# fnzhan/EMLight

Hardware: AMD Instinct MI355X
Metric: training images/sec (regression step: DenseNet-BC fwd + Sinkhorn loss + bwd + Adam) (higher is better)
Workload: dtype f32; 1 GPU; RegressionNetwork train step, BASELINE configs[1]; per_gpu_batch=64, global_batch=64, anchors=128, parallelism=single

## Files before the change

emlight_amd/RegressionNetwork/dense_engine_bwd.py:

```python
import ctypes
import os

import torch

from .. import _lib
from .._knobs import knob_choice, knob_flag


def _r16(v):
    return (v + 15) // 16 * 16


def _side_stream(dev, prio):
    if prio <= 0:
        return torch.cuda.Stream(device=dev, priority=prio)
    hip = ctypes.CDLL("libamdhip64.so")
    h = ctypes.c_void_p()
    with torch.cuda.device(dev):
        rc = hip.hipStreamCreateWithPriority(ctypes.byref(h), ctypes.c_uint(1), ctypes.c_int(prio))
    if rc != 0:
        raise RuntimeError("hipStreamCreateWithPriority failed (%d)" % rc)
    return torch.cuda.ExternalStream(h.value, device=dev)


def _masked_stream(dev, n_cu, keep):
    hip = ctypes.CDLL("libamdhip64.so")
    words = (n_cu + 31) // 32
    mask = (ctypes.c_uint32 * words)()
    for i in range(n_cu):
        if keep(i):
            mask[i // 32] |= 1 << (i % 32)
    h = ctypes.c_void_p()
    with torch.cuda.device(dev):
        rc = hip.hipExtStreamCreateWithCUMask(ctypes.byref(h), ctypes.c_uint32(words), mask)
    if rc != 0:
        raise RuntimeError("hipExtStreamCreateWithCUMask failed (%d)" % rc)
    return torch.cuda.ExternalStream(h.value, device=dev)


class _BwdBuffers:
    def gf12(self, r):
        if self.GF12[r] is None:
            self.GF12[r] = self._gf12_new()
        return self.GF12[r]

    def __init__(self, enc, ws, dev):
        f32 = dict(dtype=torch.float32, device=dev)
        self.G = [torch.zeros(blk["P"], blk["ld"], **f32) for blk in ws.blocks]
        self.GF = torch.zeros(ws.F.shape[0], ws.F.shape[1], **f32)
        maxP = ws.blocks[0]["P"]
        self.DZ = torch.empty(2, maxP, 48, **f32)
        self.ring = max(1, int(os.environ.get("EML_WGRAD_RING", 4))) if enc.overlap_wgrad(dev) else 1
        self.GF12 = [None] * self.ring
        self._gf12_new = lambda: torch.empty(maxP, 12, **f32)
        self.N12 = torch.empty(maxP, 12, **f32)
        self.TOP = torch.empty(2 * maxP * 12, **f32) if knob_flag("EML_DGRAD_TOP", True) else None
        kp, ko, g = enc.kp_max, max(enc.ko_max, 48), enc.grid_max
        self.Wd = [[torch.empty(lay["Kp"] * 48, **f32) for lay in blk["layers"]] for blk in ws.blocks]
        self.WdT = [torch.empty(blk["trans"]["Kp"] * blk["trans"]["Ko"], **f32) for blk in ws.blocks]
        self.permutes = None
        self.coef = torch.zeros(8, max(kp, ko), **f32)
        self.part2 = torch.zeros(2, g * kp * 2, dtype=torch.float64, device=dev)
        self.partW = torch.empty(g * max(kp * 48, 2 * 27 * 256, 4 * 1024), **f32)
        i32 = dict(dtype=torch.int32, device=dev)
        self.cond = [[torch.zeros(lay["Kp"], **i32) for lay in blk["layers"]] for blk in ws.blocks]
        self.condT = [torch.zeros(blk["trans"]["Kp"], **i32) for blk in ws.blocks]
        self.any_ill = torch.zeros(1, **i32)
        self.dg_grid = 128
        self.dg_scratch = torch.empty(self.dg_grid * kp, dtype=torch.float64, device=dev)
        self.side = None
        if enc.overlap_wgrad(dev):
            m = int(os.environ.get("EML_CU_SPLIT", 0))
            self.main_masked = None
            if m > 1:
                n_cu = torch.cuda.get_device_properties(dev).multi_processor_count
                self.side = _masked_stream(dev, n_cu, lambda i: i % m == m - 1)
                self.main_masked = _masked_stream(dev, n_cu, lambda i: i % m != m - 1)
            else:
                self.side = _side_stream(dev, int(os.environ.get("EML_SIDE_PRIO", 0)))
            self.partW3 = [torch.empty(g * 2 * 27 * 256, **f32) for _ in range(self.ring)]
            self.ev_ready = [torch.cuda.Event() for _ in range(self.ring)]
            self.ev_done = [None] * self.ring


def run_backward(enc, ws, x, gpooled, need_x=False, need_params=None):
    if getattr(ws, "bwd", None) is None:
        ws.bwd = _BwdBuffers(enc, ws, x.device)
    masked = getattr(ws.bwd, "main_masked", None)
    if masked is None:
        return _run_backward(enc, ws, x, gpooled, need_x, need_params)
    cur = torch.cuda.current_stream(x.device)
    masked.wait_stream(cur)
    with torch.cuda.stream(masked):
        out = _run_backward(enc, ws, x, gpooled, need_x, need_params)
    cur.wait_stream(masked)
    return out


def _run_backward(enc, ws, x, gpooled, need_x, need_params):
    L, p, st = _lib.lib(), _lib.ptr, _lib.current_stream()
    m = enc.model
    f = m.features
    if not m.training:
        raise NotImplementedError("HIP DenseNet backward is implemented for train-mode BatchNorm "
                                  "(EMLight trains and tests in train mode, train.py:42 / test.py:36-37)")
    dev = x.device
    B, _, H, W = x.shape
    G = enc._grid(dev)
    G3 = enc._grid3(dev)
    G3d = enc._tuned("EML_GRID3_DGRAD", 2 * G3 if knob_flag("EML_D3_SHORT", False) else G3)
    Gw = enc._tuned("EML_GRID_WGRAD1", G)
    Gd = enc._tuned("EML_GRID_DGRAD", G)
    Gb = min(enc.grid_max, 4 * enc._cu)
    bw = ws.bwd
    part = ws.partials
    ring = [0]
    if bw.side is not None:
        main = torch.cuda.current_stream(dev)
        st_side = ctypes.c_void_p(bw.side.cuda_stream)
        G3s = enc._tuned("EML_GRID3_SIDE", G3)
        bw.side.wait_stream(main)
    if bw.permutes is None:
        from .dense_engine import _PermuteTable
        bw.permutes = _PermuteTable()
    items = []
    for bi_, blk_ in enumerate(ws.blocks):
        mod_ = getattr(f, "denseblock%d" % (bi_ + 1))
        for l_, lay_ in enumerate(blk_["layers"]):
            items.append((getattr(mod_, "denselayer%d" % (l_ + 1)).conv1.weight, bw.Wd[bi_][l_], 2, 48, lay_["Cin"],
                          lay_["Kp"], 48))
        tr_ = blk_["trans"]
        items.append((getattr(f, "transition%d" % (bi_ + 1)).conv.weight, bw.WdT[bi_], 2, tr_["Cout"], blk_["Ctot"],
                      tr_["Kp"], tr_["Ko"]))
    bw.permutes.launch(L, st, items)
    params = enc.param_list()
    if need_params is None:
        need_params = [True] * len(params)
    from .._dist import grad_slot
    grads = {}
    for q, need in zip(params, need_params):
        slot = grad_slot(q) if need else None
        grads[id(q)] = slot if slot is not None else torch.empty_like(q)
    gr = lambda q: p(grads[id(q)])
    coefs = [tuple(bw.coef[3 * k + i] for i in range(3)) for k in range(2)]
    cA, cB, cC = coefs[0]
    sB, sC = bw.coef[6], bw.coef[7]

    direct = knob_choice("EML_DGAMMA_DIRECT", "always", ("always", "never")) != "never"
    c3_fold = knob_flag("EML_C3_FOLD", True)
    c3_gf = knob_flag("EML_C3_GF", False)
    bw.any_ill.zero_()

    def dgamma_direct(blk, X_ld, Pin, Hin, Win, pool, DY, ld_dy, Zr, ld_z, co, Cout, conv, Cin, scale1, shift1, cond, bn):
        if not direct:
            return
        a, b, c = co if co is not None else (None, None, None)
        _lib.check(L.eml_dense_bn_dgamma_direct_f32(
            p(blk["X"]), X_ld, Pin, Hin, Win, pool, p(DY), ld_dy, p(Zr), ld_z, p(a), p(b), p(c), Cout, p(conv.weight), Cin,
            p(scale1), p(shift1), p(blk["mean"]), p(blk["istd"]), p(cond), p(bw.dg_scratch), gr(bn.weight), bw.dg_grid, st),
            "eml_dense_bn_dgamma_direct_f32")

    def finalize(R, pstride, count, bn, mean, istd, C, Cpad, coef=0, s_acc=None, src=None, c_lo=0, c_hi=None, conv=None,
                 cond=None):
        a, b, c = coefs[coef] if coef is not None else (None, None, None)
        wargs = (p(bn.bias), p(conv.weight), gr(conv.weight), conv.weight.shape[0]) if conv is not None else (None, None, None, 0)
        _lib.check(L.eml_dense_bn_bwd_finalize_f32(
            p(part if src is None else src), R, pstride, float(count), p(bn.weight), p(mean), p(istd), C, Cpad, 1,
            gr(bn.weight), gr(bn.bias), p(a), p(b), p(c),
            p(sB) if s_acc is not None else None, p(sC) if s_acc is not None else None, int(bool(s_acc)),
            c_lo, Cpad if c_hi is None else c_hi, *wargs, p(cond), p(bw.any_ill) if cond is not None else None, st),
            "eml_dense_bn_bwd_finalize_f32")

    def parr(tensors):
        return (ctypes.c_void_p * len(tensors))(*[t.data_ptr() for t in tensors])

    def materialize(Gbuf, blk, c0, n):
        _lib.check(L.eml_dense_grad_materialize_f32(p(Gbuf), blk["ld"], p(blk["X"]), blk["ld"], p(sB), p(sC), c0, n,
                                                    blk["P"], st), "eml_dense_grad_materialize_f32")

    cf, k = enc.trans_cout[-1], enc.avgpool
    ldF = ws.F.shape[1]
    _lib.check(L.eml_dense_head_pool_bwd_f32(p(gpooled), p(ws.F), ldF, cf, B, ws.hf, ws.wf, k, p(bw.GF), ldF, st),
               "eml_dense_head_pool_bwd_f32")
    dY, ld_dy = bw.GF, ldF
    nb = len(ws.blocks)
    for bi in reversed(range(nb)):
        blk, tr = ws.blocks[bi], ws.blocks[bi]["trans"]
        mod = getattr(f, "denseblock%d" % (bi + 1))
        T, LN = getattr(f, "transition%d" % (bi + 1)), getattr(f, "last_norm%d" % (bi + 1))
        P, Hb, Wb, ld, ctot = blk["P"], blk["H"], blk["W"], blk["ld"], blk["Ctot"]
        cout, Ko, kpt = tr["Cout"], tr["Ko"], tr["Kp"]
        Pn = B * (Hb // 2) * (Wb // 2)
        Gbuf = bw.G[bi]
        gl0 = sum(enc.block_layers[:bi])
        top2 = bw.TOP[:2 * P * 12].view(2, P, 12) if bw.TOP is not None else None
        _lib.check(L.eml_dense_bn_bwd_stats_f32(p(dY), ld_dy, p(tr["T"]), Ko, None, 0, 0, cout, Pn, p(tr["tmean"]),
                                                p(tr["tistd"]), p(part), Gb, st), "eml_dense_bn_bwd_stats_f32")
        finalize(Gb, 2 * cout, Pn, LN, tr["tmean"], tr["tistd"], cout, Ko, coef=0)
        _lib.check(L.eml_dense_conv1x1_bwd_weight_f32(
            p(tr["A"]), kpt, Pn, Hb // 2, Wb // 2, 0, kpt, ctot, p(tr["one"]), p(tr["zero"]), p(dY), ld_dy, p(tr["T"]),
            Ko, p(cA), p(cB), p(cC), cout, p(bw.partW), gr(T.conv.weight), G, None, None, 0, None, 0, None, None, st),
            "eml_dense_conv1x1_bwd_weight_f32")
        _lib.check(L.eml_dense_conv1x1_bwd_data_f32(
            p(dY), ld_dy, p(tr["T"]), Ko, p(cA), p(cB), p(cC), Ko, p(bw.WdT[bi]), None, ld, p(tr["scale"]),
            p(tr["shift"]), None, None, Pn, Hb, Wb, 1, kpt, p(Gbuf), ld, 0, p(part), G, p(tr["mask16"]), st),
            "eml_dense_conv1x1_bwd_data_f32")
        finalize(G, 2 * kpt, P, T.norm, blk["mean"], blk["istd"], ctot, kpt, coef=None, s_acc=False, conv=T.conv,
                 cond=bw.condT[bi])
        dgamma_direct(blk, ld, P, Hb, Wb, 1, dY, ld_dy, tr["T"], Ko, coefs[0], cout, T.conv, ctot, tr["scale"], tr["shift"],
                      bw.condT[bi], T.norm)
        def conv2_backward(l, slot, n12=False, narrow_lo=None, top=False):
            lay = blk["layers"][l]
            Lm = getattr(mod, "denselayer%d" % (l + 1))
            cin, kp, z, dz = lay["Cin"], lay["Kp"], blk["Z"][l], bw.DZ[slot]
            gsrc = (p(bw.N12), 12, 0) if n12 else (p(top2[1]), 12, 0) if top else (p(Gbuf), ld, cin)
            r = ring[0] = (ring[0] + 1) % bw.ring
            if bw.side is not None and bw.ev_done[r] is not None:
                main.wait_event(bw.ev_done[r])
            fold = (bw.side is None and c3_fold
                    and L.eml_dense_conv3x3_bwd_fused_supported(gsrc[1], gsrc[2], ld, cin) == 1)
            q = ws.drop_plan[bi][l] if ws.drop_plan is not None else 0.0
            drop = (ws.drop_key, gl0 + l, q) if q > 0 else ()
            if fold:
                fn = "eml_dense_conv3x3_bwd_fused_drop_f32" if drop else "eml_dense_conv3x3_bwd_fused_f32"
                _lib.check(getattr(L, fn)(*gsrc, p(Lm.conv2.weight), p(z), p(lay["zmean"]), p(lay["zistd"]), p(dz), B, Hb, Wb,
                                          p(part), G3d, p(blk["X"]), ld, cin, p(sB), p(sC), p(bw.gf12(r)) if c3_gf else None,
                                          p(lay["scale2"]), p(lay["shift2"]), p(bw.partW), gr(Lm.conv2.weight), *drop, st), fn)
            else:
                fn = "eml_dense_conv3x3_bwd_data_drop_f32" if drop else "eml_dense_conv3x3_bwd_data_f32"
                _lib.check(getattr(L, fn)(*gsrc, p(Lm.conv2.weight), p(z), p(lay["zmean"]), p(lay["zistd"]), p(dz), B, Hb, Wb,
                                          p(part), G3d, p(blk["X"]), ld, cin, p(sB), p(sC), p(bw.gf12(r)), *drop, st), fn)
            if fold:
                pass
            elif bw.side is None:
                _lib.check(L.eml_dense_conv3x3_bwd_weight_f32(p(bw.gf12(r)), 12, 0, p(z), p(lay["scale2"]),
                                                              p(lay["shift2"]), B, Hb, Wb, p(bw.partW),
                                                              gr(Lm.conv2.weight), G3, st),
                           "eml_dense_conv3x3_bwd_weight_f32")
            else:
                bw.ev_ready[r].record(main)
                bw.side.wait_event(bw.ev_ready[r])
                _lib.check(L.eml_dense_conv3x3_bwd_weight_f32(p(bw.gf12(r)), 12, 0, p(z), p(lay["scale2"]),
                                                              p(lay["shift2"]), B, Hb, Wb, p(bw.partW3[r]),
                                                              gr(Lm.conv2.weight), G3s, st_side),
                           "eml_dense_conv3x3_bwd_weight_f32")
                if bw.ev_done[r] is None:
                    bw.ev_done[r] = torch.cuda.Event()
                bw.ev_done[r].record(bw.side)
            finalize(G3d, 96, P, Lm.norm2, lay["zmean"], lay["zistd"], 48, 48, coef=slot)
            a, b, c = coefs[slot]
            _lib.check(L.eml_dense_conv1x1_bwd_weight_f32(
                p(blk["X"]), ld, P, Hb, Wb, 0, kp, cin, p(lay["scale1"]), p(lay["shift1"]), p(dz), 48, p(z), 48,
                p(a), p(b), p(c), 48, p(bw.partW), gr(Lm.conv1.weight), Gw, p(dz),
                *((p(Lm.conv1.weight), narrow_lo, *((p(top2[0]), 12) if top else (p(Gbuf), ld)), p(bw.N12),
                   p(bw.part2[slot])) if narrow_lo is not None
                  else (None, 0, None, 0, None, None)), st), "eml_dense_conv1x1_bwd_weight_f32")
            return Lm

        def dgrad(layers, slots, k_lo, k_hi, top=False):
            lays = [blk["layers"][l] for l in layers]
            if top:
                _lib.check(L.eml_dense_conv1x1_bwd_data_multi_top_f32(
                    parr([bw.DZ[s_] for s_ in slots]), parr([bw.Wd[bi][l_] for l_ in layers]),
                    parr([y["scale1"] for y in lays]), parr([y["shift1"] for y in lays]),
                    parr([bw.part2[s_] for s_ in slots]), (ctypes.c_int * len(layers))(*[y["Kp"] for y in lays]),
                    P, k_hi, p(Gbuf), ld, Gd, parr([y["mask"] for y in lays]), p(top2), st),
                    "eml_dense_conv1x1_bwd_data_multi_top_f32")
                return
            _lib.check(L.eml_dense_conv1x1_bwd_data_multi_f32(
                len(layers), parr([bw.DZ[s_] for s_ in slots]), None, None, None, None,
                parr([bw.Wd[bi][l_] for l_ in layers]),
                parr([y["scale1"] for y in lays]), parr([y["shift1"] for y in lays]),
                parr([bw.part2[s_] for s_ in slots]), (ctypes.c_int * len(layers))(*[y["Kp"] for y in lays]),
                None, ld, None, None, P, k_lo, k_hi, p(Gbuf), ld, Gd,
                parr([y["mask"] for y in lays]), st),
                "eml_dense_conv1x1_bwd_data_multi_f32")

        def bn1_finalize(l, Lm, slot, c_lo, c_hi, rows=None):
            lay = blk["layers"][l]
            finalize(Gd if rows is None else rows, 2 * lay["Kp"], P, Lm.norm1, blk["mean"], blk["istd"], lay["Cin"], lay["Kp"], coef=None,
                     s_acc=True, src=bw.part2[slot], c_lo=c_lo, c_hi=c_hi, conv=Lm.conv1, cond=bw.cond[bi][l])

        def bn1_direct(l, Lm, slot):
            lay = blk["layers"][l]
            dgamma_direct(blk, ld, P, Hb, Wb, 0, bw.DZ[slot], 48, None, 0, None, 48, Lm.conv1, lay["Cin"], lay["scale1"],
                          lay["shift1"], bw.cond[bi][l], Lm.norm1)

        l = len(blk["layers"]) - 1
        have_top = False
        while l >= 0:
            if l >= 1:
                la, lb = l, l - 1
                cin_a, cin_b = blk["layers"][la]["Cin"], blk["layers"][lb]["Cin"]
                Lma = conv2_backward(la, 0, narrow_lo=cin_b, top=have_top)
                bn1_finalize(la, Lma, 0, cin_b, cin_a, rows=Gw)
                Lmb = conv2_backward(lb, 1, n12=True)
                to_top = (top2 is not None and lb >= 2 and blk["layers"][la]["mask"] is not None and bw.side is None
                          and cin_b >= 24 and cin_b % 4 == 0)
                dgrad([la, lb], [0, 1], 0, cin_b, top=to_top)
                have_top = to_top
                bn1_finalize(la, Lma, 0, 0, cin_b)
                bn1_finalize(lb, Lmb, 1, 0, blk["layers"][lb]["Kp"])
                bn1_direct(la, Lma, 0)
                bn1_direct(lb, Lmb, 1)
                l -= 2
            else:
                Lm0 = conv2_backward(l, 0)
                dgrad([l], [0], 0, blk["layers"][l]["Cin"])
                bn1_finalize(l, Lm0, 0, 0, blk["layers"][l]["Kp"])
                bn1_direct(l, Lm0, 0)
                l -= 1
        c0b = blk["C0"]
        norm0_fused = bi == 0 and knob_flag("EML_NORM0_FUSED", True) and c0b % 4 == 0 and c0b <= 32
        if not norm0_fused:
            materialize(Gbuf, blk, 0, c0b)
        dY, ld_dy = Gbuf, ld
    b0 = ws.blocks[0]
    c0 = enc.c_init
    if norm0_fused:
        _lib.check(L.eml_dense_norm0_bwd_stats_f32(p(dY), ld_dy, p(ws.Y0), c0, p(ws.scale0), p(ws.shift0), p(sB), p(sC), c0,
                                                   b0["P"], p(ws.mean0), p(ws.istd0), p(part), Gb, st),
                   "eml_dense_norm0_bwd_stats_f32")
    else:
        _lib.check(L.eml_dense_bn_bwd_stats_f32(p(dY), ld_dy, p(ws.Y0), c0, p(b0["X"]), b0["ld"], 1, c0, b0["P"],
                                                p(ws.mean0), p(ws.istd0), p(part), Gb, st), "eml_dense_bn_bwd_stats_f32")
    finalize(Gb, 2 * c0, b0["P"], f.norm0, ws.mean0, ws.istd0, c0, _r16(c0), coef=0)
    if norm0_fused:
        _lib.check(L.eml_dense_conv0_bwd_weight_fused_f32(p(x), p(dY), ld_dy, p(ws.Y0), c0, p(ws.scale0), p(ws.shift0), p(sB),
                                                          p(sC), p(cA), p(cB), p(cC), B, H, W, p(bw.partW),
                                                          gr(f.conv0.weight), G, st), "eml_dense_conv0_bwd_weight_fused_f32")
    else:
        _lib.check(L.eml_dense_conv0_bwd_weight_f32(p(x), p(dY), ld_dy, p(b0["X"]), b0["ld"], p(ws.Y0), c0, p(cA), p(cB),
                                                    p(cC), B, H, W, p(bw.partW), gr(f.conv0.weight), G, st),
                   "eml_dense_conv0_bwd_weight_f32")
    dx = None
    if need_x:
        dx = torch.empty(B, 3, H, W, dtype=torch.float32, device=dev)
        X1 = (None, 0) if norm0_fused else (p(b0["X"]), b0["ld"])
        _lib.check(L.eml_dense_conv0_bwd_data_f32(p(dY), ld_dy, *X1, p(ws.Y0), c0, p(ws.scale0), p(ws.shift0), p(sB), p(sC),
                                                  p(cA), p(cB), p(cC), p(f.conv0.weight), B, H, W, p(dx), st),
                   "eml_dense_conv0_bwd_data_f32")
    if bw.side is not None:
        main.wait_stream(bw.side)
    return dx, [grads[id(q)] for q in params]
```

emlight_amd/_lib.py:

```python
import ctypes
import os
import threading

_HERE = os.path.dirname(os.path.abspath(__file__))
LIB_PATH = os.environ.get("EML_LIB_PATH") or os.path.join(_HERE, "libemlight_hip.so")

_f32p = ctypes.c_void_p
_i32p = ctypes.c_void_p
_f64p = ctypes.c_void_p
_stream = ctypes.c_void_p
_int = ctypes.c_int
_u64 = ctypes.c_ulonglong

ABI_VERSION = 31

SIGNATURES = {
    "eml_abi_version": (_int, []),
    "eml_last_error": (ctypes.c_char_p, []),
    "eml_sg_rasterise_f32": (_int, [_f32p, _f32p, _f32p, _f32p, _int, _int, _int, _int, _stream]),
    "eml_sg_rasterise_ex_f32": (_int, [_f32p, _f32p, _f32p, _f32p, _int, _int, _int, _int, _int, ctypes.c_void_p, _stream]),
    "eml_sg_rasterise_bwd_colors_f32": (_int, [_f32p, _f32p, _f32p, _f32p, _int, _int, _int, _int, _stream]),
    "eml_emd_anchor_cost_f32": (_int, [_f32p, _f32p, _int, _stream]),
    "eml_sinkhorn_schedule_f32": (_int, [_f32p, _f32p, ctypes.c_long, ctypes.c_double, ctypes.c_double, _int,
                                         ctypes.c_double, _f32p, _f32p, _i32p, _f32p, _stream]),
    "eml_sinkhorn_work_floats": (ctypes.c_size_t, [_int, _int]),
    "eml_sinkhorn_fwd_f32": (_int, [_f32p, _f32p, _f32p, _f32p, _f32p, _f32p, ctypes.c_double, ctypes.c_double, _int,
                                    ctypes.c_double, _f32p, _f32p, _i32p, _f32p, _f32p, _f32p, _f32p, _f32p, _int, _int,
                                    _stream]),
    "eml_sinkhorn_fwd_ex_f32": (_int, [_f32p, _f32p, _f32p, _f32p, _f32p, _f32p, ctypes.c_double, ctypes.c_double, _int,
                                       ctypes.c_double, _f32p, _f32p, _i32p, _f32p, _f32p, _f32p, _f32p, _f32p, _int, _int,
                                       _int, _stream]),
    "eml_sinkhorn_fwd_rho_f32": (_int, [_f32p, _f32p, _f32p, _f32p, _f32p, _f32p, ctypes.c_double, ctypes.c_double, _int,
                                        ctypes.c_double, _f32p, _f32p, _i32p, _f32p, _f32p, _f32p, _f32p, _f32p, _int, _int,
                                        _int, ctypes.c_double, _f32p, _stream]),
    "eml_sinkhorn_bwd_f32": (_int, [_f32p, _f32p, _f32p, _int, _int, _stream]),
    "eml_sinkhorn_dim_work_floats": (ctypes.c_size_t, [_int, _int, _int]),
    "eml_sinkhorn_fwd_dim_f32": (_int, [_f32p, _f32p, _f32p, _f32p, _f32p, _f32p, ctypes.c_double, ctypes.c_double, _int,
                                        ctypes.c_double, _f32p, _f32p, _i32p, _f32p, _f32p, _f32p, _f32p, _f32p, _int, _int,
                                        _int, _int, ctypes.c_double, _f32p, _stream]),
    "eml_sinkhorn_schedule_dim_f32": (_int, [_f32p, _f32p, ctypes.c_long, _int, ctypes.c_double, ctypes.c_double, _int,
                                             ctypes.c_double, _f32p, _f32p, _i32p, _f32p, _stream]),
    "eml_sinkhorn_bwd_weights_f32": (_int, [_f32p, _f32p, _f32p, _f32p, _int, _int, _stream]),
    "eml_l1_pairs_partial_doubles": (ctypes.c_size_t, [_int]),
    "eml_l1_pairs_fwd_f32": (_int, [_int, ctypes.c_void_p, ctypes.c_void_p, ctypes.c_void_p, ctypes.c_void_p, ctypes.c_void_p,
                                    ctypes.c_void_p, _f64p, _f32p, _stream]),
    "eml_l1_pairs_bwd_f32": (_int, [_int, ctypes.c_void_p, ctypes.c_void_p, ctypes.c_void_p, ctypes.c_void_p, ctypes.c_void_p,
                                    ctypes.c_void_p, _f32p, ctypes.c_void_p, ctypes.c_void_p, ctypes.c_void_p, _stream]),
    "eml_colsum_partial_doubles": (ctypes.c_size_t, [_int]),
    "eml_colsum_f32": (_int, [_f32p, ctypes.c_long, _int, _f64p, _f32p, _stream]),
    "eml_gt_anchor_index_i32": (_int, [_f32p, _int, _int, _int, _i32p, _stream]),
    "eml_gt_parametrise_f64": (_int, [_f32p, _i32p, _i32p, _int, _int, _int, _int, _f32p, _f32p, _f32p, _stream]),
    "eml_pano_crop_f32": (_int, [ctypes.c_void_p, _int, _int, _int, _int, _int, _int, ctypes.c_double, ctypes.c_double, _f64p,
                                 ctypes.c_double, _f64p, _f32p, _stream]),
    "eml_pano_resize_area_f32": (_int, [_f32p, _int, _int, _int, _int, _int, ctypes.c_double, _f64p, _f32p, _stream]),
    "eml_tonemap_work_floats": (ctypes.c_size_t, [_int]),
    "eml_tonemap_f32": (_int, [_f32p, _int, ctypes.c_long, _int, ctypes.c_double, ctypes.c_double, ctypes.c_double, _f32p,
                               _int, _f32p, _f32p, _i32p, _f32p, ctypes.c_void_p, _stream]),
    "eml_projector_targets_work_floats": (ctypes.c_size_t, [_int, _int, _int]),
    "eml_projector_targets_f32": (_int, [_f32p, _f32p, _int, _int, _int, _f32p, _f32p, _f32p, _stream]),
    "eml_resize_bilinear_f32": (_int, [_f32p, _f32p, _int, _int, _int, _int, _int, _int, _int, _f32p, _stream]),
    "eml_sphere_tap_table_f32": (_int, [_f32p, _int, _int, _int, _int, _i32p, _f32p, _stream]),
    "eml_sphere_im2col_f32": (_int, [_f32p, _i32p, _f32p, _f32p, _int, _int, _int, _int, _stream]),
    "eml_sphere_col2im_f32": (_int, [_f32p, _i32p, _i32p, _f32p, _f32p, _int, _int, _int, _int, _stream]),
    "eml_sphere_conv_fwd_fused_f32": (_int, [_f32p, _i32p, _f32p, _f32p, _f32p, _f32p, _int, _int, _int, _int, _int, _int,
                                             _stream]),
    "eml_sphere_conv_fwd_fused_ex_f32": (_int, [_f32p, _i32p, _f32p, _f32p, _f32p, _f32p, _int, _int, _int, _int, _int, _int,
                                                _f32p, ctypes.c_float, _int, _stream]),
    "eml_sphere_conv_small_supported": (_int, [_int, _int]),
    "eml_sphere_conv_small_fwd_f32": (_int, [_f32p, _i32p, _f32p, _f32p, _f32p, _f32p, _int, _int, _int, _int, _int,
                                             ctypes.c_float, _stream]),
    "eml_sphere_conv_small_wgrad_partial_floats": (ctypes.c_size_t, [_int, _int, _int, _int]),
    "eml_sphere_conv_small_wgrad_f32": (_int, [_f32p, _i32p, _f32p, _f32p, _f32p, ctypes.c_float, _f32p, _f32p, _f32p, _int,
                                               _int, _int, _int, _int, _stream]),
    "eml_sphere_conv_small_da9_f32": (_int, [_f32p, _f32p, ctypes.c_float, _f32p, _f32p, ctypes.c_long, _int, _int, _stream]),
    "eml_spade_norm_modulate_up2_fwd_f32": (_int, [_f32p, _f32p, _f32p, _int, _int, _int, _int, ctypes.c_float, _f32p, _f32p,
                                                   _stream]),
    "eml_spade_norm_modulate_bwd_cols_f32": (_int, [_f32p, _f32p, _f32p, _f32p, _f32p, _int, _int, _int, _int, _int,
                                                    ctypes.c_float, _f32p, _f32p, _f32p, _int, _stream]),
    "eml_sg_rasterise_bwd_work_floats": (ctypes.c_size_t, [_int, _int, _int, _int]),
    "eml_sg_rasterise_bwd_colors_ex_f32": (_int, [_f32p, _f32p, _f32p, _f32p, _f32p, _int, _int, _int, _int, _int, _stream]),
    "eml_sg_rasterise_bwd_full_work_floats": (ctypes.c_size_t, [_int, _int, _int, _int]),
    "eml_sg_rasterise_bwd_f32": (_int, [_f32p, _f32p, _f32p, _f32p, _f32p, _f32p, _f32p, _f32p, _int, _int, _int, _int, _int,
                                        _stream]),
    "eml_sphere_conv_narrow_supported": (_int, [_int, _int]),
    "eml_sphere_conv_narrow_fwd_f32": (_int, [_f32p, _i32p, _f32p, _f32p, _f32p, _f32p, _int, _int, _int, _int, _int, _stream]),
    "eml_sphere_conv_narrow_dgrad_f32": (_int, [_f32p, _i32p, _f32p, _int, _f32p, _f32p, _int, _int, _int, _int, _int, _stream]),
    "eml_sphere_conv_narrow_wgrad_partial_floats": (ctypes.c_size_t, [_int, _int, _int, _int]),
    "eml_sphere_conv_narrow_wgrad_f32": (_int, [_f32p, _i32p, _f32p, _f32p, _f32p, _f32p, _int, _int, _int, _int, _int, _stream]),
    "eml_sphere_conv_narrow_scratch_floats": (ctypes.c_size_t, [_int, _int]),
    "eml_sphere_conv_narrow_fwd2_f32": (_int, [_f32p, _i32p, _f32p, _f32p, _f32p, _f32p, _f32p, _int, _int, _int, _int, _int, _stream]),
    "eml_sphere_conv_narrow_wgrad2_partial_floats": (ctypes.c_size_t, [_int, _int, _int]),
    "eml_sphere_conv_narrow_dgrad2_f32": (_int, [_f32p, _i32p, _f32p, _int, ctypes.c_void_p, _f32p, _f32p, _f32p, _int, _int, _int,
                                                 _int, _int, _int, _stream]),
    "eml_sphere_conv_narrow_wgrad2_f32": (_int, [_f32p, _i32p, _f32p, _int, ctypes.c_void_p, _f32p, _f32p, _f32p, _f32p, _int, _int,
                                                 _int, _int, _int, _stream]),
    "eml_sphere_conv_spade_supported": (_int, [_int, _int, ctypes.c_long]),
    "eml_sphere_conv_spade_fwd_f32": (_int, [_f32p, _i32p, _f32p, _f32p, _f32p, _f32p, _f32p, _f32p, _f32p, _f32p, _int, _int,
                                             _int, _int, _int, _int, ctypes.c_float, _int, _stream]),
    "eml_spade_norm_modulate_bwd_y_f32": (_int, [_f32p, _f32p, _f32p, _f32p, _f32p, _f32p, _int, _int, _int, _int, _int,
                                                 ctypes.c_float, _f32p, _f32p, _f32p, _int, _stream]),
    "eml_bn_bwd_apply_up2_f32": (_int, [_f32p, _f32p, _int, _int, _int, _int, _f32p, _f32p, _f32p, _f32p, _stream]),
    "eml_spectral_norm_scratch_floats": (ctypes.c_size_t, [_int, _int]),
    "eml_spectral_norm_w2_f32": (_int, [_f32p, _f32p, _f32p, _int, ctypes.c_float, _f32p, _f32p, _f32p, _f32p, _int, _int,
                                        _stream]),
    "eml_spectral_norm_w2_bwd_f32": (_int, [_f32p, _f32p, _f32p, _f32p, _f32p, _f32p, _f32p, _int, _int, _stream]),
    "eml_spectral_norm_w2_batch_f32": (_int, [_int, ctypes.c_void_p, ctypes.c_void_p, ctypes.c_void_p, _int, ctypes.c_float,
                                              ctypes.c_void_p, ctypes.c_void_p, ctypes.c_void_p, ctypes.c_void_p, ctypes.c_void_p,
                                              ctypes.c_void_p, _stream]),
    "eml_spade_heads_w2_f32": (_int, [_f32p, _f32p, _f32p, _f32p, _f32p, _f32p, _int, _int, _int, _stream]),
    "eml_instance_norm_act_fwd_f32": (_int, [_f32p, _f32p, _f32p, _int, _int, _int, _int, ctypes.c_float, ctypes.c_float,
                                             _stream]),
    "eml_instance_norm_act_bwd_f32": (_int, [_f32p, _f32p, _f32p, _f32p, _int, _int, _int, _int, ctypes.c_float, _stream]),
    "eml_sphere_conv_dgrad_fused_f32": (_int, [_f32p, _i32p, _f32p, _i32p, _int, _f32p, _f32p, _int, _int, _int, _int, _int,
                                               _int, _stream]),
    "eml_sphere_conv_lowres_variant": (_int, [_int, _int, _int, _int]),
    "eml_sphere_conv_lowres_table_i32": (_int, [_i32p, _i32p, _i32p, _int, _int, _stream]),
    "eml_sphere_conv_lowres_partial_floats": (ctypes.c_size_t, [ctypes.c_long, _int, _int]),
    "eml_sphere_conv_lowres_f32": (_int, [_f32p, _i32p, _f32p, _i32p, _int, _i32p, _int, _f32p, _f32p, _f32p, _f32p, _int, _int,
                                          _int, _int, _int, _int, _f32p, ctypes.c_float, _stream]),
    "eml_sphere_conv_wgrad_partial_floats": (ctypes.c_size_t, [_int, _int, _int]),
    "eml_sphere_conv_wgrad_fused_f32": (_int, [_f32p, _i32p, _f32p, _f32p, _f32p, _f32p, _int, _int, _int, _int, _int, _int,
                                               _stream]),
    "eml_spade_modulate_fwd_f32": (_int, [_f32p, _int, _f32p, _int, _f32p, _int, ctypes.c_long, _int, ctypes.c_float,
                                          _stream]),
    "eml_spade_modulate_bwd_f32": (_int, [_f32p, _int, _f32p, _int, _f32p, _int, _f32p, _int, _f32p, _int, ctypes.c_long,
                                          _int, ctypes.c_float, _stream]),
    "eml_bn_stats_f32": (_int, [_f32p, _int, ctypes.c_long, _int, _f32p, _int, _stream]),
    "eml_bn_fold_f64": (_int, [_f32p, _int, _int, _f32p, _stream]),
    "eml_bn_finalize_f32": (_int, [_f32p, _int, ctypes.c_float, ctypes.c_float, _f32p, _f32p, _f32p, _f32p, _stream]),
    "eml_spade_norm_modulate_fwd_f32": (_int, [_f32p, _int, _f32p, _int, _f32p, _int, ctypes.c_long, _int, ctypes.c_float,
                                               _f32p, _f32p, _stream]),
    "eml_bn_bwd_apply_f32": (_int, [_f32p, _int, _f32p, _int, ctypes.c_long, _int, _f32p, _f32p, _f32p, _f32p, _int,
                                    _stream]),
    "eml_dense_conv0_fwd_f32": (_int, [_f32p, _f32p, _f32p, _int, _int, _int, _int, _int, _f32p, _int, _stream]),
    "eml_dense_conv0_fwd_mfma_f32": (_int, [_f32p, _f32p, _f32p, _int, _int, _int, _int, _int, _f32p, _int, _stream]),
    "eml_dense_bn_apply_f32": (_int, [_f32p, _int, _f32p, _int, _int, ctypes.c_long, _f32p, _f32p, _int, _f32p,
                                      _int, _stream]),
    "eml_dense_bn_prepare_f32": (_int, [_f32p, _int, _int, _int, _int, ctypes.c_double, _f32p, _f32p, _f32p, _f32p,
                                        _f32p, _f32p, _f32p, _int, _int, ctypes.c_float, ctypes.c_float, _int,
                                        _f32p, _f32p, _stream]),
    "eml_dense_permute_w1_f32": (_int, [_f32p, _int, _int, _int, _f32p, _stream]),
    "eml_dense_permute_w2_f32": (_int, [_f32p, _int, _f32p, _stream]),
    "eml_dense_permute_batch_f32": (_int, [ctypes.c_void_p, _int, _stream]),
    "eml_dense_conv1x1_fwd_f32": (_int, [_f32p, _int, ctypes.c_long, _int, _int, _int, _int, _f32p, _f32p, _f32p,
                                         _int, _f32p, _int, _f32p, _int, ctypes.c_void_p, _stream]),
    "eml_dense_conv3x3_fwd_f32": (_int, [_f32p, _f32p, _f32p, _f32p, _f32p, _int, _int, _int, _int, _int, _f32p,
                                         _int, _stream]),
    "eml_dense_permute_w2_tp_f32": (_int, [_f32p, _f32p, _stream]),
    "eml_dense_conv3x3_fwd_tp_supported": (_int, [_int, _int, _int]),
    "eml_dense_conv3x3_fwd_tp_f32": (_int, [_f32p, _f32p, _f32p, _f32p, _f32p, _int, _int, _int, _int, _int, _int, _f32p,
                                            _int, _stream]),
    "eml_dense_conv3x3_fwd_drop_f32": (_int, [_f32p, _f32p, _f32p, _f32p, _f32p, _int, _int, _int, _int, _int, _f32p,
                                              _int, _u64, _int, ctypes.c_double, _stream]),
    "eml_dense_conv3x3_fwd_tp_drop_f32": (_int, [_f32p, _f32p, _f32p, _f32p, _f32p, _int, _int, _int, _int, _int, _int, _f32p,
                                                 _int, _u64, _int, ctypes.c_double, _stream]),
    "eml_dense_dropout_mask_u16": (_int, [_u64, _int, ctypes.c_double, ctypes.c_long, ctypes.c_void_p, _stream]),
    "eml_dense_pool_act_f32": (_int, [_f32p, _int, _int, _int, _int, _int, _f32p, _f32p, _f32p, _int, ctypes.c_void_p,
                                      _stream]),
    "eml_dense_head_pool_fwd_f32": (_int, [_f32p, _int, _int, _int, _int, _int, _int, _f32p, _stream]),
    "eml_dense_conv3x3_bwd_data_f32": (_int, [_f32p, _int, _int, _f32p, _f32p, _f32p, _f32p, _f32p, _int, _int, _int,
                                              _f32p, _int, _f32p, _int, _int, _f32p, _f32p, _f32p, _stream]),
    "eml_dense_conv3x3_bwd_fused_supported": (_int, [_int, _int, _int, _int]),
    "eml_dense_conv3x3_bwd_fused_f32": (_int, [_f32p, _int, _int, _f32p, _f32p, _f32p, _f32p, _f32p, _int, _int, _int, _f64p, _int,
                                               _f32p, _int, _int, _f32p, _f32p, _f32p, _f32p, _f32p, _f32p, _f32p, _stream]),
    "eml_dense_conv3x3_bwd_data_drop_f32": (_int, [_f32p, _int, _int, _f32p, _f32p, _f32p, _f32p, _f32p, _int, _int, _int,
                                                   _f32p, _int, _f32p, _int, _int, _f32p, _f32p, _f32p, _u64, _int,
                                                   ctypes.c_double, _stream]),
    "eml_dense_conv3x3_bwd_fused_drop_f32": (_int, [_f32p, _int, _int, _f32p, _f32p, _f32p, _f32p, _f32p, _int, _int, _int,
                                                    _f64p, _int, _f32p, _int, _int, _f32p, _f32p, _f32p, _f32p, _f32p, _f32p,
                                                    _f32p, _u64, _int, ctypes.c_double, _stream]),
    "eml_dense_conv3x3_bwd_weight_f32": (_int, [_f32p, _int, _int, _f32p, _f32p, _f32p, _int, _int, _int, _f32p,
                                                _f32p, _int, _stream]),
    "eml_dense_bn_bwd_finalize_f32": (_int, [_f32p, _int, _int, ctypes.c_double, _f32p, _f32p, _f32p, _int, _int,
                                             _int, _f32p, _f32p, _f32p, _f32p, _f32p, _f32p, _f32p, _int, _int, _int,
                                             _f32p, _f32p, _f32p, _int, _i32p, _i32p, _stream]),
    "eml_dense_bn_dgamma_direct_f32": (_int, [_f32p, _int, ctypes.c_long, _int, _int, _int, _f32p, _int, _f32p, _int,
                                              _f32p, _f32p, _f32p, _int, _f32p, _int, _f32p, _f32p, _f32p, _f32p, _i32p,
                                              _f32p, _f32p, _int, _stream]),
    "eml_dense_conv1x1_bwd_weight_f32": (_int, [_f32p, _int, ctypes.c_long, _int, _int, _int, _int, _int, _f32p,
                                                _f32p, _f32p, _int, _f32p, _int, _f32p, _f32p, _f32p, _int, _f32p,
                                                _f32p, _int, _f32p, _f32p, _int, _f32p, _int, _f32p, _f32p, _stream]),
    "eml_dense_conv1x1_bwd_narrow_f32": (_int, [_f32p, _f32p, _int, _int, _f32p, _int, _f32p, _f32p, _f32p, _f32p,
                                                ctypes.c_long, _f32p, _int, _f32p, _f32p, _int, _int, _stream]),
    "eml_dense_permute_w1_bwd_f32": (_int, [_f32p, _int, _int, _int, _int, _f32p, _stream]),
    "eml_dense_conv1x1_bwd_data_f32": (_int, [_f32p, _int, _f32p, _int, _f32p, _f32p, _f32p, _int, _f32p, _f32p,
                                              _int, _f32p, _f32p, _f32p, _f32p, ctypes.c_long, _int, _int, _int,
                                              _int, _f32p, _int, _int, _f32p, _int, ctypes.c_void_p, _stream]),
    "eml_dense_conv1x1_bwd_data_multi_f32": (_int, [_int] + [ctypes.c_void_p] * 10 + [_f32p, _int, _f32p, _f32p,
                                                    ctypes.c_long, _int, _int, _f32p, _int, _int, ctypes.c_void_p,
                                                    _stream]),
    "eml_dense_conv1x1_bwd_data_multi_top_f32": (_int, [ctypes.c_void_p] * 6 + [ctypes.c_long, _int, _f32p, _int, _int,
                                                        ctypes.c_void_p, _f32p, _stream]),
    "eml_dense_grad_materialize_f32": (_int, [_f32p, _int, _f32p, _int, _f32p, _f32p, _int, _int, ctypes.c_long,
                                              _stream]),
    "eml_dense_bn_bwd_stats_f32": (_int, [_f32p, _int, _f32p, _int, _f32p, _int, _int, _int, ctypes.c_long, _f32p,
                                          _f32p, _f32p, _int, _stream]),
    "eml_dense_norm0_bwd_stats_f32": (_int, [_f32p, _int, _f32p, _int, _f32p, _f32p, _f32p, _f32p, _int, ctypes.c_long, _f32p, _f32p,
                                             ctypes.c_void_p, _int, _stream]),
    "eml_dense_conv0_bwd_weight_fused_f32": (_int, [_f32p, _f32p, _int, _f32p, _int, _f32p, _f32p, _f32p, _f32p, _f32p, _f32p, _f32p,
                                                    _int, _int, _int, _f32p, _f32p, _int, _stream]),
    "eml_dense_conv0_bwd_weight_f32": (_int, [_f32p, _f32p, _int, _f32p, _int, _f32p, _int, _f32p, _f32p, _f32p,
                                              _int, _int, _int, _f32p, _f32p, _int, _stream]),
    "eml_dense_conv0_bwd_data_f32": (_int, [_f32p, _int, _f32p, _int, _f32p, _int, _f32p, _f32p, _f32p, _f32p, _f32p, _f32p,
                                            _f32p, _f32p, _int, _int, _int, _f32p, _stream]),
    "eml_dense_head_pool_bwd_f32": (_int, [_f32p, _f32p, _int, _int, _int, _int, _int, _int, _f32p, _int, _stream]),
}

_lock = threading.Lock()
_lib = None


class EmlightHipError(RuntimeError):
    pass


def lib():
    global _lib
    if _lib is not None:
        return _lib
    with _lock:
        if _lib is not None:
            return _lib
        if not os.path.exists(LIB_PATH):
            raise EmlightHipError(
                "libemlight_hip.so not found at %s -- build it with "
                "`python -c 'import __graft_entry__ as g; g.build()'` or `make -C emlight_amd/csrc`. "
                "There is no CPU fallback." % LIB_PATH)
        handle = ctypes.CDLL(LIB_PATH)
        for name, (res, args) in SIGNATURES.items():
            try:
                fn = getattr(handle, name)
            except AttributeError as e:
                raise EmlightHipError("libemlight_hip.so lacks symbol %s" % name) from e
            fn.restype, fn.argtypes = res, args
        got = handle.eml_abi_version()
        if got != ABI_VERSION:
            raise EmlightHipError("libemlight_hip.so has ABI version %d, this binding expects %d -- rebuild it "
                                  "(make -C emlight_amd/csrc)" % (got, ABI_VERSION))
        _lib = handle
    from . import _gemm_selection
    _gemm_selection.ensure_if_requested()
    return _lib


_DEBUG_SYNC = bool(os.environ.get("EML_DEBUG_SYNC"))


def check(rc, what):
    if rc != 0:
        msg = lib().eml_last_error()
        raise EmlightHipError("%s failed (rc=%d): %s" % (what, rc, msg.decode() if msg else "?"))
    if _DEBUG_SYNC:
        import sys
        import torch
        sys.stderr.write("[eml] %s ... " % what)
        sys.stderr.flush()
        torch.cuda.synchronize()
        sys.stderr.write("ok\n")


def ptr(t):
    if t is None:
        return None
    return ctypes.c_void_p(t.data_ptr())


def current_stream():
    import torch
    return ctypes.c_void_p(torch.cuda.current_stream().cuda_stream)


def require_gpu_tensor(t, name, dtype=None):
    import torch
    if not isinstance(t, torch.Tensor) or not t.is_cuda:
        raise EmlightHipError("%s must be a tensor on the MI355X (got %s); there is no CPU path"
                              % (name, getattr(t, "device", type(t))))
    if t.dtype != (dtype or torch.float32):
        raise EmlightHipError("%s must be %s (got %s)" % (name, dtype or torch.float32, t.dtype))
    return t.contiguous()
```

emlight_amd/csrc/dense_bwd.hip:

```cpp
#include "eml_common.h"
#include "eml_dropout.h"

#include <cstdint>
#include <cstdlib>
#include <type_traits>

namespace {

using f32x4 = __attribute__((ext_vector_type(4))) float;

__device__ __forceinline__ f32x4 mfma16(float a, float b, f32x4 c) {
  return __builtin_amdgcn_mfma_f32_16x16x4f32(a, b, c, 0, 0, 0);
}
__device__ __forceinline__ float f4c(const float4& v, int t) { return t == 0 ? v.x : t == 1 ? v.y : t == 2 ? v.z : v.w; }
__device__ __forceinline__ double shfl_xor_d(double v, int m) { return __shfl_xor(v, m, 64); }

constexpr int kTH = 8, kTW = 32, kHH = kTH + 2, kHW = kTW + 2;

constexpr int kPSG = 14;
constexpr int kBD = 512;
constexpr int kGRows = 2;
constexpr int kGPass = kHH / kGRows;

template <bool FUSE, bool WIDE, int TH, bool DROP = false>
// ... 837 lines not shown
    asm volatile("s_mov_b32 %0, m0\n\ts_mov_b32 m0, %2\n\ts_nop 0\n\tglobal_load_lds_dwordx4 %1, off\n\ts_mov_b32 m0, %0"
                 : "=&s"(keep) : "v"(src), "s"(dst) : "memory");
  };

  int tile = blockIdx.x, cur = 0;
  __syncthreads();
  if (tile < ntiles) {
    stage_begin(tile);
    g_load(0);
    g_load(1);
    {
      const int b = tile / (ty_n * tx_n), rem = tile - b * (ty_n * tx_n);
#pragma unroll
      for (int it = 0; it < kZI; ++it) z_dma(it, b, (rem / tx_n) * kTH, (rem % tx_n) * kTW, 0);
    }
    g_wait();
    g_commit(0, g_l);
    g_commit(1, g_l);
    g_store(0);
    g_store(1);
  }
  __syncthreads();
#ifdef EML_STAMPS
  unsigned long long st_acc[5] = {0, 0, 0, 0, 0}, st_last = __builtin_readcyclecounter();
#endif
  for (; tile < ntiles; tile += gridDim.x) {
    const int nxt = tile + gridDim.x;
    const float* gc = g_l + cur * kGT;
    float* gn = g_l + (cur ^ 1) * kGT;
    const int b = tile / (ty_n * tx_n), rem = tile - b * (ty_n * tx_n);
    const int ty = rem / tx_n, tx = rem - ty * tx_n;
    const int gy = ty * kTH + wave;
    size_t prow[2];
    bool pv[2];
#pragma unroll
    for (int m = 0; m < 2; ++m) {
      const int gx = tx * kTW + 16 * m + r;
      pv[m] = gy < H && gx < W;
      prow[m] = ((size_t)(b * H + min(gy, H - 1)) * W + min(gx, W - 1)) * 48;
    }
    stage_begin(nxt < ntiles ? nxt : tile);
    f32x4 acc[2][3];
#pragma unroll
    for (int m = 0; m < 2; ++m)
#pragma unroll
      for (int n = 0; n < 3; ++n) acc[m][n] = f32x4{0.f, 0.f, 0.f, 0.f};
    float aq[2][2], wq[2][3];
#pragma unroll
    for (int n = 0; n < 3; ++n) wq[0][n] = w_l[n * 64 + lane];
#pragma unroll
    for (int m = 0; m < 2; ++m) aq[0][m] = gc[((wave + 2) * kHW + 16 * m + r + 2) * kPSG + kk];
#pragma unroll
    for (int tap = 0; tap < 9; ++tap) {
#pragma unroll
      for (int s3 = 0; s3 < 3; ++s3) {
        const int gi = tap * 3 + s3;
        if (gi < 2) {
          g_load(gi);
          asm volatile("" ::: "memory");
          __builtin_amdgcn_sched_barrier(0);
        }
        if (gi + 1 < 27) {
          const int tn = (gi + 1) / 3, sn = (gi + 1) - 3 * tn, dyn = tn / 3, dxn = tn - 3 * dyn;
#pragma unroll
          for (int n = 0; n < 3; ++n) wq[(gi + 1) & 1][n] = w_l[((gi + 1) * 3 + n) * 64 + lane];
#pragma unroll
          for (int m = 0; m < 2; ++m)
            aq[(gi + 1) & 1][m] = gc[((wave + 2 - dyn) * kHW + 16 * m + r + 2 - dxn) * kPSG + 4 * sn + kk];
        }
        __builtin_amdgcn_sched_barrier(0);
#pragma unroll
        for (int m = 0; m < 2; ++m)
#pragma unroll
          for (int n = 0; n < 3; ++n) acc[m][n] = mfma16(wq[gi & 1][n], aq[gi & 1][m], acc[m][n]);
        if (gi >= 25) {
          __builtin_amdgcn_sched_barrier(0);
          if (gi == 25) g_wait();
          g_commit(gi - 25, gn);
        }
      }
    }
    g_store(0);
    g_store(1);
    EML_C3_STAMP(0);
#ifndef EML_C3_NOZWAIT
    asm volatile("s_waitcnt vmcnt(0)" ::: "memory");
#endif
    eml::lds_barrier();
    EML_C3_STAMP(1);
    const float* ga = gc + ((2 * pairj + 1) * kHW + kk + 1) * kPSG;
    const float* zc = z_l + cur * (kTH * kTW * kZS);
    const float* zb = zc + (kTW * 2 * pairj + kk) * kZS + r;
    const int xl0 = ty * kTH + 2 * pairj < H ? W - tx * kTW - kk : 0, xl1 = ty * kTH + 2 * pairj + 1 < H ? W - tx * kTW - kk : 0;
    auto phase_b = [&](auto nt_tag) {
      constexpr int NT = decltype(nt_tag)::value;
      float av[2][NT], bz[2][3];
#pragma unroll
      for (int i = 0; i < NT; ++i) av[0][i] = ga[goff[i]];
#pragma unroll
      for (int n = 0; n < 3; ++n) bz[0][n] = zb[16 * n];
#pragma unroll
      for (int ks = 0; ks < 16; ++ks) {
        if (ks + 1 < 16) {
          const int k1 = ks + 1, go = ((k1 >> 3) * kHW + 4 * (k1 & 7)) * kPSG, zo = ((k1 >> 3) * kTW + 4 * (k1 & 7)) * kZS;
#pragma unroll
          for (int i = 0; i < NT; ++i) av[k1 & 1][i] = ga[go + goff[i]];
#pragma unroll
          for (int n = 0; n < 3; ++n) bz[k1 & 1][n] = zb[zo + 16 * n];
        }
        __builtin_amdgcn_sched_barrier(0);
        if (ks == 1) {
          const int t2 = nxt < ntiles ? nxt : tile;
          const int b2 = t2 / (ty_n * tx_n), rem2 = t2 - b2 * (ty_n * tx_n);
#ifndef EML_C3_NOZDMA
#pragma unroll
          for (int it = 0; it < kZI; ++it) z_dma(it, b2, (rem2 / tx_n) * kTH, (rem2 % tx_n) * kTW, cur ^ 1);
#endif
          __builtin_amdgcn_sched_barrier(0);
        }
        const bool pin = 4 * (ks & 7) < (ks < 8 ? xl0 : xl1);
        float bv[3];
#pragma unroll
        for (int n = 0; n < 3; ++n) bv[n] = pin ? fmaf(bz[ks & 1][n], scb[n], shb[n]) : 0.f;
#pragma unroll
        for (int i = 0; i < NT; ++i) {
          const float a = (i < 3 || r < 12) ? av[ks & 1][i] : 0.f;
#pragma unroll
          for (int n = 0; n < 3; ++n) accw[i][n] = mfma16(a, bv[n], accw[i][n]);
        }
        if (ks == 2 || ks == 4 || ks == 6) {
          const int n = (ks - 2) >> 1;
          float l1[4] = {0.f, 0.f, 0.f, 0.f}, l2[4] = {0.f, 0.f, 0.f, 0.f};
#pragma unroll
          for (int m = 0; m < 2; ++m) {
            const float4 z = *reinterpret_cast<const float4*>(zc + (kTW * wave + 16 * m + r) * kZS + 16 * n + 4 * kk);
#pragma unroll
            for (int g = 0; g < 4; ++g) {
              const float v = pv[m] ? acc[m][n][g] : 0.f;
              l1[g] += v;
              l2[g] = fmaf(v, f4c(z, g), l2[g]);
            }
          }
#pragma unroll
          for (int g = 0; g < 4; ++g) {
            const float t1 = eml::row16_sum(l1[g]), t2 = eml::row16_sum(l2[g]);
            if (r == 0) {
              double* d = red + (wave * 48 + 16 * n + 4 * kk + g) * 2;
              d[0] += (double)t1;
              d[1] += (double)t2;
            }
          }
        } else if (ks >= 8 && ks < 14) {
          const int si = ks - 8, m = si / 3, n = si - 3 * m;
          if (pv[m])
            *reinterpret_cast<float4*>(DZ + prow[m] + 16 * n + 4 * kk) =
                make_float4(acc[m][n][0], acc[m][n][1], acc[m][n][2], acc[m][n][3]);
        }
        __builtin_amdgcn_sched_barrier(0);
      }
    };
    if (role == 0) phase_b(std::integral_constant<int, 3>{});
    else phase_b(std::integral_constant<int, 4>{});
    EML_C3_STAMP(2);
    eml::lds_barrier();
    EML_C3_STAMP(3);
#ifdef EML_STAMPS
    st_acc[4] += 1;
#endif
    cur ^= 1;
  }
#ifdef EML_STAMPS
  if (tid == 0)
    for (int i = 0; i < 5; ++i) atomicAdd(&eml_c3_stamps[i], st_acc[i]);
#endif
  asm volatile("s_waitcnt vmcnt(0)" ::: "memory");
  __syncthreads();
  float* wsum = smem;
  for (int w8 = 0; w8 < 8; ++w8) {
    if (wave == w8) {
#pragma unroll
      for (int i = 0; i < 4; ++i)
        if (i < 3 + role) {
#pragma unroll
          for (int n = 0; n < 3; ++n)
#pragma unroll
            for (int g = 0; g < 4; ++g) {
              float* q = wsum + ((((3 * role + i) * 3 + n) * 16 + 4 * kk + g) * 16 + r);
              *q = ((w8 & 3) == 0 ? 0.f : *q) + accw[i][n][g];
            }
        }
    }
    __syncthreads();
  }
  for (int e = tid; e < 21 * 256; e += 512) partialW[(size_t)blockIdx.x * (21 * 256) + e] = wsum[e];
  if (tid < 48) {
    double t1 = 0.0, t2 = 0.0;
#pragma unroll
    for (int w8 = 0; w8 < 8; ++w8) {
      t1 += red[(w8 * 48 + tid) * 2 + 0];
      t2 += red[(w8 * 48 + tid) * 2 + 1];
    }
    partials[(size_t)blockIdx.x * 96 + 2 * tid + 0] = t1;
    partials[(size_t)blockIdx.x * 96 + 2 * tid + 1] = (double)zistd[tid] * (t2 - (double)zmean[tid] * t1);
  }
}


__global__ __launch_bounds__(256) void bn_bwd_finalize_kernel(
    const double* __restrict__ partials, int R, int pstride, double count, const float* __restrict__ gamma,
    const float* __restrict__ mean, const float* __restrict__ istd, int C, int Cpad, int training,
    float* __restrict__ dgamma, float* __restrict__ dbeta, float* __restrict__ cA, float* __restrict__ cB,
    float* __restrict__ cC, float* __restrict__ sB, float* __restrict__ sC, int s_accumulate, int c_lo, int c_hi,
    const float* __restrict__ beta, const float* __restrict__ Wc, const float* __restrict__ dWc, int w_rows,
    int* __restrict__ cond , int* __restrict__ any_cond ) {
  const int lane = threadIdx.x & 63, wave = threadIdx.x >> 6;
  const int c = c_lo + blockIdx.x * 4 + wave;
  if (c >= Cpad || c >= c_hi) return;
  float a = 0.f, b = 0.f, d = 0.f;
  if (c < C) {
    double S1 = 0.0, S2 = 0.0;
    for (int g = lane; g < R; g += 64) {
      S1 += partials[(size_t)g * pstride + 2 * c];
      S2 += partials[(size_t)g * pstride + 2 * c + 1];
    }
    double Q = 0.0;
    if (Wc)
      for (int o = lane; o < w_rows; o += 64) Q += (double)Wc[(size_t)o * C + c] * (double)dWc[(size_t)o * C + c];
#pragma unroll
    for (int o = 32; o > 0; o >>= 1) {
      S1 += __shfl_xor(S1, o, 64);
      S2 += __shfl_xor(S2, o, 64);
      Q += __shfl_xor(Q, o, 64);
    }
    if (Wc) {
      const double ga0 = gamma[c], bs = (double)beta[c] * S1, num = Q - bs;
      S2 = fabs(ga0) >= 1e-12 ? num / ga0 : 0.0;
      if (cond && lane == 0) {
        const int ill = fabs(ga0) < 1e-3 * fabs((double)beta[c]) || ga0 == 0.0;
        cond[c] = ill;
        if (ill && any_cond) *any_cond = 1;
      }
    }
    if (lane == 0) {
      dgamma[c] = (float)S2;
      dbeta[c] = (float)S1;
    }
    const double ga = gamma[c], is = istd[c], mu = mean[c];
    a = (float)(ga * is);
    if (training) {
      b = (float)(-ga * is * is * S2 / count);
      d = (float)(-ga * is * S1 / count + ga * is * is * S2 / count * mu);
    }
  }
  if (lane != 0) return;
  if (cA) {
    cA[c] = a;
    cB[c] = b;
    cC[c] = d;
  }
  if (sB) {
    sB[c] = (s_accumulate ? sB[c] : 0.f) + b;
    sC[c] = (s_accumulate ? sC[c] : 0.f) + d;
  }
}

__global__ __launch_bounds__(256) void reduce_rows_kernel(const float* __restrict__ partial, int R, size_t row_stride,
                                                          int mode, int dim0, int dim1, int n0,
                                                          float* __restrict__ out) {
  __shared__ double red[4][64];
  const int tid = threadIdx.x, e = blockIdx.x * 64 + (tid & 63), slice = tid >> 6;
  size_t src = 0, dst = 0;
  bool valid = false;
  if (mode == 0) {
    const int k = e / 48, o = e - 48 * k;
    valid = k < dim0 && o < dim1;
    src = (size_t)e;
    dst = (size_t)(n0 + o) * dim0 + k;
  } else if (mode == 1) {
    const int o = e & 15, ci = (e >> 4) & 15, pair = e >> 8, tap = pair / 3, mc = pair - 3 * tap;
    valid = pair < 27 && o < 12;
    src = (size_t)e;
    dst = (size_t)(o * 48 + 16 * mc + ci) * 9 + tap;
  } else if (mode == 3) {
    const int j = e & 15, i = (e >> 4) & 15, tn = e >> 8, t = tn / 3, n = tn - 3 * t, row = 16 * t + i;
    valid = tn < 21 && row < 108;
    src = (size_t)e;
    dst = (size_t)((row % 12) * 48 + 16 * n + j) * 9 + row / 12;
  } else {
    const int t = e >> 5, o = e & 31;
    valid = t < 27 && o < dim1;
    src = (size_t)e;
    dst = (size_t)o * 27 + t;
  }
  double s = 0.0;
  if (valid) {
#pragma unroll 8
    for (int r = slice; r < R; r += 4) s += (double)partial[(size_t)r * row_stride + src];
  }
  red[slice][tid & 63] = s;
  __syncthreads();
  if (slice == 0 && valid) out[dst] = (float)((red[0][tid] + red[1][tid]) + (red[2][tid] + red[3][tid]));
}

struct NarrowArgs {
  const float* W1;
  const float* G;
  float* N12;
  double* partials;
  int Cin, k_lo, ldg;
};
template <bool POOL, bool NARROW = false, int VEC = 2>
__global__ __launch_bounds__(256, (NARROW || VEC == 4) ? 2 : 1) void conv1x1_bwd_weight_kernel(
    const float* __restrict__ X, int ldx, int P, int Hin, int Win, int Kp, const float* __restrict__ scale1,
    const float* __restrict__ shift1, const float* __restrict__ DY, int ld_dy, const float* __restrict__ Zr,
    int ld_z, const float* __restrict__ cA, const float* __restrict__ cB, const float* __restrict__ cC, int n_valid,
    int n_load ,
    float* __restrict__ partial ,
    float* __restrict__ dz_out ,
    NarrowArgs na) {
  __shared__ __attribute__((aligned(16))) float dz_l[2][64 * 48];
  const int tid = threadIdx.x, lane = tid & 63, wave = tid >> 6;
  const int r = lane & 15, kk = lane >> 4;
  static_assert(VEC == 2 || (VEC == 4 && !POOL), "float4 operand: dense layers only");
  constexpr int GW = 16 * VEC;
  constexpr int MAXG = VEC == 2 ? 3 : 2;
  const int ngroups = (Kp + GW - 1) / GW;
  float nsk[4] = {0.f, 0.f, 0.f, 0.f}, ntk[4] = {0.f, 0.f, 0.f, 0.f};
  double ns1[4] = {0.0, 0.0, 0.0, 0.0};
  const int kq = min(kk, 2);
  if constexpr (NARROW) {
#pragma unroll
    for (int g = 0; g < 4; ++g) {
      nsk[g] = kk < 3 ? scale1[na.k_lo + 4 * kq + g] : 0.f;
      ntk[g] = kk < 3 ? shift1[na.k_lo + 4 * kq + g] : 0.f;
    }
  }

  float sv[MAXG][VEC], tv[MAXG][VEC];
  int coff[MAXG];
  bool gv[MAXG];
#pragma unroll
  for (int i = 0; i < MAXG; ++i) {
    const int cg = wave + 4 * i;
    const int ch = GW * cg + VEC * r;
    gv[i] = cg < ngroups && ch < Kp;
    coff[i] = gv[i] ? ch : 0;
#pragma unroll
    for (int t = 0; t < VEC; ++t) {
      sv[i][t] = gv[i] ? scale1[ch + t] : 0.f;
      tv[i][t] = gv[i] ? shift1[ch + t] : 0.f;
    }
  }
  const int spix = tid >> 2, sq = tid & 3;
  __shared__ __attribute__((aligned(16))) float co_l[3 * 48];
  __shared__ float wn_l[NARROW ? 12 * 64 : 1];
  constexpr bool CO_LDS = NARROW || VEC == 4;
  float4 sa_r[CO_LDS ? 1 : 3], sb_r[CO_LDS ? 1 : 3], sc_r[CO_LDS ? 1 : 3];
  if constexpr (CO_LDS) {
    if (tid < 48) {
      const bool v = tid < n_valid;
      co_l[tid] = v ? cA[tid] : 0.f;
      co_l[48 + tid] = v ? cB[tid] : 0.f;
      co_l[96 + tid] = v ? cC[tid] : 0.f;
    }
  } else {
#pragma unroll
    for (int j = 0; j < 3; ++j) {
      const int col = 4 * (sq + 4 * j);
      float a[4], b[4], c[4];
#pragma unroll
      for (int e = 0; e < 4; ++e) {
        const bool v = col + e < n_valid;
        a[e] = v ? cA[col + e] : 0.f;
        b[e] = v ? cB[col + e] : 0.f;
        c[e] = v ? cC[col + e] : 0.f;
      }
      sa_r[j] = make_float4(a[0], a[1], a[2], a[3]);
      sb_r[j] = make_float4(b[0], b[1], b[2], b[3]);
      sc_r[j] = make_float4(c[0], c[1], c[2], c[3]);
    }
  }
  if constexpr (NARROW) {
    for (int e = tid; e < 12 * 64; e += 256) {
      const int st = e >> 6, l = e & 63, rr = l & 15, k4 = l >> 4;
      wn_l[e] = rr < 12 ? na.W1[(size_t)(4 * st + k4) * na.Cin + na.k_lo + rr] : 0.f;
    }
  }
  __syncthreads();
  f32x4 acc[MAXG][VEC][3];
#pragma unroll
  for (int i = 0; i < MAXG; ++i)
#pragma unroll
    for (int t = 0; t < VEC; ++t)
#pragma unroll
      for (int n = 0; n < 3; ++n) acc[i][t][n] = f32x4{0.f, 0.f, 0.f, 0.f};

  const int Wo = Win >> 1, Ho = Hin >> 1;
  const int nchunks = (P + 63) >> 6;
  const int ngw = (ngroups > wave) ? (ngroups - wave + 3) >> 2 : 0;

  float4 rdy[3], rzr[3];
  bool rpv = false;
  int rp = 0;
  auto stage_load = [&](int chunk) {
    const int p = chunk * 64 + spix;
    rpv = chunk < nchunks && p < P;
    const size_t pc = rpv ? p : 0;
    rp = (int)pc;
#pragma unroll
    for (int j = 0; j < 3; ++j) {
      const int col = 4 * (sq + 4 * j);
      const bool cv = col < n_load;
      rdy[j] = cv ? *reinterpret_cast<const float4*>(DY + pc * ld_dy + col) : make_float4(0.f, 0.f, 0.f, 0.f);
      rzr[j] = cv ? *reinterpret_cast<const float4*>(Zr + pc * ld_z + col) : make_float4(0.f, 0.f, 0.f, 0.f);
    }
  };
  auto stage_write = [&](float* dzb) {
#pragma unroll
    for (int j = 0; j < 3; ++j) {
      const int col = 4 * (sq + 4 * j);
      float4 sa, sb, sc;
      if constexpr (CO_LDS) {
        sa = *reinterpret_cast<const float4*>(co_l + col);
        sb = *reinterpret_cast<const float4*>(co_l + 48 + col);
        sc = *reinterpret_cast<const float4*>(co_l + 96 + col);
      } else {
        sa = sa_r[j];
        sb = sb_r[j];
        sc = sc_r[j];
      }
      float4 v;
      v.x = rpv ? fmaf(sa.x, rdy[j].x, fmaf(sb.x, rzr[j].x, sc.x)) : 0.f;
      v.y = rpv ? fmaf(sa.y, rdy[j].y, fmaf(sb.y, rzr[j].y, sc.y)) : 0.f;
      v.z = rpv ? fmaf(sa.z, rdy[j].z, fmaf(sb.z, rzr[j].z, sc.z)) : 0.f;
      v.w = rpv ? fmaf(sa.w, rdy[j].w, fmaf(sb.w, rzr[j].w, sc.w)) : 0.f;
      *reinterpret_cast<float4*>(dzb + spix * 48 + col) = v;
      if (dz_out && rpv) *reinterpret_cast<float4*>(dz_out + (size_t)rp * 48 + col) = v;
    }
  };
  auto chunk_loop = [&](auto ngw_c) {
    constexpr int NGW = decltype(ngw_c)::value;
#ifdef EML_WGRAD_DEEP
    constexpr int UQ = POOL ? 1 : 2;
    constexpr int NBUF = POOL ? 2 : 4;
#else
    constexpr int UQ = POOL ? 1 : (VEC == 4 ? 2 : 4);
    constexpr int NBUF = 2;
#endif
    constexpr int NS = POOL ? 4 : 1;
    constexpr int NB = 16 / UQ;
    constexpr int AHEAD = NBUF - 1;
    using xv_t = std::conditional_t<VEC == 2, float2, float4>;
    xv_t xr[NBUF][UQ][NGW > 0 ? NGW : 1][NS];
    auto load_batch = [&](int chunk, int q0, xv_t (&dst)[UQ][NGW > 0 ? NGW : 1][NS]) {
#pragma unroll
      for (int u = 0; u < UQ; ++u) {
        const int pc = min(chunk * 64 + 4 * (q0 + u) + kk, P - 1);
        const float* xp;
        if constexpr (POOL) {
          const int b = pc / (Ho * Wo), rem = pc - b * (Ho * Wo);
          const int oy = rem / Wo, ox = rem - oy * Wo;
          xp = X + ((size_t)(b * Hin + 2 * oy) * Win + 2 * ox) * ldx;
        } else {
          xp = X + (size_t)pc * ldx;
        }
#pragma unroll
        for (int i = 0; i < NGW; ++i)
#pragma unroll
          for (int sub = 0; sub < NS; ++sub)
            dst[u][i][sub] = *reinterpret_cast<const xv_t*>(xp + ((sub >> 1) * (size_t)Win + (sub & 1)) * ldx + coff[i]);
      }
    };
    stage_load(blockIdx.x);
    stage_write(dz_l[0]);
    if constexpr (NGW > 0) {
#pragma unroll
      for (int a = 0; a < AHEAD; ++a) load_batch(min((int)blockIdx.x, nchunks - 1), a * UQ, xr[a]);
    }
    __syncthreads();
    int it = 0;
    for (int chunk = blockIdx.x; chunk < nchunks; chunk += gridDim.x, ++it) {
      const float* dzb = dz_l[it & 1];
      stage_load(chunk + gridDim.x);
      float2 nx[2], ng[2];
      const int pn = chunk * 64 + 16 * wave + r;
      if constexpr (NARROW) {
        const size_t pc = (size_t)min(pn, P - 1);
        const float* xs = X + pc * ldx + na.k_lo + 4 * kq;
        const float* gs = na.G + pc * na.ldg + (na.ldg == 12 ? 0 : na.k_lo) + 4 * kq;
        nx[0] = *reinterpret_cast<const float2*>(xs);
        nx[1] = *reinterpret_cast<const float2*>(xs + 2);
        ng[0] = *reinterpret_cast<const float2*>(gs);
        ng[1] = *reinterpret_cast<const float2*>(gs + 2);
      }
      if constexpr (NGW > 0) {
        float bzq[2][3];
#pragma unroll
        for (int n = 0; n < 3; ++n) bzq[0][n] = dzb[kk * 48 + 16 * n + r];
#pragma unroll
        for (int bi = 0; bi < NB; ++bi) {
          const int q0 = bi * UQ;
          if (bi + AHEAD < NB)
            load_batch(chunk, q0 + AHEAD * UQ, xr[(bi + AHEAD) % NBUF]);
          else
            load_batch(min(chunk + (int)gridDim.x, nchunks - 1), (bi + AHEAD - NB) * UQ, xr[(bi + AHEAD) % NBUF]);
          __builtin_amdgcn_sched_barrier(0);
#pragma unroll
          for (int u = 0; u < UQ; ++u) {
            const int pl = 4 * (q0 + u) + kk;
            const bool pvu = chunk * 64 + pl < P;
            float bz[3];
#pragma unroll
            for (int n = 0; n < 3; ++n) bz[n] = bzq[(q0 + u) & 1][n];
            if (q0 + u + 1 < 16) {
#pragma unroll
              for (int n = 0; n < 3; ++n) bzq[(q0 + u + 1) & 1][n] = dzb[(pl + 4) * 48 + 16 * n + r];
            }
#pragma unroll
            for (int i = 0; i < NGW; ++i) {
              float av[VEC];
#pragma unroll
              for (int t = 0; t < VEC; ++t) av[t] = 0.f;
#pragma unroll
              for (int sub = 0; sub < NS; ++sub) {
                const xv_t xv = xr[bi % NBUF][u][i][sub];
                av[0] += fmaxf(fmaf(xv.x, sv[i][0], tv[i][0]), 0.f);
                av[1] += fmaxf(fmaf(xv.y, sv[i][1], tv[i][1]), 0.f);
                if constexpr (VEC == 4) {
                  av[2] += fmaxf(fmaf(xv.z, sv[i][2], tv[i][2]), 0.f);
                  av[3] += fmaxf(fmaf(xv.w, sv[i][3], tv[i][3]), 0.f);
                }
              }
#pragma unroll
              for (int t = 0; t < VEC; ++t) {
                if constexpr (POOL) av[t] *= 0.25f;
                if (!pvu) av[t] = 0.f;
              }
#pragma unroll
              for (int n = 0; n < 3; ++n)
#pragma unroll
                for (int t = 0; t < VEC; ++t) acc[i][t][n] = mfma16(av[t], bz[n], acc[i][t][n]);
            }
          }
          __builtin_amdgcn_sched_barrier(0);
        }
      }
      if constexpr (NARROW) {
        asm volatile("" ::"v"(ng[0].x), "v"(ng[0].y), "v"(ng[1].x), "v"(ng[1].y), "v"(nx[0].x), "v"(nx[0].y), "v"(nx[1].x), "v"(nx[1].y));
        f32x4 an = f32x4{0.f, 0.f, 0.f, 0.f};
#pragma unroll
        for (int st = 0; st < 12; ++st) an = mfma16(wn_l[st * 64 + lane], dzb[(16 * wave + r) * 48 + 4 * st + kk], an);
        const bool nv = pn < P && kk < 3;
        const float xg[4] = {nx[0].x, nx[0].y, nx[1].x, nx[1].y}, gg[4] = {ng[0].x, ng[0].y, ng[1].x, ng[1].y};
        float o4[4];
#pragma unroll
        for (int g = 0; g < 4; ++g) {
          const float dam = (nv && fmaf(xg[g], nsk[g], ntk[g]) > 0.f) ? an[g] : 0.f;
          o4[g] = fmaf(nsk[g], dam, gg[g]);
          ns1[g] += (double)dam;
        }
        if (nv) *reinterpret_cast<float4*>(na.N12 + ((unsigned)pn * 12u + 4u * (unsigned)kk)) = make_float4(o4[0], o4[1], o4[2], o4[3]);
      }
      stage_write(dz_l[(it + 1) & 1]);
      eml::lds_barrier();
    }
  };
  switch (ngw) {
    case 0: chunk_loop(std::integral_constant<int, 0>{}); break;
    case 1: chunk_loop(std::integral_constant<int, 1>{}); break;
    case 2: chunk_loop(std::integral_constant<int, 2>{}); break;
    default: chunk_loop(std::integral_constant<int, MAXG>{}); break;
  }
  float* out = partial + (size_t)blockIdx.x * Kp * 48;
#pragma unroll
  for (int i = 0; i < MAXG; ++i) {
    const int cg = wave + 4 * i;
#pragma unroll
    for (int t = 0; t < VEC; ++t)
#pragma unroll
      for (int g = 0; g < 4; ++g) {
        const int ch = GW * cg + VEC * (4 * kk + g) + t;
        if (cg < ngroups && ch < Kp) {
#pragma unroll
          for (int n = 0; n < 3; ++n) out[(size_t)ch * 48 + 16 * n + r] = acc[i][t][n][g];
        }
      }
  }
  if constexpr (NARROW) {
    __syncthreads();
    double* red = reinterpret_cast<double*>(&dz_l[0][0]);
#pragma unroll
    for (int g = 0; g < 4; ++g) {
#pragma unroll
      for (int o = 1; o < 16; o <<= 1) ns1[g] += shfl_xor_d(ns1[g], o);
      if (r == 0 && kk < 3) red[wave * 12 + 4 * kk + g] = ns1[g];
    }
    __syncthreads();
    if (tid < 12) {
      double* dst = na.partials + ((size_t)blockIdx.x * Kp + na.k_lo + tid) * 2;
      dst[0] = (red[tid] + red[12 + tid]) + (red[24 + tid] + red[36 + tid]);
      dst[1] = 0.0;
    }
  }
}

template <bool POOL, bool RES , int NCH = 4>
__global__ __launch_bounds__(256) void conv1x1_bwd_data_kernel(
    const float* __restrict__ DY, int ld_dy, const float* __restrict__ Zr, int ld_z, const float* __restrict__ cA,
    const float* __restrict__ cB, const float* __restrict__ cC, int Ko, const float* __restrict__ Wd,
    const float* __restrict__ X, int ldx, const float* __restrict__ scale1, const float* __restrict__ shift1,
    const float* __restrict__ mean, const float* __restrict__ istd, int P, int Hin, int Win, int Kp,
    float* __restrict__ Gd, int ldg, int accumulate, double* __restrict__ partials ) {
  extern __shared__ __attribute__((aligned(16))) float smem[];
  double* sacc = reinterpret_cast<double*>(smem);
  const int tid = threadIdx.x, lane = tid & 63, wave = tid >> 6;
  const int r = lane & 15, kk = lane >> 4;
  for (int e = tid; e < 4 * Kp * 2; e += 256) sacc[e] = 0.0;
  __syncthreads();
  double* my = sacc + (size_t)wave * Kp * 2;
  const int nnt = Kp >> 4, njo = Ko >> 4;
  const int ntiles = (P + 255) >> 8;
  const int Wo = Win >> 1, Ho = Hin >> 1;

  for (int tile = blockIdx.x; tile < ntiles; tile += gridDim.x) {
    const int p0 = tile * 256 + wave * 64;
    long prow[4];
    size_t pin[4];
#pragma unroll
    for (int m = 0; m < 4; ++m) {
      prow[m] = min(p0 + 16 * m + r, P - 1);
      if constexpr (POOL) {
        const int b = (int)(prow[m] / (Ho * Wo)), rem = (int)(prow[m] - (long)b * (Ho * Wo));
        const int oy = rem / Wo, ox = rem - oy * Wo;
        pin[m] = (size_t)(b * Hin + 2 * oy) * Win + 2 * ox;
      } else {
        pin[m] = (size_t)prow[m];
      }
    }
    auto load_dz = [&](int jo, float4 (&dz)[4]) {
      const int ch = 16 * jo + 4 * kk;
      const float4 a4 = *reinterpret_cast<const float4*>(cA + ch);
      const float4 b4 = *reinterpret_cast<const float4*>(cB + ch);
      const float4 c4 = *reinterpret_cast<const float4*>(cC + ch);
#pragma unroll
      for (int m = 0; m < 4; ++m) {
        const float4 dy = *reinterpret_cast<const float4*>(DY + prow[m] * ld_dy + ch);
        const float4 zr = *reinterpret_cast<const float4*>(Zr + prow[m] * ld_z + ch);
        dz[m].x = fmaf(a4.x, dy.x, fmaf(b4.x, zr.x, c4.x));
        dz[m].y = fmaf(a4.y, dy.y, fmaf(b4.y, zr.y, c4.y));
        dz[m].z = fmaf(a4.z, dy.z, fmaf(b4.z, zr.z, c4.z));
        dz[m].w = fmaf(a4.w, dy.w, fmaf(b4.w, zr.w, c4.w));
      }
    };
    float4 dzr[3][4];
    if constexpr (RES) {
#pragma unroll
      for (int jo = 0; jo < 3; ++jo) load_dz(jo, dzr[jo]);
    }
    for (int nt0 = 0; nt0 < nnt; nt0 += NCH) {
      f32x4 acc[4][NCH];
#pragma unroll
      for (int m = 0; m < 4; ++m)
#pragma unroll
        for (int n = 0; n < NCH; ++n) acc[m][n] = f32x4{0.f, 0.f, 0.f, 0.f};
      auto mma = [&](int jo, const float4 (&dz)[4]) {
#pragma unroll
        for (int n = 0; n < NCH; ++n) {
          const int nt = min(nt0 + n, nnt - 1);
          const float4 w = *reinterpret_cast<const float4*>(Wd + ((((size_t)nt * njo + jo) * 4 + kk) * 16 + r) * 4);
#pragma unroll
          for (int t = 0; t < 4; ++t)
#pragma unroll
            for (int m = 0; m < 4; ++m) acc[m][n] = mfma16(f4c(w, t), f4c(dz[m], t), acc[m][n]);
        }
      };
      if constexpr (RES) {
#pragma unroll
        for (int jo = 0; jo < 3; ++jo) mma(jo, dzr[jo]);
      } else {
        for (int jo = 0; jo < njo; ++jo) {
          float4 dz[4];
          load_dz(jo, dz);
          mma(jo, dz);
        }
      }
#pragma unroll
      for (int n = 0; n < NCH; ++n) {
        const int nt = nt0 + n;
        if (nt < nnt) {
          const int k4 = 16 * nt + 4 * kk;
          const float4 sk = *reinterpret_cast<const float4*>(scale1 + k4);
          const float4 tk = *reinterpret_cast<const float4*>(shift1 + k4);
          const float4 mu = *reinterpret_cast<const float4*>(mean + k4);
          const float4 is = *reinterpret_cast<const float4*>(istd + k4);
          float l1[4] = {0.f, 0.f, 0.f, 0.f}, l2[4] = {0.f, 0.f, 0.f, 0.f};
#pragma unroll
          for (int m = 0; m < 4; ++m) {
            if (p0 + 16 * m + r < P) {
              const float da[4] = {acc[m][n][0], acc[m][n][1], acc[m][n][2], acc[m][n][3]};
              constexpr int NSUB = POOL ? 4 : 1;
#pragma unroll
              for (int sub = 0; sub < NSUB; ++sub) {
                const size_t pi = pin[m] + (sub >> 1) * (size_t)Win + (sub & 1);
                const float4 xv = *reinterpret_cast<const float4*>(X + pi * ldx + k4);
                float4* gp = reinterpret_cast<float4*>(Gd + pi * ldg + k4);
                float4 g = accumulate ? *gp : make_float4(0.f, 0.f, 0.f, 0.f);
                const float f = POOL ? 0.25f : 1.0f;
                const float d0 = (fmaf(xv.x, sk.x, tk.x) > 0.f) ? f * da[0] : 0.f;
                const float d1 = (fmaf(xv.y, sk.y, tk.y) > 0.f) ? f * da[1] : 0.f;
                const float d2 = (fmaf(xv.z, sk.z, tk.z) > 0.f) ? f * da[2] : 0.f;
                const float d3 = (fmaf(xv.w, sk.w, tk.w) > 0.f) ? f * da[3] : 0.f;
                g.x = fmaf(sk.x, d0, g.x);
                g.y = fmaf(sk.y, d1, g.y);
                g.z = fmaf(sk.z, d2, g.z);
                g.w = fmaf(sk.w, d3, g.w);
                *gp = g;
                l1[0] += d0;
                l1[1] += d1;
                l1[2] += d2;
                l1[3] += d3;
                l2[0] = fmaf(d0, (xv.x - mu.x) * is.x, l2[0]);
                l2[1] = fmaf(d1, (xv.y - mu.y) * is.y, l2[1]);
                l2[2] = fmaf(d2, (xv.z - mu.z) * is.z, l2[2]);
                l2[3] = fmaf(d3, (xv.w - mu.w) * is.w, l2[3]);
              }
            }
          }
#pragma unroll
          for (int g = 0; g < 4; ++g) {
            l1[g] = eml::row16_sum(l1[g]);
            l2[g] = eml::row16_sum(l2[g]);
            if (r == 0) {
              my[2 * (k4 + g)] += (double)l1[g];
              my[2 * (k4 + g) + 1] += (double)l2[g];
            }
          }
        }
      }
    }
  }
  __syncthreads();
  for (int e = tid; e < Kp * 2; e += 256)
    partials[(size_t)blockIdx.x * Kp * 2 + e] =
        (sacc[e] + sacc[(size_t)Kp * 2 + e]) + (sacc[(size_t)2 * Kp * 2 + e] + sacc[(size_t)3 * Kp * 2 + e]);
}

template <int MT, int NCH, bool ACC , bool MASKED = false, int NJO = 0>
__global__ __launch_bounds__(256, 2) void transition_bwd_data_kernel(
    const float* __restrict__ DY, int ld_dy, const float* __restrict__ Zr, int ld_z, const float* __restrict__ cA,
    const float* __restrict__ cB, const float* __restrict__ cC, int Ko, const float* __restrict__ Wd,
    const float* __restrict__ X, int ldx, const float* __restrict__ scale1, const float* __restrict__ shift1,
    const float* __restrict__ mean, const float* __restrict__ istd, int P, int Hin, int Win, int Kp,
    float* __restrict__ Gd, int ldg, double* __restrict__ partials ,
    const unsigned short* __restrict__ mask16) {
  extern __shared__ __attribute__((aligned(16))) float smem[];
  double* sacc = reinterpret_cast<double*>(smem);
  float* vec_l = reinterpret_cast<float*>(sacc + (size_t)4 * Kp * 2);
  float* co_l = vec_l + 4 * Kp;
  float* stg = co_l + 3 * Ko + (size_t)(threadIdx.x >> 6) * 16 * 36;
  const int tid = threadIdx.x, lane = tid & 63, wave = tid >> 6;
  const int r = lane & 15, kk = lane >> 4;
  for (int e = tid; e < 4 * Kp * 2; e += 256) sacc[e] = 0.0;
  for (int e = tid; e < Kp; e += 256) {
    vec_l[e] = scale1[e];
    vec_l[Kp + e] = shift1[e];
    vec_l[2 * Kp + e] = MASKED ? 0.f : mean[e];
    vec_l[3 * Kp + e] = MASKED ? 0.f : istd[e];
  }
  for (int e = tid; e < Ko; e += 256) {
    co_l[e] = cA[e];
    co_l[Ko + e] = cB[e];
    co_l[2 * Ko + e] = cC[e];
  }
  __syncthreads();
  double* my = sacc + (size_t)wave * Kp * 2;
  const int nnt = Kp >> 4, njo = Ko >> 4;
  constexpr int TP = 64 * MT;
  const int ntiles = (P + TP - 1) / TP;
  const int Wo = Win >> 1, Ho = Hin >> 1;

  for (int tile = blockIdx.x; tile < ntiles; tile += gridDim.x) {
    const int p0 = tile * TP + wave * 16 * MT;
    long prow[MT];
    size_t pin[MT];
    bool pv[MT];
#pragma unroll
    for (int m = 0; m < MT; ++m) {
      pv[m] = p0 + 16 * m + r < P;
      prow[m] = min(p0 + 16 * m + r, P - 1);
      const int b = (int)(prow[m] / (Ho * Wo)), rem = (int)(prow[m] - (long)b * (Ho * Wo));
      const int oy = rem / Wo, ox = rem - oy * Wo;
      pin[m] = (size_t)(b * Hin + 2 * oy) * Win + 2 * ox;
    }
    size_t pinx[MT][2];
    bool pvx[MT][2];
    if constexpr (MASKED && !ACC) {
#pragma unroll
      for (int m = 0; m < MT; ++m)
#pragma unroll
        for (int h = 0; h < 2; ++h) {
          const int src = (lane >> 3) + 8 * h;
          pinx[m][h] = (size_t)__shfl((unsigned long long)pin[m], src, 64);
          pvx[m][h] = __shfl((int)pv[m], src, 64) != 0;
        }
    }
    float4 dzr[NJO > 0 ? NJO : 1][MT];
    if constexpr (NJO > 0) {
#pragma unroll
      for (int jo = 0; jo < NJO; ++jo) {
        const int ch = 16 * jo + 4 * kk;
        const float4 a4 = *reinterpret_cast<const float4*>(co_l + ch);
        const float4 b4 = *reinterpret_cast<const float4*>(co_l + Ko + ch);
        const float4 c4 = *reinterpret_cast<const float4*>(co_l + 2 * Ko + ch);
#pragma unroll
        for (int m = 0; m < MT; ++m) {
          const float4 y4 = *reinterpret_cast<const float4*>(DY + prow[m] * ld_dy + ch);
          const float4 z4 = *reinterpret_cast<const float4*>(Zr + prow[m] * ld_z + ch);
          dzr[jo][m].x = fmaf(a4.x, y4.x, fmaf(b4.x, z4.x, c4.x));
          dzr[jo][m].y = fmaf(a4.y, y4.y, fmaf(b4.y, z4.y, c4.y));
          dzr[jo][m].z = fmaf(a4.z, y4.z, fmaf(b4.z, z4.z, c4.z));
          dzr[jo][m].w = fmaf(a4.w, y4.w, fmaf(b4.w, z4.w, c4.w));
        }
      }
    }
    for (int nt0 = 0; nt0 < nnt; nt0 += NCH) {
      float4 xv[MASKED ? 1 : MT][MASKED ? 1 : NCH][4], gs[ACC ? MT : 1][ACC ? NCH : 1][4];
      unsigned mk[MT][NCH];
#pragma unroll
      for (int n = 0; n < NCH; ++n) {
        const int k4 = 16 * min(nt0 + n, nnt - 1) + 4 * kk;
#pragma unroll
        for (int m = 0; m < MT; ++m) {
          if constexpr (MASKED) mk[m][n] = mask16[(size_t)prow[m] * (Kp >> 2) + (k4 >> 2)];
#pragma unroll
          for (int sub = 0; sub < 4; ++sub) {
            const size_t pi = pin[m] + (sub >> 1) * (size_t)Win + (sub & 1);
            if constexpr (!MASKED) xv[m][n][sub] = *reinterpret_cast<const float4*>(X + pi * ldx + k4);
            if constexpr (ACC) gs[m][n][sub] = *reinterpret_cast<const float4*>(Gd + pi * ldg + k4);
          }
        }
      }
      f32x4 acc[MT][NCH];
#pragma unroll
      for (int m = 0; m < MT; ++m)
#pragma unroll
        for (int n = 0; n < NCH; ++n) acc[m][n] = f32x4{0.f, 0.f, 0.f, 0.f};
      float4 ry[MT], rz[MT], wq[NCH];
      auto load_group = [&](int jo) {
        const int ch = 16 * jo + 4 * kk;
        if constexpr (NJO == 0) {
#pragma unroll
          for (int m = 0; m < MT; ++m) {
            ry[m] = *reinterpret_cast<const float4*>(DY + prow[m] * ld_dy + ch);
            rz[m] = *reinterpret_cast<const float4*>(Zr + prow[m] * ld_z + ch);
          }
        }
#pragma unroll
        for (int n = 0; n < NCH; ++n) {
          const int nt = min(nt0 + n, nnt - 1);
          wq[n] = *reinterpret_cast<const float4*>(Wd + ((((size_t)nt * njo + jo) * 4 + kk) * 16 + r) * 4);
        }
      };
      load_group(0);
      auto group_step = [&](int jo, const float4 (&dz)[MT]) {
        float4 wc[NCH];
#pragma unroll
        for (int n = 0; n < NCH; ++n) wc[n] = wq[n];
        load_group(min(jo + 1, njo - 1));
        __builtin_amdgcn_sched_barrier(0);
#pragma unroll
        for (int t = 0; t < 4; ++t)
#pragma unroll
          for (int n = 0; n < NCH; ++n)
#pragma unroll
            for (int m = 0; m < MT; ++m) acc[m][n] = mfma16(f4c(wc[n], t), f4c(dz[m], t), acc[m][n]);
      };
      if constexpr (NJO > 0) {
#pragma unroll
        for (int jo = 0; jo < NJO; ++jo) group_step(jo, dzr[jo]);
      } else {
        for (int jo = 0; jo < njo; ++jo) {
          const int ch = 16 * jo + 4 * kk;
          const float4 a4 = *reinterpret_cast<const float4*>(co_l + ch);
          const float4 b4 = *reinterpret_cast<const float4*>(co_l + Ko + ch);
          const float4 c4 = *reinterpret_cast<const float4*>(co_l + 2 * Ko + ch);
          float4 dz[MT];
#pragma unroll
// ... 643 lines not shown
  }
#pragma unroll
  for (int g = 0; g < 4; ++g) {
    red[wave][lane][2 * g] = live ? a1[g] : 0.0;
    red[wave][lane][2 * g + 1] = live ? a2[g] : 0.0;
  }
  __syncthreads();
  for (int e = tid; e < C * 2; e += 256) {
    const int c = e >> 1, k = e & 1, q = c >> 2, g = c & 3;
    double t = 0.0;
    for (int w = 0; w < 4; ++w)
      for (int sl = 0; sl < PW; ++sl) t += red[w][sl * CQ + q][2 * g + k];
    partials[(size_t)blockIdx.x * C * 2 + e] = t;
  }
}

template <bool FUSED>
__global__ __launch_bounds__(256) void conv0_bwd_weight_kernel(
    const float* __restrict__ x, const float* __restrict__ Gd, int ldg, const float* __restrict__ X1, int ldx,
    const float* __restrict__ Y0, int C0, const float* __restrict__ cA, const float* __restrict__ cB,
    const float* __restrict__ cC, int B, int H, int W, float* __restrict__ partial ,
    const float* __restrict__ scale0, const float* __restrict__ shift0, const float* __restrict__ sB,
    const float* __restrict__ sC) {
  const int tid = threadIdx.x, lane = tid & 63, wave = tid >> 6;
  const int r = lane & 15, kk = lane >> 4;
  f32x4 acc[2][2];
#pragma unroll
  for (int i = 0; i < 2; ++i)
#pragma unroll
    for (int n = 0; n < 2; ++n) acc[i][n] = f32x4{0.f, 0.f, 0.f, 0.f};
  float ca[2], cb[2], cc[2], fs0[2] = {0.f, 0.f}, ft0[2] = {0.f, 0.f}, fb[2] = {0.f, 0.f}, fc[2] = {0.f, 0.f};
  bool ov[2];
#pragma unroll
  for (int n = 0; n < 2; ++n) {
    ov[n] = 16 * n + r < C0;
    ca[n] = ov[n] ? cA[16 * n + r] : 0.f;
    cb[n] = ov[n] ? cB[16 * n + r] : 0.f;
    cc[n] = ov[n] ? cC[16 * n + r] : 0.f;
    if constexpr (FUSED) {
      fs0[n] = ov[n] ? scale0[16 * n + r] : 0.f;
      ft0[n] = ov[n] ? shift0[16 * n + r] : 0.f;
      fb[n] = ov[n] ? sB[16 * n + r] : 0.f;
      fc[n] = ov[n] ? sC[16 * n + r] : 0.f;
    }
  }
  int ci[2], dyi[2], dxi[2];
  bool iv[2];
#pragma unroll
  for (int i = 0; i < 2; ++i) {
    const int t = 16 * i + r;
    iv[i] = t < 27;
    ci[i] = iv[i] ? t / 9 : 0;
    dyi[i] = iv[i] ? (t % 9) / 3 - 1 : 0;
    dxi[i] = iv[i] ? (t % 3) - 1 : 0;
  }
  const size_t P = (size_t)B * H * W, plane = (size_t)H * W;
  const size_t nq = (P + 3) >> 2;
  constexpr int kU = 4;
  for (size_t q0 = ((size_t)blockIdx.x * 4 + wave) * kU; q0 < nq; q0 += (size_t)gridDim.x * 4 * kU) {
    float av[kU][2], gv[kU][2], xv[kU][2], yv[kU][2];
    bool pvu[kU], inb[kU][2];
#pragma unroll
    for (int u = 0; u < kU; ++u) {
      const size_t p = 4 * (q0 + u) + kk;
      pvu[u] = p < P;
      const size_t pc = pvu[u] ? p : P - 1;
      const int b = (int)(pc / plane), rem = (int)(pc - (size_t)b * plane);
      const int yy = rem / W, xx = rem - yy * W;
#pragma unroll
      for (int i = 0; i < 2; ++i) {
        const int gy = yy + dyi[i], gx = xx + dxi[i];
        inb[u][i] = pvu[u] && iv[i] && gy >= 0 && gy < H && gx >= 0 && gx < W;
        const int gyc = min(max(gy, 0), H - 1), gxc = min(max(gx, 0), W - 1);
        av[u][i] = x[((size_t)(b * 3 + ci[i]) * H + gyc) * W + gxc];
      }
#pragma unroll
      for (int n = 0; n < 2; ++n) {
        const int o = ov[n] ? 16 * n + r : 0;
        gv[u][n] = Gd[pc * ldg + o];
        if constexpr (!FUSED) xv[u][n] = X1[pc * ldx + o];
        yv[u][n] = Y0[pc * C0 + o];
      }
    }
#pragma unroll
    for (int u = 0; u < kU; ++u) {
      float a[2], d[2];
#pragma unroll
      for (int i = 0; i < 2; ++i) a[i] = inb[u][i] ? av[u][i] : 0.f;
#pragma unroll
      for (int n = 0; n < 2; ++n) {
        float g;
        if constexpr (FUSED) {
          const float xx = fmaxf(fmaf(yv[u][n], fs0[n], ft0[n]), 0.f);
          g = xx > 0.f ? gv[u][n] + fmaf(fb[n], xx, fc[n]) : 0.f;
        } else {
          g = xv[u][n] > 0.f ? gv[u][n] : 0.f;
        }
        const float v = fmaf(ca[n], g, fmaf(cb[n], yv[u][n], cc[n]));
        d[n] = (pvu[u] && ov[n]) ? v : 0.f;
      }
#pragma unroll
      for (int i = 0; i < 2; ++i)
#pragma unroll
        for (int n = 0; n < 2; ++n) acc[i][n] = mfma16(a[i], d[n], acc[i][n]);
    }
  }
  float* out = partial + ((size_t)blockIdx.x * 4 + wave) * 1024;
#pragma unroll
  for (int i = 0; i < 2; ++i)
#pragma unroll
    for (int n = 0; n < 2; ++n)
#pragma unroll
      for (int g = 0; g < 4; ++g) out[(16 * i + 4 * kk + g) * 32 + 16 * n + r] = acc[i][n][g];
}

constexpr int kC0dTH = 8, kC0dTW = 32, kC0dC = 24;
constexpr int kC0dHW = kC0dTW + 2, kC0dNP = (kC0dTH + 2) * kC0dHW;
constexpr int kC0dLd = 28;
constexpr int kC0dPP = 256 / (kC0dC / 4);
constexpr int kC0dPasses = (kC0dNP + kC0dPP - 1) / kC0dPP;

template <bool FUSED>
__global__ __launch_bounds__(256) void conv0_bwd_data_kernel(
    const float* __restrict__ Gd, int ldg, const float* __restrict__ X1, int ldx, const float* __restrict__ Y0,
    const float* __restrict__ scale0, const float* __restrict__ shift0, const float* __restrict__ sB,
    const float* __restrict__ sC, const float* __restrict__ cA, const float* __restrict__ cB, const float* __restrict__ cC,
    const float* __restrict__ W0, int B, int H, int W, float* __restrict__ dX) {
  __shared__ __attribute__((aligned(16))) float dz[kC0dNP * kC0dLd];
  __shared__ __attribute__((aligned(16))) float wl[9 * 3 * kC0dC];
  const int tid = threadIdx.x;
  for (int e = tid; e < kC0dC * 27; e += 256) wl[((e % 9) * 3 + (e % 27) / 9) * kC0dC + e / 27] = W0[e];
  const int q = tid % (kC0dC / 4), s0 = tid / (kC0dC / 4);
  const bool stager = s0 < kC0dPP;
  const int o4 = 4 * q;
  const float4 ca = *reinterpret_cast<const float4*>(cA + o4), cb = *reinterpret_cast<const float4*>(cB + o4),
               cc = *reinterpret_cast<const float4*>(cC + o4);
  float4 fs0 = {0.f, 0.f, 0.f, 0.f}, ft0 = fs0, fb = fs0, fc = fs0;
  if constexpr (FUSED) {
    fs0 = *reinterpret_cast<const float4*>(scale0 + o4);
    ft0 = *reinterpret_cast<const float4*>(shift0 + o4);
    fb = *reinterpret_cast<const float4*>(sB + o4);
    fc = *reinterpret_cast<const float4*>(sC + o4);
  }
  const float cav[4] = {ca.x, ca.y, ca.z, ca.w}, cbv[4] = {cb.x, cb.y, cb.z, cb.w}, ccv[4] = {cc.x, cc.y, cc.z, cc.w};
  const float fsv[4] = {fs0.x, fs0.y, fs0.z, fs0.w}, ftv[4] = {ft0.x, ft0.y, ft0.z, ft0.w};
  const float fbv[4] = {fb.x, fb.y, fb.z, fb.w}, fcv[4] = {fc.x, fc.y, fc.z, fc.w};
  const int ty = tid / kC0dTW, tx = tid % kC0dTW;
  const int tiles_x = (W + kC0dTW - 1) / kC0dTW, tiles_y = (H + kC0dTH - 1) / kC0dTH;
  const size_t plane = (size_t)H * W;
  {
    const int b = (int)(blockIdx.x / (tiles_y * tiles_x));
    const int r = (int)(blockIdx.x - b * tiles_y * tiles_x);
    const int h0 = (r / tiles_x) * kC0dTH, w0 = (r % tiles_x) * kC0dTW;
    float4 gv[kC0dPasses], yv[kC0dPasses], xv[kC0dPasses];
    bool in[kC0dPasses];
#pragma unroll
    for (int k = 0; k < kC0dPasses; ++k) {
      const int s = s0 + k * kC0dPP;
      const int hy = h0 - 1 + s / kC0dHW, hx = w0 - 1 + s % kC0dHW;
      in[k] = stager && s < kC0dNP && hy >= 0 && hy < H && hx >= 0 && hx < W;
      const size_t p = (size_t)b * plane + (size_t)(in[k] ? hy : 0) * W + (in[k] ? hx : 0);
      gv[k] = in[k] ? *reinterpret_cast<const float4*>(Gd + p * ldg + o4) : float4{0.f, 0.f, 0.f, 0.f};
      yv[k] = in[k] ? *reinterpret_cast<const float4*>(Y0 + p * kC0dC + o4) : float4{0.f, 0.f, 0.f, 0.f};
      if constexpr (!FUSED) xv[k] = in[k] ? *reinterpret_cast<const float4*>(X1 + p * ldx + o4) : float4{0.f, 0.f, 0.f, 0.f};
    }
#pragma unroll
    for (int k = 0; k < kC0dPasses; ++k) {
      const int s = s0 + k * kC0dPP;
      if (!stager || s >= kC0dNP) continue;
      const float g4[4] = {gv[k].x, gv[k].y, gv[k].z, gv[k].w}, y4[4] = {yv[k].x, yv[k].y, yv[k].z, yv[k].w};
      float d[4];
#pragma unroll
      for (int e = 0; e < 4; ++e) {
        float g;
        if constexpr (FUSED) {
          const float xx = fmaxf(fmaf(y4[e], fsv[e], ftv[e]), 0.f);
          g = xx > 0.f ? g4[e] + fmaf(fbv[e], xx, fcv[e]) : 0.f;
        } else {
          const float x4[4] = {xv[k].x, xv[k].y, xv[k].z, xv[k].w};
          g = x4[e] > 0.f ? g4[e] : 0.f;
        }
        d[e] = in[k] ? fmaf(cav[e], g, fmaf(cbv[e], y4[e], ccv[e])) : 0.f;
      }
      *reinterpret_cast<float4*>(&dz[s * kC0dLd + o4]) = float4{d[0], d[1], d[2], d[3]};
    }
    __syncthreads();
    float acc[3] = {0.f, 0.f, 0.f};
#pragma unroll
    for (int ky = 0; ky < 3; ++ky)
#pragma unroll
      for (int kx = 0; kx < 3; ++kx) {
        const float* src = &dz[((ty + 2 - ky) * kC0dHW + (tx + 2 - kx)) * kC0dLd];
        const float* wt = &wl[(ky * 3 + kx) * 3 * kC0dC];
#pragma unroll
        for (int o4i = 0; o4i < kC0dC / 4; ++o4i) {
          const float4 v = *reinterpret_cast<const float4*>(src + 4 * o4i);
          const float vv[4] = {v.x, v.y, v.z, v.w};
#pragma unroll
          for (int c = 0; c < 3; ++c) {
            const float4 wq = *reinterpret_cast<const float4*>(wt + c * kC0dC + 4 * o4i);
            const float ww[4] = {wq.x, wq.y, wq.z, wq.w};
#pragma unroll
            for (int e = 0; e < 4; ++e) acc[c] = fmaf(ww[e], vv[e], acc[c]);
          }
        }
      }
    const int h = h0 + ty, w = w0 + tx;
    if (h < H && w < W) {
#pragma unroll
      for (int c = 0; c < 3; ++c) dX[((size_t)b * 3 + c) * plane + (size_t)h * W + w] = acc[c];
    }
  }
}

__global__ __launch_bounds__(256) void head_pool_bwd_kernel(const float* __restrict__ gp, const float* __restrict__ F,
                                                            int ldf, int C, int B, int H, int W, int k,
                                                            float* __restrict__ dF, int ldd) {
  const int Ho = H / k, Wo = W / k;
  const size_t total = (size_t)B * H * W * C;
  const float inv = 1.0f / (float)(k * k);
  for (size_t e = (size_t)blockIdx.x * 256 + threadIdx.x; e < total; e += (size_t)gridDim.x * 256) {
    const int c = (int)(e % C);
    const size_t p = e / C;
    const int xx = (int)(p % W);
    const size_t rest = p / W;
    const int yy = (int)(rest % H), b = (int)(rest / H);
    const int oy = yy / k, ox = xx / k;
    float v = 0.f;
    if (oy < Ho && ox < Wo && F[p * ldf + c] > 0.f) v = gp[(((size_t)b * C + c) * Ho + oy) * Wo + ox] * inv;
    dF[p * ldd + c] = v;
  }
}

}

__global__ __launch_bounds__(256) void bn_dgamma_direct_partial_kernel(
    const float* __restrict__ X, int ldx, long P, int Hin, int Win, int pool, const float* __restrict__ DY, int ld_dy,
    const float* __restrict__ Zr, int ld_z, const float* __restrict__ cA, const float* __restrict__ cB,
    const float* __restrict__ cC, int Cout, const float* __restrict__ W, int Cin, const float* __restrict__ scale1,
    const float* __restrict__ shift1, const float* __restrict__ mean, const float* __restrict__ istd,
    const int* __restrict__ cond, double* __restrict__ partial) {
  __shared__ int list[384];
  __shared__ int cnt;
  __shared__ float wcol[192], co[3][192];
  __shared__ double red[4];
  const int tid = threadIdx.x;
  if (tid == 0) cnt = 0;
  __syncthreads();
  for (int c = tid; c < Cin; c += 256)
    if (cond[c]) list[atomicAdd(&cnt, 1)] = c;
  __syncthreads();
  const int n = cnt;
  if (n == 0) return;
  for (int o = tid; o < Cout; o += 256) {
    co[0][o] = Zr ? cA[o] : 1.f;
    co[1][o] = Zr ? cB[o] : 0.f;
    co[2][o] = Zr ? cC[o] : 0.f;
  }
  const long per = (P + gridDim.x - 1) / gridDim.x, p_lo = (long)blockIdx.x * per, p_hi = min(P, p_lo + per);
  const int Ho = Hin >> 1, Wo = Win >> 1;
  for (int li = 0; li < n; ++li) {
    const int c = list[li];
    __syncthreads();
    for (int o = tid; o < Cout; o += 256) wcol[o] = W[(size_t)o * Cin + c];
    __syncthreads();
    const float s1 = scale1[c], t1 = shift1[c];
    const double mu = mean[c], is = istd[c];
    double acc = 0.0;
    for (long p = p_lo + tid; p < p_hi; p += 256) {
      const float x = X[(size_t)p * ldx + c];
      if (fmaf(x, s1, t1) > 0.f) {
        long pp = p;
        if (pool) {
          const long b = p / ((long)Hin * Win), rem = p - b * (long)Hin * Win;
          const int y = (int)(rem / Win), xx = (int)(rem - (long)y * Win);
          pp = (b * Ho + (y >> 1)) * Wo + (xx >> 1);
        }
        const float* dy = DY + (size_t)pp * ld_dy;
        const float* zr = Zr ? Zr + (size_t)pp * ld_z : dy;
        double d = 0.0;
        for (int o = 0; o < Cout; ++o) d += (double)wcol[o] * (double)fmaf(co[0][o], dy[o], fmaf(co[1][o], zr[o], co[2][o]));
        if (pool) d *= 0.25;
        acc += d * (((double)x - mu) * is);
      }
    }
#pragma unroll
    for (int o = 32; o > 0; o >>= 1) acc += shfl_xor_d(acc, o);
    if ((tid & 63) == 0) red[tid >> 6] = acc;
    __syncthreads();
    if (tid == 0) partial[(size_t)blockIdx.x * Cin + c] = (red[0] + red[1]) + (red[2] + red[3]);
  }
}

__global__ __launch_bounds__(256) void bn_dgamma_direct_reduce_kernel(const double* __restrict__ partial, int R, int Cin,
                                                                      const int* __restrict__ cond,
                                                                      float* __restrict__ dgamma) {
  const int c = blockIdx.x * 256 + threadIdx.x;
  if (c >= Cin || !cond[c]) return;
  double s = 0.0;
  for (int g = 0; g < R; ++g) s += partial[(size_t)g * Cin + c];
  dgamma[c] = (float)s;
}

extern "C" int eml_dense_conv3x3_bwd_data_f32(const float* G, int ldg, int c0, const float* W2, const float* Z,
                                              const float* zmean, const float* zistd, float* DZ, int B, int H, int W,
                                              double* partials, int grid, const float* X, int ldx, int cx,
                                              const float* sB, const float* sC, float* GF, eml_stream_t stream) {
  if (!G || !W2 || !Z || !zmean || !zistd || !DZ || !partials || B < 1 || H < 1 || W < 1 || grid < 1 || (c0 & 1) ||
      (ldg & 1))
    return eml::fail(EML_EINVAL, "eml_dense_conv3x3_bwd_data_f32: bad arguments");
  if (X) {
    if (!sB || !sC || !GF || (ldx & 1))
      return eml::fail(EML_EINVAL, "eml_dense_conv3x3_bwd_data_f32: fused affine needs X, sB, sC, GF");
    if (cx < 0 || (cx & 1)) return eml::fail(EML_EINVAL, "eml_dense_conv3x3_bwd_data_f32: cx must be even");
  }
  static const bool narrow = [] { const char* v = getenv("EML_D3_NARROW"); return v && v[0] == '1'; }();
  static const bool tall = [] { const char* v = getenv("EML_D3_SHORT"); return !(v && v[0] == '1'); }();
  const auto al16 = [](const void* q) { return (reinterpret_cast<uintptr_t>(q) & 15) == 0; };
  const bool wide = !narrow && (ldg & 3) == 0 && (c0 & 3) == 0 && al16(G) &&
                    (!X || ((ldx & 3) == 0 && (cx & 3) == 0 && al16(X) && al16(sB) && al16(sC) && al16(GF)));
#define EML_LAUNCH_D3(FUSEV, WIDEV, THV)                                                                                \
  hipLaunchKernelGGL((conv3x3_bwd_data_kernel<FUSEV, WIDEV, THV>), dim3(grid), dim3(THV * 64), 0, (hipStream_t)stream, G, ldg, \
                     c0, W2, Z, zmean, zistd, DZ, B, H, W, partials, X, ldx, cx, sB, sC, GF, eml::DropKey{})
  if (X) {
    if (tall) { if (wide) EML_LAUNCH_D3(true, true, 8); else EML_LAUNCH_D3(true, false, 8); }
    else      { EML_LAUNCH_D3(true, false, 4); }
  } else {
    if (tall) { if (wide) EML_LAUNCH_D3(false, true, 8); else EML_LAUNCH_D3(false, false, 8); }
    else      { if (wide) EML_LAUNCH_D3(false, true, 4); else EML_LAUNCH_D3(false, false, 4); }
  }
#undef EML_LAUNCH_D3
  return eml::check_launch("eml_dense_conv3x3_bwd_data_f32");
}

extern "C" int eml_dense_conv3x3_bwd_data_drop_f32(const float* G, int ldg, int c0, const float* W2, const float* Z,
                                                   const float* zmean, const float* zistd, float* DZ, int B, int H, int W,
                                                   double* partials, int grid, const float* X, int ldx, int cx,
                                                   const float* sB, const float* sC, float* GF, unsigned long long seed,
                                                   int layer, double p, eml_stream_t stream) {
  if (!G || !W2 || !Z || !zmean || !zistd || !DZ || !partials || B < 1 || H < 1 || W < 1 || grid < 1 || (c0 & 1) ||
      (ldg & 1))
    return eml::fail(EML_EINVAL, "eml_dense_conv3x3_bwd_data_drop_f32: bad arguments");
  if (!X || !sB || !sC || !GF || (ldx & 1))
    return eml::fail(EML_EINVAL, "eml_dense_conv3x3_bwd_data_drop_f32: fused affine needs X, sB, sC, GF");
  if (cx < 0 || (cx & 1)) return eml::fail(EML_EINVAL, "eml_dense_conv3x3_bwd_data_drop_f32: cx must be even");
  if (!(p >= 0.0 && p <= 1.0) || layer < 0)
    return eml::fail(EML_EINVAL, "eml_dense_conv3x3_bwd_data_drop_f32: p must be in [0, 1] and layer >= 0 (p = %g, layer = %d)", p,
                     layer);
  if ((long long)B * H * W > 0x7FFFFFFFll)
    return eml::fail(EML_EINVAL, "eml_dense_conv3x3_bwd_data_drop_f32: B*H*W must fit the 32-bit pixel counter");
  static const bool narrow = [] { const char* v = getenv("EML_D3_NARROW"); return v && v[0] == '1'; }();
  static const bool tall = [] { const char* v = getenv("EML_D3_SHORT"); return !(v && v[0] == '1'); }();
  const auto al16 = [](const void* q) { return (reinterpret_cast<uintptr_t>(q) & 15) == 0; };
  const bool wide = !narrow && (ldg & 3) == 0 && (c0 & 3) == 0 && al16(G) && (ldx & 3) == 0 && (cx & 3) == 0 && al16(X) &&
                    al16(sB) && al16(sC) && al16(GF);
  const eml::DropKey dk = eml_drop_key(seed, layer, p);
#define EML_LAUNCH_D3(WIDEV, THV)                                                                                       \
  hipLaunchKernelGGL((conv3x3_bwd_data_kernel<true, WIDEV, THV, true>), dim3(grid), dim3(THV * 64), 0, (hipStream_t)stream, G, \
                     ldg, c0, W2, Z, zmean, zistd, DZ, B, H, W, partials, X, ldx, cx, sB, sC, GF, dk)
  if (tall) { if (wide) EML_LAUNCH_D3(true, 8); else EML_LAUNCH_D3(false, 8); }
  else      { EML_LAUNCH_D3(false, 4); }
#undef EML_LAUNCH_D3
  return eml::check_launch("eml_dense_conv3x3_bwd_data_drop_f32");
}

extern "C" int eml_dense_conv3x3_bwd_weight_f32(const float* G, int ldg, int c0, const float* Z, const float* scale2,
                                                const float* shift2, int B, int H, int W, float* partial, float* dW2,
                                                int grid, eml_stream_t stream) {
  if (!G || !Z || !scale2 || !shift2 || !partial || !dW2 || B < 1 || H < 1 || W < 1 || grid < 1)
    return eml::fail(EML_EINVAL, "eml_dense_conv3x3_bwd_weight_f32: bad arguments");
  static const bool greg = [] { const char* v = getenv("EML_W3_GREG"); return v && v[0] == '1'; }();
  if (!greg && (ldg & 3) == 0 && (c0 & 3) == 0 && (reinterpret_cast<uintptr_t>(G) & 15) == 0) {
    const size_t lds = (size_t)(2 * kHH * kHW * kPSW + 2 * kGL) * sizeof(float);
    EML_ENSURE_LDS((&conv3x3_bwd_weight_kernel<true>), lds);
    hipLaunchKernelGGL(conv3x3_bwd_weight_kernel<true>, dim3(grid), dim3(kBW), lds, (hipStream_t)stream, G, ldg, c0, Z,
                       scale2, shift2, B, H, W, partial);
  } else {
    const size_t lds = (size_t)(2 * kHH * kHW * kPSW) * sizeof(float);
    EML_ENSURE_LDS((&conv3x3_bwd_weight_kernel<false>), lds);
    hipLaunchKernelGGL(conv3x3_bwd_weight_kernel<false>, dim3(grid), dim3(kBW), lds, (hipStream_t)stream, G, ldg, c0, Z,
                       scale2, shift2, B, H, W, partial);
  }
  int rc = eml::check_launch("eml_dense_conv3x3_bwd_weight_f32");
  if (rc) return rc;
  hipLaunchKernelGGL(reduce_rows_kernel, dim3(27 * 256 / 64), dim3(256), 0, (hipStream_t)stream, partial, 2 * grid,
                     (size_t)27 * 256, 1, 0, 0, 0, dW2);
  return eml::check_launch("eml_dense_conv3x3_bwd_weight_f32(reduce)");
}

#ifdef EML_STAMPS
extern "C" int eml_c3_read_stamps(unsigned long long* out, int reset) {
  if (hipMemcpyFromSymbol(out, HIP_SYMBOL(eml_c3_stamps), 8 * sizeof(unsigned long long)) != hipSuccess) return -1;
  if (reset) {
    const unsigned long long z[8] = {0};
    if (hipMemcpyToSymbol(HIP_SYMBOL(eml_c3_stamps), z, sizeof(z)) != hipSuccess) return -1;
  }
  return 0;
}
#endif
extern "C" int eml_dense_conv3x3_bwd_fused_supported(int ldg, int c0, int ldx, int cx) {
  return ((ldg & 1) == 0 && (c0 & 1) == 0 && (ldx & 1) == 0 && (cx & 1) == 0) ? 1 : 0;
}
template <bool DROP>
static int conv3x3_bwd_fused_launch(const char* name, const float* G, int ldg, int c0, const float* W2, const float* Z,
                                    const float* zmean, const float* zistd, float* DZ, int B, int H, int W, double* partials,
                                    int grid, const float* X, int ldx, int cx, const float* sB, const float* sC, float* GF,
                                    const float* scale2, const float* shift2, float* partialW, float* dW2, eml::DropKey dk,
                                    eml_stream_t stream) {
  if (!G || !W2 || !Z || !zmean || !zistd || !DZ || !partials || !X || !sB || !sC || !scale2 || !shift2 || !partialW ||
      !dW2 || B < 1 || H < 1 || W < 1 || grid < 1 || cx < 0)
    return eml::fail(EML_EINVAL, "%s: bad arguments", name);
  const auto al16 = [](const void* q) { return (reinterpret_cast<uintptr_t>(q) & 15) == 0; };
  if (!eml_dense_conv3x3_bwd_fused_supported(ldg, c0, ldx, cx) || !al16(G) || !al16(X) || !al16(GF) || !al16(Z) || !al16(scale2) ||
      !al16(shift2))
    return eml::fail(EML_EINVAL, "%s: needs even ldg, c0, ldx, cx and 16-byte aligned buffers", name);
  const bool a16 = (ldg & 3) == 0 && (c0 & 3) == 0 && (ldx & 3) == 0 && (cx & 3) == 0;
#ifndef EML_C3_WTP
#define EML_C3_WTP 1
#endif
#if EML_C3_WTP
  const size_t lds = (size_t)(2 * kHH * kHW * kPSG + 2 * kTH * kTW * 48 + 27 * 3 * 64 + 32) * sizeof(float) + 8 * 48 * 2 * sizeof(double);
  if (a16) {
    if (GF) {
      EML_ENSURE_LDS((&conv3x3_bwd_fused_tp_kernel<true, DROP, true>), lds);
      hipLaunchKernelGGL((conv3x3_bwd_fused_tp_kernel<true, DROP, true>), dim3(grid), dim3(512), lds, (hipStream_t)stream, G, ldg, c0, W2, Z,
                         zmean, zistd, DZ, B, H, W, partials, X, ldx, cx, sB, sC, GF, scale2, shift2, partialW, dk);
    } else {
      EML_ENSURE_LDS((&conv3x3_bwd_fused_tp_kernel<true, DROP, false>), lds);
      hipLaunchKernelGGL((conv3x3_bwd_fused_tp_kernel<true, DROP, false>), dim3(grid), dim3(512), lds, (hipStream_t)stream, G, ldg, c0, W2, Z,
                         zmean, zistd, DZ, B, H, W, partials, X, ldx, cx, sB, sC, GF, scale2, shift2, partialW, dk);
    }
  } else {
    if (GF) {
      EML_ENSURE_LDS((&conv3x3_bwd_fused_tp_kernel<false, DROP, true>), lds);
      hipLaunchKernelGGL((conv3x3_bwd_fused_tp_kernel<false, DROP, true>), dim3(grid), dim3(512), lds, (hipStream_t)stream, G, ldg, c0, W2, Z,
                         zmean, zistd, DZ, B, H, W, partials, X, ldx, cx, sB, sC, GF, scale2, shift2, partialW, dk);
    } else {
      EML_ENSURE_LDS((&conv3x3_bwd_fused_tp_kernel<false, DROP, false>), lds);
      hipLaunchKernelGGL((conv3x3_bwd_fused_tp_kernel<false, DROP, false>), dim3(grid), dim3(512), lds, (hipStream_t)stream, G, ldg, c0, W2, Z,
                         zmean, zistd, DZ, B, H, W, partials, X, ldx, cx, sB, sC, GF, scale2, shift2, partialW, dk);
    }
  }
  int rc = eml::check_launch(name);
  if (rc) return rc;
  hipLaunchKernelGGL(reduce_rows_kernel, dim3(21 * 256 / 64), dim3(256), 0, (hipStream_t)stream, partialW, grid,
                     (size_t)21 * 256, 3, 0, 0, 0, dW2);
  return eml::check_launch(DROP ? "eml_dense_conv3x3_bwd_fused_drop_f32(reduce)" : "eml_dense_conv3x3_bwd_fused_f32(reduce)");
#else
  const size_t lds = (size_t)(2 * kHH * kHW * kPSG + kHH * kHW * kPSW + 27 * 3 * 64 + 32) * sizeof(float) + 8 * 48 * 2 * sizeof(double);
  if (a16) {
    if (GF) {
      EML_ENSURE_LDS((&conv3x3_bwd_fused_kernel<true, DROP, true>), lds);
      hipLaunchKernelGGL((conv3x3_bwd_fused_kernel<true, DROP, true>), dim3(grid), dim3(512), lds, (hipStream_t)stream, G, ldg, c0, W2, Z, zmean,
                         zistd, DZ, B, H, W, partials, X, ldx, cx, sB, sC, GF, scale2, shift2, partialW, dk);
    } else {
      EML_ENSURE_LDS((&conv3x3_bwd_fused_kernel<true, DROP, false>), lds);
      hipLaunchKernelGGL((conv3x3_bwd_fused_kernel<true, DROP, false>), dim3(grid), dim3(512), lds, (hipStream_t)stream, G, ldg, c0, W2, Z, zmean,
                         zistd, DZ, B, H, W, partials, X, ldx, cx, sB, sC, GF, scale2, shift2, partialW, dk);
    }
  } else {
    if (GF) {
      EML_ENSURE_LDS((&conv3x3_bwd_fused_kernel<false, DROP, true>), lds);
      hipLaunchKernelGGL((conv3x3_bwd_fused_kernel<false, DROP, true>), dim3(grid), dim3(512), lds, (hipStream_t)stream, G, ldg, c0, W2, Z, zmean,
                         zistd, DZ, B, H, W, partials, X, ldx, cx, sB, sC, GF, scale2, shift2, partialW, dk);
    } else {
      EML_ENSURE_LDS((&conv3x3_bwd_fused_kernel<false, DROP, false>), lds);
      hipLaunchKernelGGL((conv3x3_bwd_fused_kernel<false, DROP, false>), dim3(grid), dim3(512), lds, (hipStream_t)stream, G, ldg, c0, W2, Z, zmean,
                         zistd, DZ, B, H, W, partials, X, ldx, cx, sB, sC, GF, scale2, shift2, partialW, dk);
    }
  }
  int rc = eml::check_launch(name);
  if (rc) return rc;
  hipLaunchKernelGGL(reduce_rows_kernel, dim3(27 * 256 / 64), dim3(256), 0, (hipStream_t)stream, partialW, 2 * grid,
                     (size_t)27 * 256, 1, 0, 0, 0, dW2);
  return eml::check_launch(DROP ? "eml_dense_conv3x3_bwd_fused_drop_f32(reduce)" : "eml_dense_conv3x3_bwd_fused_f32(reduce)");
#endif
}

extern "C" int eml_dense_conv3x3_bwd_fused_f32(const float* G, int ldg, int c0, const float* W2, const float* Z,
                                               const float* zmean, const float* zistd, float* DZ, int B, int H, int W,
                                               double* partials, int grid, const float* X, int ldx, int cx,
                                               const float* sB, const float* sC, float* GF, const float* scale2,
                                               const float* shift2, float* partialW, float* dW2, eml_stream_t stream) {
  return conv3x3_bwd_fused_launch<false>("eml_dense_conv3x3_bwd_fused_f32", G, ldg, c0, W2, Z, zmean, zistd, DZ, B, H, W, partials,
                                         grid, X, ldx, cx, sB, sC, GF, scale2, shift2, partialW, dW2, eml::DropKey{}, stream);
}

extern "C" int eml_dense_conv3x3_bwd_fused_drop_f32(const float* G, int ldg, int c0, const float* W2, const float* Z,
                                                    const float* zmean, const float* zistd, float* DZ, int B, int H, int W,
                                                    double* partials, int grid, const float* X, int ldx, int cx,
                                                    const float* sB, const float* sC, float* GF, const float* scale2,
                                                    const float* shift2, float* partialW, float* dW2, unsigned long long seed,
                                                    int layer, double p, eml_stream_t stream) {
  if (!(p >= 0.0 && p <= 1.0) || layer < 0)
    return eml::fail(EML_EINVAL, "eml_dense_conv3x3_bwd_fused_drop_f32: p must be in [0, 1] and layer >= 0 (p = %g, layer = %d)", p,
                     layer);
  if ((long long)B * H * W > 0x7FFFFFFFll)
    return eml::fail(EML_EINVAL, "eml_dense_conv3x3_bwd_fused_drop_f32: B*H*W must fit the 32-bit pixel counter");
  return conv3x3_bwd_fused_launch<true>("eml_dense_conv3x3_bwd_fused_drop_f32", G, ldg, c0, W2, Z, zmean, zistd, DZ, B, H, W,
                                        partials, grid, X, ldx, cx, sB, sC, GF, scale2, shift2, partialW, dW2,
                                        eml_drop_key(seed, layer, p), stream);
}

namespace {
__global__ __launch_bounds__(256) void dropout_mask_kernel(eml::DropKey dk, unsigned P, unsigned short* __restrict__ out) {
  for (unsigned q = blockIdx.x * 256u + threadIdx.x; q < P; q += gridDim.x * 256u) {
    unsigned m = 0;
#pragma unroll
    for (unsigned grp = 0; grp < 3; ++grp) {
      const uint4 d = eml::drop_draws(dk, q, grp);
#pragma unroll
      for (int w = 0; w < 4; ++w)
        if ((unsigned long long)eml::draw_word(d, w) >= dk.thr) m |= 1u << (4 * grp + w);
    }
    out[q] = (unsigned short)m;
  }
}
}

extern "C" int eml_dense_dropout_mask_u16(unsigned long long seed, int layer, double p, long P, unsigned short* mask,
                                          eml_stream_t stream) {
  if (!mask || P < 1 || P > 0x7FFFFFFFl || layer < 0 || !(p >= 0.0 && p <= 1.0))
    return eml::fail(EML_EINVAL, "eml_dense_dropout_mask_u16: bad arguments (mask null, P outside [1, 2^31), layer < 0 or p "
                                 "outside [0, 1])");
  const unsigned grid = (unsigned)std::min<long>((P + 255) / 256, 4096);
  hipLaunchKernelGGL(dropout_mask_kernel, dim3(grid), dim3(256), 0, (hipStream_t)stream, eml_drop_key(seed, layer, p), (unsigned)P,
                     mask);
  return eml::check_launch("eml_dense_dropout_mask_u16");
}

extern "C" int eml_dense_bn_bwd_finalize_f32(const double* partials, int R, int pstride, double count,
                                             const float* gamma, const float* mean, const float* istd, int C, int Cpad,
                                             int training, float* dgamma, float* dbeta, float* cA, float* cB,
                                             float* cC, float* sB, float* sC, int s_accumulate, int c_lo,
                                             int c_hi, const float* beta, const float* W, const float* dW, int w_rows,
                                             int* cond, int* any_cond, eml_stream_t stream) {
  if (!partials || !gamma || !mean || !istd || !dgamma || !dbeta || C < 1 || Cpad < C || R < 1 ||
      (cA && (!cB || !cC)) || (sB && !sC) || c_lo < 0 || c_hi <= c_lo)
    return eml::fail(EML_EINVAL, "eml_dense_bn_bwd_finalize_f32: bad arguments");
  if (W && (!dW || !beta || w_rows < 1))
    return eml::fail(EML_EINVAL, "eml_dense_bn_bwd_finalize_f32: W given without dW / beta / w_rows");
  if (c_hi > Cpad) c_hi = Cpad;
  hipLaunchKernelGGL(bn_bwd_finalize_kernel, dim3((c_hi - c_lo + 3) / 4), dim3(256), 0, (hipStream_t)stream, partials,
                     R, pstride, count, gamma, mean, istd, C, Cpad, training, dgamma, dbeta, cA, cB, cC, sB, sC,
                     s_accumulate, c_lo, c_hi, beta, W, dW, w_rows, W ? cond : nullptr, W ? any_cond : nullptr);
  return eml::check_launch("eml_dense_bn_bwd_finalize_f32");
}

extern "C" int eml_dense_bn_dgamma_direct_f32(const float* X, int ldx, long P, int Hin, int Win, int pool, const float* DY,
                                              int ld_dy, const float* Zr, int ld_z, const float* cA, const float* cB,
                                              const float* cC, int Cout, const float* W, int Cin, const float* scale1,
                                              const float* shift1, const float* mean, const float* istd, const int* cond,
                                              double* scratch, float* dgamma, int grid, eml_stream_t stream) {
  if (!X || !DY || !W || !scale1 || !shift1 || !mean || !istd || !cond || !scratch || !dgamma || P < 1 || grid < 1 ||
      Cin < 1 || Cin > 384 || Cout < 1 || Cout > 192 || Cin > ldx || Cout > ld_dy || (Zr && (!cA || !cB || !cC || Cout > ld_z)) ||
      (pool && ((Hin | Win) & 1)))
    return eml::fail(EML_EINVAL, "eml_dense_bn_dgamma_direct_f32: bad arguments (Cin <= 384, Cout <= 192, even maps when pooled)");
  hipLaunchKernelGGL(bn_dgamma_direct_partial_kernel, dim3(grid), dim3(256), 0, (hipStream_t)stream, X, ldx, P, Hin, Win,
                     pool, DY, ld_dy, Zr, ld_z, cA, cB, cC, Cout, W, Cin, scale1, shift1, mean, istd, cond, scratch);
  int rc = eml::check_launch("eml_dense_bn_dgamma_direct_f32(partial)");
  if (rc) return rc;
  hipLaunchKernelGGL(bn_dgamma_direct_reduce_kernel, dim3((Cin + 255) / 256), dim3(256), 0, (hipStream_t)stream, scratch,
                     grid, Cin, cond, dgamma);
  return eml::check_launch("eml_dense_bn_dgamma_direct_f32(reduce)");
}

extern "C" int eml_dense_conv1x1_bwd_weight_f32(const float* X, int ldx, long P, int Hin, int Win, int pool, int Kp,
                                                int Cin, const float* scale1, const float* shift1, const float* DY,
                                                int ld_dy, const float* Zr, int ld_z, const float* cA, const float* cB,
                                                const float* cC, int Cout, float* partial, float* dW, int grid,
                                                float* dz_out, const float* W1, int k_lo, const float* G, int ldg,
                                                float* N12, double* partials_n, eml_stream_t stream) {
  if (dz_out && (Cout != 48 || pool))
    return eml::fail(EML_EINVAL, "eml_dense_conv1x1_bwd_weight_f32: dz_out is for dense layers (Cout == 48, no pool)");
  if (N12 && (Cout != 48 || pool || !W1 || !G || !partials_n || k_lo < 0 || (k_lo & 1) || k_lo + 12 > Cin || (ldg & 1) ||
              (ldg != 12 && k_lo + 12 > ldg)))
    return eml::fail(EML_EINVAL, "eml_dense_conv1x1_bwd_weight_f32: fused narrow pass needs a dense layer, W1, G, partials_n "
                                 "and an even k_lo with k_lo + 12 <= Cin (k_lo=%d, Cin=%d)", k_lo, Cin);
  if (!X || !scale1 || !shift1 || !DY || !Zr || !cA || !cB || !cC || !partial || !dW || P < 1 || grid < 1 || Kp < 32 ||
      (Kp & 15) || Cin > Kp || Cout < 1)
    return eml::fail(EML_EINVAL, "eml_dense_conv1x1_bwd_weight_f32: bad arguments");
  const int nchunks = (Cout + 47) / 48;
  for (int ch = 0; ch < nchunks; ++ch) {
    const int n0 = ch * 48, nv = (Cout - n0 < 48) ? Cout - n0 : 48;
    int n_load = ((ld_dy < ld_z ? ld_dy : ld_z) - n0) & ~3;
    if (n_load > 48) n_load = 48;
    if (n_load < nv) return eml::fail(EML_EINVAL, "eml_dense_conv1x1_bwd_weight_f32: DY/Zr rows narrower than Cout");
    const NarrowArgs na{W1, G, N12, partials_n, Cin, k_lo, ldg};
    static const int vec_env = [] { const char* v = getenv("EML_W1_VEC"); return v ? atoi(v) : 0; }();
    const bool vec4 = !pool && (ldx & 3) == 0 && (reinterpret_cast<uintptr_t>(X) & 15) == 0 &&
                      vec_env == 4;
    if (vec4 && N12 && vec_env == 4)
      hipLaunchKernelGGL((conv1x1_bwd_weight_kernel<false, true, 4>), dim3(grid), dim3(256), 0, (hipStream_t)stream, X, ldx,
                         (int)P, Hin, Win, Kp, scale1, shift1, DY + n0, ld_dy, Zr + n0, ld_z, cA + n0, cB + n0, cC + n0,
                         nv, n_load, partial, dz_out, na);
    else if (vec4 && !N12)
      hipLaunchKernelGGL((conv1x1_bwd_weight_kernel<false, false, 4>), dim3(grid), dim3(256), 0, (hipStream_t)stream, X, ldx,
                         (int)P, Hin, Win, Kp, scale1, shift1, DY + n0, ld_dy, Zr + n0, ld_z, cA + n0, cB + n0, cC + n0,
                         nv, n_load, partial, dz_out, na);
    else if (pool)
      hipLaunchKernelGGL((conv1x1_bwd_weight_kernel<true, false>), dim3(grid), dim3(256), 0, (hipStream_t)stream, X, ldx,
                         (int)P, Hin, Win, Kp, scale1, shift1, DY + n0, ld_dy, Zr + n0, ld_z, cA + n0, cB + n0, cC + n0,
                         nv, n_load, partial, nullptr, na);
    else if (N12)
      hipLaunchKernelGGL((conv1x1_bwd_weight_kernel<false, true>), dim3(grid), dim3(256), 0, (hipStream_t)stream, X, ldx,
                         (int)P, Hin, Win, Kp, scale1, shift1, DY + n0, ld_dy, Zr + n0, ld_z, cA + n0, cB + n0, cC + n0,
                         nv, n_load, partial, dz_out, na);
    else
      hipLaunchKernelGGL((conv1x1_bwd_weight_kernel<false, false>), dim3(grid), dim3(256), 0, (hipStream_t)stream, X, ldx,
                         (int)P, Hin, Win, Kp, scale1, shift1, DY + n0, ld_dy, Zr + n0, ld_z, cA + n0, cB + n0, cC + n0,
                         nv, n_load, partial, dz_out, na);
    int rc = eml::check_launch("eml_dense_conv1x1_bwd_weight_f32");
    if (rc) return rc;
    hipLaunchKernelGGL(reduce_rows_kernel, dim3((Cin * 48 + 63) / 64), dim3(256), 0, (hipStream_t)stream, partial,
                       grid, (size_t)Kp * 48, 0, Cin, nv, n0, dW);
    rc = eml::check_launch("eml_dense_conv1x1_bwd_weight_f32(reduce)");
    if (rc) return rc;
  }
  return EML_OK;
}

extern "C" int eml_dense_permute_w1_bwd_f32(const float* W, int Cout, int Cin, int Kp, int Ko, float* Wd,
                                            eml_stream_t stream) {
  if (!W || !Wd || Cout < 1 || Cin < 1 || Kp < Cin || (Kp & 15) || Ko < Cout || (Ko & 15))
    return eml::fail(EML_EINVAL, "eml_dense_permute_w1_bwd_f32: bad arguments");
  hipLaunchKernelGGL(permute_w1_bwd_kernel, dim3(64), dim3(256), 0, (hipStream_t)stream, W, Cout, Cin, Kp, Ko, Wd);
  return eml::check_launch("eml_dense_permute_w1_bwd_f32");
}

extern "C" int eml_dense_conv1x1_bwd_data_f32(const float* DY, int ld_dy, const float* Zr, int ld_z, const float* cA,
                                              const float* cB, const float* cC, int Ko, const float* Wd,
                                              const float* X, int ldx, const float* scale1, const float* shift1,
                                              const float* mean, const float* istd, long P, int Hin, int Win, int pool,
                                              int Kp, float* G, int ldg, int accumulate, double* partials, int grid,
                                              const unsigned short* relu_mask16, eml_stream_t stream) {
  if (!DY || !Zr || !cA || !cB || !cC || !Wd || (!relu_mask16 && (!X || !mean || !istd)) || !scale1 || !shift1 || !G ||
      !partials || P < 1 || grid < 1 || (Kp & 15) || (Ko & 15) || Ko > ld_dy || Ko > ld_z || (ld_dy & 3) || (ld_z & 3) ||
      (ldx & 3) || (ldg & 3) || (!relu_mask16 && Kp > ldx) || Kp > ldg)
    return eml::fail(EML_EINVAL, "eml_dense_conv1x1_bwd_data_f32: bad arguments");
  if (relu_mask16 && !(pool && Ko != 48))
    return eml::fail(EML_EINVAL, "eml_dense_conv1x1_bwd_data_f32: relu_mask16 is for the transition form (pool, Ko != 48)");
  const size_t lds = (size_t)4 * Kp * 2 * sizeof(double);
#define EML_LAUNCH_BWD_DATA(POOLV, RESV, NCHV)                                                                        \
  hipLaunchKernelGGL((conv1x1_bwd_data_kernel<POOLV, RESV, NCHV>), dim3(grid), dim3(256), lds, (hipStream_t)stream, DY, \
                     ld_dy, Zr, ld_z, cA, cB, cC, Ko, Wd, X, ldx, scale1, shift1, mean, istd, (int)P, Hin, Win, Kp, G, \
                     ldg, accumulate, partials)
  if (pool) {
    if (Ko == 48) {
      EML_LAUNCH_BWD_DATA(true, true, 4);
    } else {
      const size_t lds_t = lds + (size_t)(4 * Kp + 3 * Ko + 4 * 16 * 36) * sizeof(float);
#define EML_LAUNCH_TRANSITION(ACCV, MSKV)                                                                              \
  do {                                                                                                                \
    EML_ENSURE_LDS((&transition_bwd_data_kernel<2, 2, ACCV, MSKV>), lds_t);                                 \
    hipLaunchKernelGGL((transition_bwd_data_kernel<2, 2, ACCV, MSKV>), dim3(grid), dim3(256), lds_t,                   \
                       (hipStream_t)stream, DY, ld_dy, Zr, ld_z, cA, cB, cC, Ko, Wd, X, ldx, scale1, shift1, mean, istd, \
                       (int)P, Hin, Win, Kp, G, ldg, partials, relu_mask16);                                           \
  } while (0)
#define EML_LAUNCH_TRANSITION_RES(NJOV)                                                                                \
  do {                                                                                                                \
    EML_ENSURE_LDS((&transition_bwd_data_kernel<2, 2, false, true, NJOV>), lds_t);                                     \
    hipLaunchKernelGGL((transition_bwd_data_kernel<2, 2, false, true, NJOV>), dim3(grid), dim3(256), lds_t,            \
                       (hipStream_t)stream, DY, ld_dy, Zr, ld_z, cA, cB, cC, Ko, Wd, X, ldx, scale1, shift1, mean, istd, \
                       (int)P, Hin, Win, Kp, G, ldg, partials, relu_mask16);                                           \
  } while (0)
      if (relu_mask16 && !accumulate && Ko == 112) EML_LAUNCH_TRANSITION_RES(7);
      else if (relu_mask16 && !accumulate && Ko == 160) EML_LAUNCH_TRANSITION_RES(10);
      else if (relu_mask16 && !accumulate && Ko == 176) EML_LAUNCH_TRANSITION_RES(11);
      else if (relu_mask16) {
        if (accumulate) EML_LAUNCH_TRANSITION(true, true); else EML_LAUNCH_TRANSITION(false, true);
      } else {
        if (accumulate) EML_LAUNCH_TRANSITION(true, false); else EML_LAUNCH_TRANSITION(false, false);
      }
#undef EML_LAUNCH_TRANSITION
#undef EML_LAUNCH_TRANSITION_RES
    }
  } else {
    if (Ko == 48) EML_LAUNCH_BWD_DATA(false, true, 2); else EML_LAUNCH_BWD_DATA(false, false, 4);
  }
#undef EML_LAUNCH_BWD_DATA
  return eml::check_launch("eml_dense_conv1x1_bwd_data_f32");
}

namespace {
int launch_bwd_data_multi(int n_layers, const float* const* DZ, const float* const* Zr, const float* const* cA,
                          const float* const* cB, const float* const* cC, const float* const* Wd,
                          const float* const* scale1, const float* const* shift1, double* const* partials, const int* Kp,
                          const float* X, int ldx, const float* mean, const float* istd, long P, int k_lo, int k_hi,
                          float* G, int ldg, int grid, const unsigned long long* const* relu_masks, float* top,
                          eml_stream_t stream) {
  if (top && (n_layers != 2 || !relu_masks || Zr || k_lo != 0 || k_hi < 24 || (k_hi & 3) || P * 12 > 2147483647L))
    return eml::fail(EML_EINVAL, "eml_dense_conv1x1_bwd_data_multi_top_f32: the compact top-24 output needs two layers, "
                                 "relu_masks, materialised dz, k_lo == 0 and k_hi >= 24, a multiple of 4 (k_hi=%d)", k_hi);
  if (n_layers < 1 || n_layers > 2 || !DZ || !Wd || !scale1 || !shift1 || !partials ||
      !Kp || (!relu_masks && (!X || !mean || !istd)) || !G || P < 1 || grid < 1 || k_lo < 0 || k_hi <= k_lo ||
      (ldx & 3) || (ldg & 3))
    return eml::fail(EML_EINVAL, "eml_dense_conv1x1_bwd_data_multi_f32: bad arguments");
  const bool raw = Zr == nullptr;
  if (!raw && (!cA || !cB || !cC))
    return eml::fail(EML_EINVAL, "eml_dense_conv1x1_bwd_data_multi_f32: Zr given without cA/cB/cC");
  if (relu_masks && !raw)
    return eml::fail(EML_EINVAL, "eml_dense_conv1x1_bwd_data_multi_f32: relu_masks needs the materialised dz (Zr == NULL)");
  BwdLayer L[2];
  const unsigned long long* Mk[2] = {nullptr, nullptr};
  int kmax = 0;
  for (int j = 0; j < 2; ++j) {
    const int s = j < n_layers ? j : 0;
    const unsigned long long* mk = relu_masks ? relu_masks[s] : nullptr;
    Mk[j] = mk;
    L[j] = raw ? BwdLayer{DZ[s], nullptr, nullptr, nullptr, nullptr, Wd[s], scale1[s], shift1[s], partials[s], Kp[s]}
               : BwdLayer{DZ[s], Zr[s], cA[s], cB[s], cC[s], Wd[s], scale1[s], shift1[s], partials[s], Kp[s]};
    if (!DZ[s] || (!raw && !Zr[s]) || !Wd[s] || !partials[s] || (relu_masks && !mk) || (Kp[s] & 15) ||
        (!relu_masks && Kp[s] > ldx) || Kp[s] > ldg)
      return eml::fail(EML_EINVAL, "eml_dense_conv1x1_bwd_data_multi_f32: bad layer %d", s);
    if (Kp[s] > kmax) kmax = Kp[s];
  }
  if (((k_hi + 15) & ~15) > kmax) return eml::fail(EML_EINVAL, "eml_dense_conv1x1_bwd_data_multi_f32: range beyond Kp");
  const size_t lds = (size_t)n_layers * 4 * kmax * 2 * sizeof(double) + (size_t)(2 + 2 * n_layers) * kmax * sizeof(float);
  if (lds > 80 * 1024) return eml::fail(EML_EINVAL, "eml_dense_conv1x1_bwd_data_multi_f32: Kp=%d does not fit LDS", kmax);
#define EML_LAUNCH_MULTI(NLV, MTV, RAWV, MSKV)                                                                       \
  do {                                                                                                              \
    EML_ENSURE_LDS((&conv1x1_bwd_data_multi_kernel<NLV, MTV, RAWV, MSKV>), lds);                                 \
    hipLaunchKernelGGL((conv1x1_bwd_data_multi_kernel<NLV, MTV, RAWV, MSKV>), dim3(grid), dim3(256), lds,            \
                       (hipStream_t)stream, L[0], L[1], X, ldx, mean, istd, (int)P, k_lo, k_hi, G, ldg, kmax,        \
                       Mk[0], Mk[1], (float*)nullptr);                                                              \
  } while (0)
  if (n_layers == 1) {
    if (relu_masks) EML_LAUNCH_MULTI(1, 4, true, true);
    else if (raw) EML_LAUNCH_MULTI(1, 4, true, false);
    else EML_LAUNCH_MULTI(1, 4, false, false);
  } else if (top) {
    EML_ENSURE_LDS((&conv1x1_bwd_data_multi_kernel<2, 2, true, true, true>), lds);
    hipLaunchKernelGGL((conv1x1_bwd_data_multi_kernel<2, 2, true, true, true>), dim3(grid), dim3(256), lds,
                       (hipStream_t)stream, L[0], L[1], X, ldx, mean, istd, (int)P, k_lo, k_hi, G, ldg, kmax, Mk[0], Mk[1],
                       top);
  } else {
    if (relu_masks) EML_LAUNCH_MULTI(2, 2, true, true);
    else if (raw) EML_LAUNCH_MULTI(2, 2, true, false);
    else EML_LAUNCH_MULTI(2, 2, false, false);
  }
#undef EML_LAUNCH_MULTI
  return eml::check_launch("eml_dense_conv1x1_bwd_data_multi_f32");
}
}

extern "C" int eml_dense_conv1x1_bwd_data_multi_f32(int n_layers, const float* const* DZ, const float* const* Zr,
                                                    const float* const* cA, const float* const* cB,
                                                    const float* const* cC, const float* const* Wd,
                                                    const float* const* scale1, const float* const* shift1,
                                                    double* const* partials, const int* Kp, const float* X, int ldx,
                                                    const float* mean, const float* istd, long P, int k_lo, int k_hi,
                                                    float* G, int ldg, int grid,
                                                    const unsigned long long* const* relu_masks, eml_stream_t stream) {
  return launch_bwd_data_multi(n_layers, DZ, Zr, cA, cB, cC, Wd, scale1, shift1, partials, Kp, X, ldx, mean, istd, P, k_lo,
                               k_hi, G, ldg, grid, relu_masks, nullptr, stream);
}

extern "C" int eml_dense_conv1x1_bwd_data_multi_top_f32(const float* const* DZ, const float* const* Wd,
                                                        const float* const* scale1, const float* const* shift1,
                                                        double* const* partials, const int* Kp, long P, int k_hi,
                                                        float* G, int ldg, int grid,
                                                        const unsigned long long* const* relu_masks, float* top,
                                                        eml_stream_t stream) {
  if (!top) return eml::fail(EML_EINVAL, "eml_dense_conv1x1_bwd_data_multi_top_f32: top is NULL");
  return launch_bwd_data_multi(2, DZ, nullptr, nullptr, nullptr, nullptr, Wd, scale1, shift1, partials, Kp, nullptr, 0,
                               nullptr, nullptr, P, 0, k_hi, G, ldg, grid, relu_masks, top, stream);
}

extern "C" int eml_dense_conv1x1_bwd_narrow_f32(const float* DZ, const float* W1, int Cin, int k_lo, const float* X,
                                                int ldx, const float* scale1, const float* shift1, const float* mean,
                                                const float* istd, long P, const float* G, int ldg, float* N12,
                                                double* partials, int Kp, int grid, eml_stream_t stream) {
  if (!DZ || !W1 || !X || !scale1 || !shift1 || !mean || !istd || !G || !N12 || !partials || P < 1 || grid < 1 ||
      k_lo < 0 || (k_lo & 1) || k_lo + 12 > Cin || Cin > Kp || (ldx & 1) || (ldg & 1) || Kp > ldx || Kp > ldg)
    return eml::fail(EML_EINVAL, "eml_dense_conv1x1_bwd_narrow_f32: bad arguments");
  hipLaunchKernelGGL((conv1x1_bwd_narrow_kernel<4>), dim3(grid), dim3(256), 0, (hipStream_t)stream, DZ, W1, Cin, k_lo, X,
                     ldx, scale1, shift1, mean, istd, (int)P, G, ldg, N12, partials, Kp);
  return eml::check_launch("eml_dense_conv1x1_bwd_narrow_f32");
}

extern "C" int eml_dense_grad_materialize_f32(float* G, int ldg, const float* X, int ldx, const float* sB,
                                              const float* sC, int c0, int n, long P, eml_stream_t stream) {
  if (!G || !X || !sB || !sC || P < 1 || n < 2 || (n & 1) || (c0 & 1) || (ldg & 1) || (ldx & 1))
    return eml::fail(EML_EINVAL, "eml_dense_grad_materialize_f32: bad arguments");
  const size_t total = (size_t)P * (n >> 1);
  const int grid = (int)((total + 255) / 256 < 8192 ? (total + 255) / 256 : 8192);
  hipLaunchKernelGGL(grad_materialize_kernel, dim3(grid), dim3(256), 0, (hipStream_t)stream, G, ldg, X, ldx, sB, sC, c0,
                     n, (size_t)P);
  return eml::check_launch("eml_dense_grad_materialize_f32");
}

extern "C" int eml_dense_bn_bwd_stats_f32(const float* DY, int ld_dy, const float* raw, int ld_raw, const float* out,
                                          int ld_out, int relu, int C, long P, const float* mean, const float* istd,
                                          double* partials, int grid, eml_stream_t stream) {
  if (!DY || !raw || !mean || !istd || !partials || (relu && !out) || C < 1 || C > 384 || P < 1 || grid < 1)
    return eml::fail(EML_EINVAL, "eml_dense_bn_bwd_stats_f32: bad arguments");
  auto a16 = [](const void* q) { return (reinterpret_cast<size_t>(q) & 15) == 0; };
  if (C <= 32 && (C & 3) == 0 && ((ld_dy | ld_raw | (relu ? ld_out : 0)) & 3) == 0 && a16(DY) && a16(raw) && (!relu || a16(out)) &&
      a16(mean) && a16(istd)) {
    hipLaunchKernelGGL(bn_bwd_stats_small_kernel, dim3(grid), dim3(256), 0, (hipStream_t)stream, DY, ld_dy, raw, ld_raw, out, ld_out,
                       relu, C, (size_t)P, mean, istd, partials);
    return eml::check_launch("eml_dense_bn_bwd_stats_f32");
  }
  const size_t lds = (size_t)4 * ((C + 63) / 64) * 64 * 2 * sizeof(double);
  hipLaunchKernelGGL(bn_bwd_stats_kernel, dim3(grid), dim3(256), lds, (hipStream_t)stream, DY, ld_dy, raw, ld_raw, out,
                     ld_out, relu, C, (size_t)P, mean, istd, partials);
  return eml::check_launch("eml_dense_bn_bwd_stats_f32");
}

extern "C" int eml_dense_conv0_bwd_weight_f32(const float* x, const float* G, int ldg, const float* X1, int ldx,
                                              const float* Y0, int C0, const float* cA, const float* cB,
                                              const float* cC, int B, int H, int W, float* partial, float* dW0,
                                              int grid, eml_stream_t stream) {
  if (!x || !G || !X1 || !Y0 || !cA || !cB || !cC || !partial || !dW0 || C0 < 1 || C0 > 32 || B < 1 || grid < 1)
    return eml::fail(EML_EINVAL, "eml_dense_conv0_bwd_weight_f32: bad arguments");
  hipLaunchKernelGGL(conv0_bwd_weight_kernel<false>, dim3(grid), dim3(256), 0, (hipStream_t)stream, x, G, ldg, X1, ldx, Y0, C0,
                     cA, cB, cC, B, H, W, partial, nullptr, nullptr, nullptr, nullptr);
  int rc = eml::check_launch("eml_dense_conv0_bwd_weight_f32");
  if (rc) return rc;
  hipLaunchKernelGGL(reduce_rows_kernel, dim3(27 * 32 / 64 + 1), dim3(256), 0, (hipStream_t)stream, partial, grid * 4,
                     (size_t)1024, 2, 0, C0, 0, dW0);
  return eml::check_launch("eml_dense_conv0_bwd_weight_f32(reduce)");
}

extern "C" int eml_dense_head_pool_bwd_f32(const float* gpooled, const float* F, int ldf, int C, int B, int H, int W,
                                           int k, float* dF, int ldd, eml_stream_t stream) {
  if (!gpooled || !F || !dF || C < 1 || B < 1 || k < 1) return eml::fail(EML_EINVAL, "eml_dense_head_pool_bwd_f32: bad arguments");
  const size_t total = (size_t)B * H * W * C;
  const int grid = (int)((total + 255) / 256 < 4096 ? (total + 255) / 256 : 4096);
  hipLaunchKernelGGL(head_pool_bwd_kernel, dim3(grid), dim3(256), 0, (hipStream_t)stream, gpooled, F, ldf, C, B, H, W, k,
                     dF, ldd);
  return eml::check_launch("eml_dense_head_pool_bwd_f32");
}

extern "C" int eml_dense_norm0_bwd_stats_f32(const float* G, int ldg, const float* Y0, int ld_y0, const float* scale0,
                                             const float* shift0, const float* sB, const float* sC, int C, long P,
                                             const float* mean, const float* istd, double* partials, int grid,
                                             eml_stream_t stream) {
  auto a16 = [](const void* q) { return (reinterpret_cast<size_t>(q) & 15) == 0; };
  if (!G || !Y0 || !scale0 || !shift0 || !sB || !sC || !mean || !istd || !partials || C < 4 || C > 32 || (C & 3) || P < 1 ||
      grid < 1 || ((ldg | ld_y0) & 3) || !a16(G) || !a16(Y0) || !a16(scale0) || !a16(shift0) || !a16(sB) || !a16(sC) || !a16(mean) ||
      !a16(istd))
    return eml::fail(EML_EINVAL, "eml_dense_norm0_bwd_stats_f32: bad arguments (C a multiple of 4 <= 32, 16-byte aligned operands)");
  hipLaunchKernelGGL(norm0_bwd_stats_kernel, dim3(grid), dim3(256), 0, (hipStream_t)stream, G, ldg, Y0, ld_y0, scale0, shift0, sB,
                     sC, C, (size_t)P, mean, istd, partials);
  return eml::check_launch("eml_dense_norm0_bwd_stats_f32");
}

extern "C" int eml_dense_conv0_bwd_weight_fused_f32(const float* x, const float* G, int ldg, const float* Y0, int C0,
                                                    const float* scale0, const float* shift0, const float* sB, const float* sC,
                                                    const float* cA, const float* cB, const float* cC, int B, int H, int W,
                                                    float* partial, float* dW0, int grid, eml_stream_t stream) {
  if (!x || !G || !Y0 || !scale0 || !shift0 || !sB || !sC || !cA || !cB || !cC || !partial || !dW0 || C0 < 1 || C0 > 32 || B < 1 ||
      grid < 1)
    return eml::fail(EML_EINVAL, "eml_dense_conv0_bwd_weight_fused_f32: bad arguments");
  hipLaunchKernelGGL(conv0_bwd_weight_kernel<true>, dim3(grid), dim3(256), 0, (hipStream_t)stream, x, G, ldg, nullptr, 0, Y0, C0, cA,
                     cB, cC, B, H, W, partial, scale0, shift0, sB, sC);
  int rc = eml::check_launch("eml_dense_conv0_bwd_weight_fused_f32");
  if (rc) return rc;
  hipLaunchKernelGGL(reduce_rows_kernel, dim3(27 * 32 / 64 + 1), dim3(256), 0, (hipStream_t)stream, partial, grid * 4,
                     (size_t)1024, 2, 0, C0, 0, dW0);
  return eml::check_launch("eml_dense_conv0_bwd_weight_fused_f32(reduce)");
}

extern "C" int eml_dense_conv0_bwd_data_f32(const float* G, int ldg, const float* X1, int ldx, const float* Y0, int C0,
                                            const float* scale0, const float* shift0, const float* sB, const float* sC,
                                            const float* cA, const float* cB, const float* cC, const float* W0, int B, int H,
                                            int W, float* dX, eml_stream_t stream) {
  auto a16 = [](const void* q) { return (reinterpret_cast<size_t>(q) & 15) == 0; };
  const bool fused = X1 == nullptr;
  if (!G || !Y0 || !cA || !cB || !cC || !W0 || !dX || (fused && (!scale0 || !shift0 || !sB || !sC)))
    return eml::fail(EML_EINVAL, "eml_dense_conv0_bwd_data_f32: null pointer");
  if (C0 != kC0dC || B < 1 || H < 1 || W < 1 || ldg < C0 || (ldg & 3) || (!fused && (ldx < C0 || (ldx & 3))))
    return eml::fail(EML_EINVAL, "eml_dense_conv0_bwd_data_f32: bad shape (C0 == 24, B, H, W >= 1, ldg / ldx >= 24 and multiples of 4)");
  if (!a16(G) || !a16(Y0) || (!fused && !a16(X1)) || !a16(cA) || !a16(cB) || !a16(cC) ||
      (fused && (!a16(scale0) || !a16(shift0) || !a16(sB) || !a16(sC))))
    return eml::fail(EML_EINVAL, "eml_dense_conv0_bwd_data_f32: G, X1, Y0 and the coefficient vectors must be 16-byte aligned");
  const size_t tiles = (size_t)B * ((H + kC0dTH - 1) / kC0dTH) * ((W + kC0dTW - 1) / kC0dTW);
  if (tiles > 0x7fffffff) return eml::fail(EML_EINVAL, "eml_dense_conv0_bwd_data_f32: more than 2^31 - 1 tiles of 8 x 32 pixels");
  const int grid = (int)tiles;
  if (fused)
    hipLaunchKernelGGL(conv0_bwd_data_kernel<true>, dim3(grid), dim3(256), 0, (hipStream_t)stream, G, ldg, nullptr, 0, Y0,
                       scale0, shift0, sB, sC, cA, cB, cC, W0, B, H, W, dX);
  else
    hipLaunchKernelGGL(conv0_bwd_data_kernel<false>, dim3(grid), dim3(256), 0, (hipStream_t)stream, G, ldg, X1, ldx, Y0,
                       nullptr, nullptr, nullptr, nullptr, cA, cB, cC, W0, B, H, W, dX);
  return eml::check_launch("eml_dense_conv0_bwd_data_f32");
}
```

include/emlight_hip.h:

```cpp
#ifndef EMLIGHT_HIP_H
#define EMLIGHT_HIP_H

#include <stddef.h>
#include <stdint.h>

#ifdef __cplusplus
extern "C" {
#endif

typedef void* eml_stream_t;

#define EML_OK 0
#define EML_EINVAL (-1)
#define EML_ELAUNCH (-2)

#define EML_MAX_EPS 64

#define EML_ABI_VERSION 31
int eml_abi_version(void);
const char* eml_last_error(void);

int eml_sg_rasterise_f32(const float* dirs, const float* sizes, const float* colors,
                         float* out, int B, int N, int H, int W, eml_stream_t stream);

#define EML_SG_EXHAUSTIVE 1
int eml_sg_rasterise_ex_f32(const float* dirs, const float* sizes, const float* colors, float* out,
                            int B, int N, int H, int W, int flags, unsigned long long* executed_exp,
                            eml_stream_t stream);

int eml_sg_rasterise_bwd_colors_f32(const float* dirs, const float* sizes, const float* gout,
                                    float* gcolors, int B, int N, int H, int W,
                                    eml_stream_t stream);
size_t eml_sg_rasterise_bwd_work_floats(int B, int N, int H, int W);
int eml_sg_rasterise_bwd_colors_ex_f32(const float* dirs, const float* sizes, const float* gout, float* gcolors, float* work,
                                       int B, int N, int H, int W, int flags, eml_stream_t stream);
size_t eml_sg_rasterise_bwd_full_work_floats(int B, int N, int H, int W);
int eml_sg_rasterise_bwd_f32(const float* dirs, const float* sizes, const float* colors, const float* gout, float* gdirs,
                             float* gsizes, float* gcolors, float* work, int B, int N, int H, int W, int flags,
                             eml_stream_t stream);

int eml_emd_anchor_cost_f32(const float* anchors, float* M, int N, eml_stream_t stream);

int eml_sinkhorn_schedule_f32(const float* x, const float* y, long n, double blur,
                              double scaling, int p, double diameter, const float* range_lo_hi,
                              float* eps_out, int* n_eps_out, float* diameter_out, eml_stream_t stream);

size_t eml_sinkhorn_work_floats(int B, int N);
int eml_sinkhorn_fwd_f32(const float* x, const float* y, const float* M, const float* Mt,
                         const float* alpha, const float* beta, double blur, double scaling, int p,
                         double diameter, const float* range_lo_hi, float* eps_out, int* n_eps_out,
                         float* diameter_out, float* loss, float* gx, float* gy, float* work, int B, int N,
                         eml_stream_t stream);

#define EML_SINKHORN_NO_SPLIT 1
#define EML_SINKHORN_FORCE_SPLIT 2
#define EML_SINKHORN_TEST_STALL 4
int eml_sinkhorn_fwd_ex_f32(const float* x, const float* y, const float* M, const float* Mt,
                            const float* alpha, const float* beta, double blur, double scaling, int p,
                            double diameter, const float* range_lo_hi, float* eps_out, int* n_eps_out,
                            float* diameter_out, float* loss, float* gx, float* gy, float* work, int B, int N,
                            int flags, eml_stream_t stream);

int eml_sinkhorn_fwd_rho_f32(const float* x, const float* y, const float* M, const float* Mt,
                             const float* alpha, const float* beta, double blur, double scaling, int p,
                             double diameter, const float* range_lo_hi, float* eps_out, int* n_eps_out,
                             float* diameter_out, float* loss, float* gx, float* gy, float* work, int B, int N,
                             int flags, double rho, float* lam_out, eml_stream_t stream);

int eml_sinkhorn_bwd_f32(const float* gloss, const float* gunit, float* gout, int B, int N,
                         eml_stream_t stream);

#define EML_SINKHORN_MAX_DIM 8
size_t eml_sinkhorn_dim_work_floats(int B, int N, int D);
int eml_sinkhorn_fwd_dim_f32(const float* x, const float* y, const float* M, const float* Mt,
                             const float* alpha, const float* beta, double blur, double scaling, int p,
                             double diameter, const float* range_lo_hi, float* eps_out, int* n_eps_out,
                             float* diameter_out, float* loss, float* gx, float* gy, float* work, int B, int N,
                             int D, int flags, double rho, float* lam_out, eml_stream_t stream);

int eml_sinkhorn_schedule_dim_f32(const float* x, const float* y, long n, int D, double blur, double scaling, int p,
                                  double diameter, const float* range_lo_hi, float* eps_out, int* n_eps_out,
                                  float* diameter_out, eml_stream_t stream);

int eml_sinkhorn_bwd_weights_f32(const float* gloss, const float* work, float* galpha, float* gbeta, int B, int N,
                                 eml_stream_t stream);



int eml_dense_conv0_fwd_f32(const float* x, const float* w0, float* X, int ldx, int B, int H, int W,
                            int C0, double* partials, int grid, eml_stream_t stream);
int eml_dense_conv0_fwd_mfma_f32(const float* x, const float* w0, float* X, int ldx, int B, int H, int W,
                                 int C0, double* partials, int grid, eml_stream_t stream);

int eml_dense_bn_apply_f32(const float* src, int ld_src, float* dst, int ld_dst, int C, long P,
                           const float* scale, const float* shift, int relu, double* partials,
                           int grid, eml_stream_t stream);

int eml_dense_bn_prepare_f32(const double* partials, int G, int pstride, int n_new, int c_new0,
                             double count, float* mean, float* var, float* istd, const float* gamma,
                             const float* beta, float* rmean, float* rvar, int C, int Cpad, float eps,
                             float momentum, int training, float* scale, float* shift,
                             eml_stream_t stream);

int eml_dense_permute_w1_f32(const float* W, int Cout, int Cin, int Kp, float* Wp, eml_stream_t stream);
int eml_dense_permute_w2_f32(const float* W2, int Cout, float* W2p, eml_stream_t stream);

typedef struct eml_permute_desc {
  const float* src;
  float* dst;
  int kind, Cout, Cin, Kp, Ko, reserved;
} eml_permute_desc;
int eml_dense_permute_batch_f32(const eml_permute_desc* descs, int n, eml_stream_t stream);

int eml_dense_conv1x1_fwd_f32(const float* X, int ldx, long P, int Hin, int Win, int pool, int Kp,
                              const float* scale, const float* shift, const float* Wp, int Cout,
                              float* out, int ldo, double* partials, int grid,
                              unsigned long long* relu_mask, eml_stream_t stream);

int eml_dense_conv3x3_fwd_f32(const float* Z, const float* scale2, const float* shift2,
                              const float* W2p, float* X, int ldx, int c_out0, int B, int H, int W,
                              double* partials, int grid, eml_stream_t stream);

int eml_dense_permute_w2_tp_f32(const float* W2, float* W2t, eml_stream_t stream);
int eml_dense_conv3x3_fwd_tp_supported(int B, int H, int W);
int eml_dense_conv3x3_fwd_tp_f32(const float* Z, const float* scale2, const float* shift2,
                                 const float* W2t, float* X, int ldx, int c_out0, int B, int H, int W,
                                 int band_rows, double* partials, int grid, eml_stream_t stream);

int eml_dense_conv3x3_fwd_drop_f32(const float* Z, const float* scale2, const float* shift2,
                                   const float* W2p, float* X, int ldx, int c_out0, int B, int H, int W,
                                   double* partials, int grid, unsigned long long seed, int layer, double p,
                                   eml_stream_t stream);
int eml_dense_conv3x3_fwd_tp_drop_f32(const float* Z, const float* scale2, const float* shift2,
                                      const float* W2t, float* X, int ldx, int c_out0, int B, int H, int W,
                                      int band_rows, double* partials, int grid, unsigned long long seed, int layer,
                                      double p, eml_stream_t stream);
int eml_dense_dropout_mask_u16(unsigned long long seed, int layer, double p, long P, unsigned short* mask,
                               eml_stream_t stream);

int eml_dense_pool_act_f32(const float* X, int ldx, int B, int Hin, int Win, int Kp, const float* scale,
                           const float* shift, float* A, int lda, unsigned short* relu_mask16,
                           eml_stream_t stream);

int eml_dense_head_pool_fwd_f32(const float* F, int ldf, int C, int B, int H, int W, int k,
                                float* out, eml_stream_t stream);


int eml_dense_conv3x3_bwd_data_f32(const float* G, int ldg, int c0, const float* W2, const float* Z,
                                   const float* zmean, const float* zistd, float* DZ, int B, int H,
                                   int W, double* partials, int grid, const float* X, int ldx, int cx,
                                   const float* sB, const float* sC, float* GF, eml_stream_t stream);

int eml_dense_conv3x3_bwd_fused_supported(int ldg, int c0, int ldx, int cx);
int eml_dense_conv3x3_bwd_fused_f32(const float* G, int ldg, int c0, const float* W2, const float* Z,
                                    const float* zmean, const float* zistd, float* DZ, int B, int H, int W,
                                    double* partials, int grid, const float* X, int ldx, int cx,
                                    const float* sB, const float* sC, float* GF, const float* scale2,
                                    const float* shift2, float* partialW, float* dW2, eml_stream_t stream);

int eml_dense_conv3x3_bwd_data_drop_f32(const float* G, int ldg, int c0, const float* W2, const float* Z,
                                        const float* zmean, const float* zistd, float* DZ, int B, int H,
                                        int W, double* partials, int grid, const float* X, int ldx, int cx,
                                        const float* sB, const float* sC, float* GF, unsigned long long seed,
                                        int layer, double p, eml_stream_t stream);
int eml_dense_conv3x3_bwd_fused_drop_f32(const float* G, int ldg, int c0, const float* W2, const float* Z,
                                         const float* zmean, const float* zistd, float* DZ, int B, int H, int W,
                                         double* partials, int grid, const float* X, int ldx, int cx,
                                         const float* sB, const float* sC, float* GF, const float* scale2,
                                         const float* shift2, float* partialW, float* dW2, unsigned long long seed,
                                         int layer, double p, eml_stream_t stream);

int eml_dense_conv3x3_bwd_weight_f32(const float* G, int ldg, int c0, const float* Z,
                                     const float* scale2, const float* shift2, int B, int H, int W,
                                     float* partial, float* dW2, int grid, eml_stream_t stream);

int eml_dense_bn_bwd_finalize_f32(const double* partials, int R, int pstride, double count,
                                  const float* gamma, const float* mean, const float* istd, int C,
                                  int Cpad, int training, float* dgamma, float* dbeta, float* cA,
                                  float* cB, float* cC, float* sB, float* sC, int s_accumulate,
                                  int c_lo, int c_hi, const float* beta, const float* W, const float* dW,
                                  int w_rows, int* cond, int* any_cond, eml_stream_t stream);

int eml_dense_bn_dgamma_direct_f32(const float* X, int ldx, long P, int Hin, int Win, int pool,
                                   const float* DY, int ld_dy, const float* Zr, int ld_z, const float* cA,
                                   const float* cB, const float* cC, int Cout, const float* W, int Cin,
                                   const float* scale1, const float* shift1, const float* mean,
                                   const float* istd, const int* cond, double* scratch, float* dgamma,
                                   int grid, eml_stream_t stream);

int eml_dense_conv1x1_bwd_weight_f32(const float* X, int ldx, long P, int Hin, int Win, int pool,
                                     int Kp, int Cin, const float* scale1, const float* shift1,
                                     const float* DY, int ld_dy, const float* Zr, int ld_z,
                                     const float* cA, const float* cB, const float* cC, int Cout,
                                     float* partial, float* dW, int grid, float* dz_out,
                                     const float* W1, int k_lo, const float* G, int ldg, float* N12,
                                     double* partials_n, eml_stream_t stream);

int eml_dense_permute_w1_bwd_f32(const float* W, int Cout, int Cin, int Kp, int Ko, float* Wd,
                                 eml_stream_t stream);

int eml_dense_conv1x1_bwd_data_f32(const float* DY, int ld_dy, const float* Zr, int ld_z,
                                   const float* cA, const float* cB, const float* cC, int Ko,
                                   const float* Wd, const float* X, int ldx, const float* scale1,
                                   const float* shift1, const float* mean, const float* istd, long P,
                                   int Hin, int Win, int pool, int Kp, float* G, int ldg,
                                   int accumulate, double* partials, int grid,
                                   const unsigned short* relu_mask16, eml_stream_t stream);

int eml_dense_conv1x1_bwd_data_multi_f32(int n_layers, const float* const* DZ, const float* const* Zr,
                                         const float* const* cA, const float* const* cB,
                                         const float* const* cC, const float* const* Wd,
                                         const float* const* scale1, const float* const* shift1,
                                         double* const* partials, const int* Kp, const float* X, int ldx,
                                         const float* mean, const float* istd, long P, int k_lo,
                                         int k_hi, float* G, int ldg, int grid,
                                         const unsigned long long* const* relu_masks, eml_stream_t stream);

int eml_dense_conv1x1_bwd_data_multi_top_f32(const float* const* DZ, const float* const* Wd,
                                             const float* const* scale1, const float* const* shift1,
                                             double* const* partials, const int* Kp, long P, int k_hi, float* G,
                                             int ldg, int grid, const unsigned long long* const* relu_masks,
                                             float* top, eml_stream_t stream);

int eml_dense_conv1x1_bwd_narrow_f32(const float* DZ, const float* W1, int Cin, int k_lo, const float* X,
                                     int ldx, const float* scale1, const float* shift1,
                                     const float* mean, const float* istd, long P, const float* G, int ldg,
                                     float* N12, double* partials, int Kp, int grid, eml_stream_t stream);

int eml_dense_grad_materialize_f32(float* G, int ldg, const float* X, int ldx, const float* sB,
                                   const float* sC, int c0, int n, long P, eml_stream_t stream);

int eml_dense_bn_bwd_stats_f32(const float* DY, int ld_dy, const float* raw, int ld_raw,
                               const float* out, int ld_out, int relu, int C, long P,
                               const float* mean, const float* istd, double* partials, int grid,
                               eml_stream_t stream);

int eml_dense_conv0_bwd_weight_f32(const float* x, const float* G, int ldg, const float* X1, int ldx,
                                   const float* Y0, int C0, const float* cA, const float* cB,
                                   const float* cC, int B, int H, int W, float* partial, float* dW0,
                                   int grid, eml_stream_t stream);

int eml_dense_norm0_bwd_stats_f32(const float* G, int ldg, const float* Y0, int ld_y0, const float* scale0,
                                  const float* shift0, const float* sB, const float* sC, int C, long P,
                                  const float* mean, const float* istd, double* partials, int grid, eml_stream_t stream);
int eml_dense_conv0_bwd_weight_fused_f32(const float* x, const float* G, int ldg, const float* Y0, int C0,
                                         const float* scale0, const float* shift0, const float* sB, const float* sC,
                                         const float* cA, const float* cB, const float* cC, int B, int H, int W,
                                         float* partial, float* dW0, int grid, eml_stream_t stream);

int eml_dense_conv0_bwd_data_f32(const float* G, int ldg, const float* X1, int ldx, const float* Y0, int C0,
                                 const float* scale0, const float* shift0, const float* sB, const float* sC,
                                 const float* cA, const float* cB, const float* cC, const float* W0, int B, int H, int W,
                                 float* dX, eml_stream_t stream);

int eml_dense_head_pool_bwd_f32(const float* gpooled, const float* F, int ldf, int C, int B, int H,
                                int W, int k, float* dF, int ldd, eml_stream_t stream);


int eml_sphere_tap_table_f32(const float* grid, int H, int W, int Ho, int Wo, int* idx, float* wgt,
                             eml_stream_t stream);

int eml_sphere_im2col_f32(const float* X, const int* idx, const float* wgt, float* A9, int B, int HW,
                          int Po, int C, eml_stream_t stream);

int eml_sphere_col2im_f32(const float* dA9, const int* ptr, const int* src, const float* w, float* dX,
                          int B, int HW, int Po, int C, eml_stream_t stream);

int eml_sphere_conv_fwd_fused_f32(const float* X, const int* idx, const float* wgt, const float* W2,
                                  const float* bias, float* Y, int B, int HW, int Po, int C, int O, int ke,
                                  eml_stream_t stream);
#define EML_TAP_ROWSHARE 1
int eml_sphere_conv_fwd_fused_ex_f32(const float* X, const int* idx, const float* wgt, const float* W2,
                                     const float* bias, float* Y, int B, int HW, int Po, int C, int O, int ke,
                                     const float* residual, float act_slope, int table_flags, eml_stream_t stream);
int eml_sphere_conv_small_supported(int C, int O);
int eml_sphere_conv_small_fwd_f32(const float* X, const int* idx, const float* wgt, const float* W2, const float* bias,
                                  float* Y, int B, int HW, int Po, int C, int O, float act_slope, eml_stream_t stream);
size_t eml_sphere_conv_small_wgrad_partial_floats(int B, int Po, int C, int O);
int eml_sphere_conv_small_wgrad_f32(const float* X, const int* idx, const float* wgt, const float* dY, const float* Yact,
                                    float act_slope, float* partial, float* dW2, float* db, int B, int HW, int Po, int C,
                                    int O, eml_stream_t stream);
int eml_sphere_conv_small_da9_f32(const float* dY, const float* Yact, float act_slope, const float* W2, float* dA9, long M,
                                  int C, int O, eml_stream_t stream);
int eml_sphere_conv_narrow_supported(int C, int O);
int eml_sphere_conv_narrow_fwd_f32(const float* X, const int* idx, const float* wgt, const float* W2, const float* bias, float* Y,
                                   int B, int HW, int Po, int C, int O, eml_stream_t stream);
int eml_sphere_conv_narrow_dgrad_f32(const float* dY, const int* tidx, const float* twgt, int ke, const float* W2, float* dX, int B,
                                     int HW, int Po, int C, int O, eml_stream_t stream);
size_t eml_sphere_conv_narrow_wgrad_partial_floats(int B, int Po, int C, int O);
int eml_sphere_conv_narrow_wgrad_f32(const float* X, const int* idx, const float* wgt, const float* dY, float* partial, float* dW2,
                                     int B, int HW, int Po, int C, int O, eml_stream_t stream);

size_t eml_sphere_conv_narrow_scratch_floats(int B, int HW);
int eml_sphere_conv_narrow_fwd2_f32(const float* X, const int* idx, const float* wgt, const float* W2, const float* bias,
                                    float* Y, float* scratch, int B, int HW, int Po, int C, int O, eml_stream_t stream);
size_t eml_sphere_conv_narrow_wgrad2_partial_floats(int B, int HW, int C);
int eml_sphere_conv_narrow_wgrad2_f32(const float* X, const int* tidx, const float* twgt, int ke,
                                      const unsigned char* rowmax, const float* dY, float* scratch, float* partial, float* dW2, int B, int HW, int Po, int C, int O,
                                      eml_stream_t stream);
int eml_sphere_conv_narrow_dgrad2_f32(const float* dY, const int* tidx, const float* twgt, int ke,
                                      const unsigned char* rowmax, const float* W2, float* dX, float* scratch,
                                      int scratch_has_v, int B, int HW, int Po, int C, int O, eml_stream_t stream);
int eml_sphere_conv_dgrad_fused_f32(const float* dY, const int* tidx, const float* twgt, const unsigned char* rowmax,
                                    int ke, const float* W2t, float* dX, int B, int HW, int Po, int C, int O,
                                    int table_flags, eml_stream_t stream);
int eml_sphere_conv_lowres_variant(int C, int O, int Po, int fp_max);
int eml_sphere_conv_lowres_table_i32(const int* idx, const int* fp, int* lidx, int Po, int ke, eml_stream_t stream);
size_t eml_sphere_conv_lowres_partial_floats(long M, int O, int split);
int eml_sphere_conv_lowres_f32(const float* X, const int* lidx, const float* wgt, const unsigned char* rowmax, int ke,
                               const int* fp, int fp_max, const float* W2, const float* bias, float* Y, float* partial,
                               int split, int B, int HW, int Po, int C, int O, const float* residual, float act_slope,
                               eml_stream_t stream);
size_t eml_sphere_conv_wgrad_partial_floats(int C, int O, int split_k);
int eml_sphere_conv_wgrad_fused_f32(const float* X, const int* idx, const float* wgt, const float* dY,
                                    float* partial, float* dW2, int B, int HW, int Po, int C, int O,
                                    int split_k, eml_stream_t stream);

int eml_spade_modulate_fwd_f32(const float* xn, int ld_x, const float* gb, int ld_gb, float* y, int ld_y,
                               long rows, int C, float slope, eml_stream_t stream);
int eml_spade_modulate_bwd_f32(const float* gy, int ld_gy, const float* xn, int ld_x, const float* gb,
                               int ld_gb, float* dxn, int ld_dx, float* dgb, int ld_dgb, long rows, int C,
                               float slope, eml_stream_t stream);

int eml_bn_stats_f32(const float* x, int ld, long rows, int C, double* partials, int grid, eml_stream_t stream);
int eml_bn_fold_f64(const double* partials, int R, int n, double* sums, eml_stream_t stream);
int eml_bn_finalize_f32(const double* sums, int C, float eps, float momentum, float* mean, float* istd,
                        float* running_mean, float* running_var, eml_stream_t stream);
int eml_spade_norm_modulate_fwd_f32(const float* x, int ld_x, const float* gb, int ld_gb, float* y, int ld_y,
                                    long rows, int C, float slope, const float* mean, const float* istd,
                                    eml_stream_t stream);
int eml_bn_bwd_apply_f32(const float* dxn, int ld_d, const float* x, int ld_x, long rows, int C,
                         const float* mean, const float* istd, const double* sums, float* dx, int ld_o,
                         eml_stream_t stream);

int eml_spade_norm_modulate_up2_fwd_f32(const float* x_lo, const float* gb, float* y, int B, int H, int W, int C, float slope,
                                        const float* mean, const float* istd, eml_stream_t stream);
int eml_bn_bwd_apply_up2_f32(const float* dxn, const float* x_lo, int B, int H, int W, int C, const float* mean,
                             const float* istd, const double* sums, float* dx_lo, eml_stream_t stream);

int eml_spade_norm_modulate_bwd_cols_f32(const float* gy, const float* x, const float* gb, float* dxn, float* dgb, int B, int H,
                                         int W, int C, int up2, float slope, const float* mean, const float* istd,
                                         double* partials, int grid, eml_stream_t stream);

int eml_sphere_conv_spade_supported(int Cin, int Cn, long HW);
int eml_sphere_conv_spade_fwd_f32(const float* actv, const int* idx, const float* wgt, const float* W2r, const float* bias_r,
                                  const float* x, const float* mean, const float* istd, float* Y, float* gamma_out, int B, int H,
                                  int W, int Cin, int Cn, int up2, float act_slope, int table_flags, eml_stream_t stream);
int eml_spade_norm_modulate_bwd_y_f32(const float* gy, const float* x, const float* gamma, const float* y, float* dxn, float* dgb,
                                      int B, int H, int W, int C, int up2, float slope, const float* mean, const float* istd,
                                      double* partials, int grid, eml_stream_t stream);

size_t eml_spectral_norm_scratch_floats(int O, int C);
int eml_spectral_norm_w2_f32(const float* W, float* u, float* v, int iterate, float eps, float* W2, float* sigma,
                             float* uv_used, float* scratch, int O, int C, eml_stream_t stream);
int eml_spectral_norm_w2_bwd_f32(const float* dW2, const float* W2, const float* u_used, const float* v_used,
                                 const float* sigma, double* partial, float* dW, int O, int C, eml_stream_t stream);
int eml_spectral_norm_w2_batch_f32(int n, const float* const* W, float* const* u, float* const* v, int iterate, float eps,
                                   float* const* W2, float* const* sigma, float* const* uv_used, float* const* scratch,
                                   const int* O, const int* C, eml_stream_t stream);

int eml_spade_heads_w2_f32(const float* Wg, const float* Wb, const float* bg, const float* bb, float* W2, float* b2, int Cn,
                           int C, int reorder, eml_stream_t stream);

int eml_instance_norm_act_fwd_f32(const float* x, float* y, float* stats, int B, int HW, int C, int channels_last,
                                  float eps, float slope, eml_stream_t stream);
int eml_instance_norm_act_bwd_f32(const float* gy, const float* x, const float* stats, float* dx, int B, int HW, int C,
                                  int channels_last, float slope, eml_stream_t stream);

size_t eml_l1_pairs_partial_doubles(int npairs);
int eml_l1_pairs_fwd_f32(int npairs, const float* const* f, const float* const* r, const float* const* w, const long* rows,
                         const int* C, const float* scale, double* partial, float* out, eml_stream_t stream);
int eml_l1_pairs_bwd_f32(int npairs, const float* const* f, const float* const* r, const float* const* w, const long* rows,
                         const int* C, const float* scale, const float* gout, float* const* g, float* const* gzero,
                         const long* nzero, eml_stream_t stream);

size_t eml_colsum_partial_doubles(int cols);
int eml_colsum_f32(const float* x, long rows, int cols, double* partial, float* out, eml_stream_t stream);

int eml_gt_anchor_index_i32(const double* anchors, int N, int H, int W, int* idx, eml_stream_t stream);

int eml_gt_parametrise_f64(const float* hdr, const int* csr_ptr, const int* csr_pix, int B, int H, int W,
                           int N, double* maxv, double* sums, unsigned char* map, eml_stream_t stream);

int eml_pano_crop_f32(const void* pano, int is_u8, int B, int H, int W, int h, int w, double ratio, double fov_deg,
                      const double* fov_dev, double deg, const double* deg_dev, float* out, eml_stream_t stream);

int eml_pano_resize_area_f32(const float* pano, int B, int H, int W, int h, int w, double deg, const double* deg_dev,
                             float* out, eml_stream_t stream);

size_t eml_tonemap_work_floats(int B);
int eml_tonemap_f32(const float* img, int B, long n, int use_gamma, double gamma, double percentile, double max_mapping,
                    const float* alpha_in, int clip, float* P, float* out, int* n_out, float* stats, void* work,
                    eml_stream_t stream);

size_t eml_projector_targets_work_floats(int B, int h, int w);
int eml_projector_targets_f32(const float* small, const float* alpha, int B, int h, int w, float* warped, float* map,
                              float* work, eml_stream_t stream);

int eml_resize_bilinear_f32(const float* src, const float* alpha, int clip, int B, int C, int h, int w, int oh, int ow,
                            float* out, eml_stream_t stream);

#ifdef __cplusplus
}
#endif
#endif
```

Baseline: 566.9 images/s.

## Batch dgamma-direct over layer pairs and fuse last two transition wgrad chunks

Adds a multi-set dgamma-direct kernel so the two dense layers handled together in backward share one launch and one pass over the block input X, instead of two launches. Adds an NT template parameter to the conv1x1 weight-gradient kernel so the final two 48-column output chunks of a transition conv are processed in one pass over X, followed by a two-chunk reduction kernel. The intent is to cut repeated reads of large activations and kernel launch count. In exchange it uses a larger partial scratch buffer, holds more accumulator registers and LDS per block (possibly lowering occupancy), and adds new API entry points with scratch-size checks.

```diff
diff --git a/emlight_amd/RegressionNetwork/dense_engine_bwd.py b/emlight_amd/RegressionNetwork/dense_engine_bwd.py
--- a/emlight_amd/RegressionNetwork/dense_engine_bwd.py
+++ b/emlight_amd/RegressionNetwork/dense_engine_bwd.py
@@ -61,13 +61,16 @@
         self.permutes = None
         self.coef = torch.zeros(8, max(kp, ko), **f32)
         self.part2 = torch.zeros(2, g * kp * 2, dtype=torch.float64, device=dev)
-        self.partW = torch.empty(g * max(kp * 48, 2 * 27 * 256, 4 * 1024), **f32)
+        L = _lib.lib()
+        trans_w = max(int(L.eml_dense_conv1x1_bwd_weight_scratch_floats(g, blk["trans"]["Kp"], blk["trans"]["Cout"]))
+                      for blk in ws.blocks)
+        self.partW = torch.empty(max(g * max(kp * 48, 2 * 27 * 256, 4 * 1024), trans_w), **f32)
         i32 = dict(dtype=torch.int32, device=dev)
         self.cond = [[torch.zeros(lay["Kp"], **i32) for lay in blk["layers"]] for blk in ws.blocks]
         self.condT = [torch.zeros(blk["trans"]["Kp"], **i32) for blk in ws.blocks]
         self.any_ill = torch.zeros(1, **i32)
         self.dg_grid = 128
-        self.dg_scratch = torch.empty(self.dg_grid * kp, dtype=torch.float64, device=dev)
+        self.dg_scratch = torch.zeros(1 + 2 * self.dg_grid * kp, dtype=torch.float64, device=dev)
         self.side = None
         if enc.overlap_wgrad(dev):
             m = int(os.environ.get("EML_CU_SPLIT", 0))
@@ -147,18 +150,32 @@
     sB, sC = bw.coef[6], bw.coef[7]
 
     direct = knob_choice("EML_DGAMMA_DIRECT", "always", ("always", "never")) != "never"
+    dg_multi = knob_flag("EML_DGAMMA_MULTI", True)
+    trans_onepass = knob_flag("EML_TRANS_WGRAD_ONEPASS", True)
     c3_fold = knob_flag("EML_C3_FOLD", True)
     c3_gf = knob_flag("EML_C3_GF", False)
     bw.any_ill.zero_()
 
-    def dgamma_direct(blk, X_ld, Pin, Hin, Win, pool, DY, ld_dy, Zr, ld_z, co, Cout, conv, Cin, scale1, shift1, cond, bn):
+    def dgamma_direct(blk, X_ld, Pin, Hin, Win, pool, sets):
         if not direct:
             return
-        a, b, c = co if co is not None else (None, None, None)
-        _lib.check(L.eml_dense_bn_dgamma_direct_f32(
-            p(blk["X"]), X_ld, Pin, Hin, Win, pool, p(DY), ld_dy, p(Zr), ld_z, p(a), p(b), p(c), Cout, p(conv.weight), Cin,
-            p(scale1), p(shift1), p(blk["mean"]), p(blk["istd"]), p(cond), p(bw.dg_scratch), gr(bn.weight), bw.dg_grid, st),
-            "eml_dense_bn_dgamma_direct_f32")
+        if not dg_multi:
+            for DY, ld_dy, Zr, ld_z, co, Cout, conv, Cin, scale1, shift1, cond, bn in sets:
+                a, b, c = co if co is not None else (None, None, None)
+                _lib.check(L.eml_dense_bn_dgamma_direct_f32(
+                    p(blk["X"]), X_ld, Pin, Hin, Win, pool, p(DY), ld_dy, p(Zr), ld_z, p(a), p(b), p(c), Cout, p(conv.weight),
+                    Cin, p(scale1), p(shift1), p(blk["mean"]), p(blk["istd"]), p(cond), p(bw.dg_scratch[1:]), gr(bn.weight),
+                    bw.dg_grid, st), "eml_dense_bn_dgamma_direct_f32")
+            return
+        col = lambda k: [s_[k] for s_ in sets]
+        ints = lambda k: (ctypes.c_int * len(sets))(*col(k))
+        cos = [s_[4] if s_[4] is not None else (None, None, None) for s_ in sets]
+        _lib.check(L.eml_dense_bn_dgamma_direct_multi_f32(
+            len(sets), p(blk["X"]), X_ld, Pin, Hin, Win, pool, parr(col(0)), ints(1), parr(col(2)), ints(3),
+            parr([c_[0] for c_ in cos]), parr([c_[1] for c_ in cos]), parr([c_[2] for c_ in cos]), ints(5),
+            parr([s_[6].weight for s_ in sets]), ints(7), parr(col(8)), parr(col(9)), p(blk["mean"]), p(blk["istd"]),
+            parr(col(10)), p(bw.dg_scratch), parr([grads[id(s_[11].weight)] for s_ in sets]), bw.dg_grid, st),
+            "eml_dense_bn_dgamma_direct_multi_f32")
 
     def finalize(R, pstride, count, bn, mean, istd, C, Cpad, coef=0, s_acc=None, src=None, c_lo=0, c_hi=None, conv=None,
                  cond=None):
@@ -172,7 +189,7 @@
             "eml_dense_bn_bwd_finalize_f32")
 
     def parr(tensors):
-        return (ctypes.c_void_p * len(tensors))(*[t.data_ptr() for t in tensors])
+        return (ctypes.c_void_p * len(tensors))(*[t.data_ptr() if t is not None else None for t in tensors])
 
     def materialize(Gbuf, blk, c0, n):
         _lib.check(L.eml_dense_grad_materialize_f32(p(Gbuf), blk["ld"], p(blk["X"]), blk["ld"], p(sB), p(sC), c0, n,
@@ -197,18 +214,20 @@
         _lib.check(L.eml_dense_bn_bwd_stats_f32(p(dY), ld_dy, p(tr["T"]), Ko, None, 0, 0, cout, Pn, p(tr["tmean"]),
                                                 p(tr["tistd"]), p(part), Gb, st), "eml_dense_bn_bwd_stats_f32")
         finalize(Gb, 2 * cout, Pn, LN, tr["tmean"], tr["tistd"], cout, Ko, coef=0)
-        _lib.check(L.eml_dense_conv1x1_bwd_weight_f32(
+        partw_floats = (int(L.eml_dense_conv1x1_bwd_weight_scratch_floats(G, kpt, cout)) if trans_onepass
+                        else G * kpt * 48)
+        _lib.check(L.eml_dense_conv1x1_bwd_weight_ex_f32(
             p(tr["A"]), kpt, Pn, Hb // 2, Wb // 2, 0, kpt, ctot, p(tr["one"]), p(tr["zero"]), p(dY), ld_dy, p(tr["T"]),
-            Ko, p(cA), p(cB), p(cC), cout, p(bw.partW), gr(T.conv.weight), G, None, None, 0, None, 0, None, None, st),
-            "eml_dense_conv1x1_bwd_weight_f32")
+            Ko, p(cA), p(cB), p(cC), cout, p(bw.partW), gr(T.conv.weight), G, None, None, 0, None, 0, None, None,
+            partw_floats, st), "eml_dense_conv1x1_bwd_weight_ex_f32")
         _lib.check(L.eml_dense_conv1x1_bwd_data_f32(
             p(dY), ld_dy, p(tr["T"]), Ko, p(cA), p(cB), p(cC), Ko, p(bw.WdT[bi]), None, ld, p(tr["scale"]),
             p(tr["shift"]), None, None, Pn, Hb, Wb, 1, kpt, p(Gbuf), ld, 0, p(part), G, p(tr["mask16"]), st),
             "eml_dense_conv1x1_bwd_data_f32")
         finalize(G, 2 * kpt, P, T.norm, blk["mean"], blk["istd"], ctot, kpt, coef=None, s_acc=False, conv=T.conv,
                  cond=bw.condT[bi])
-        dgamma_direct(blk, ld, P, Hb, Wb, 1, dY, ld_dy, tr["T"], Ko, coefs[0], cout, T.conv, ctot, tr["scale"], tr["shift"],
-                      bw.condT[bi], T.norm)
+        dgamma_direct(blk, ld, P, Hb, Wb, 1, [(dY, ld_dy, tr["T"], Ko, coefs[0], cout, T.conv, ctot, tr["scale"], tr["shift"],
+                                               bw.condT[bi], T.norm)])
         def conv2_backward(l, slot, n12=False, narrow_lo=None, top=False):
             lay = blk["layers"][l]
             Lm = getattr(mod, "denselayer%d" % (l + 1))
@@ -281,10 +300,10 @@
             finalize(Gd if rows is None else rows, 2 * lay["Kp"], P, Lm.norm1, blk["mean"], blk["istd"], lay["Cin"], lay["Kp"], coef=None,
                      s_acc=True, src=bw.part2[slot], c_lo=c_lo, c_hi=c_hi, conv=Lm.conv1, cond=bw.cond[bi][l])
 
-        def bn1_direct(l, Lm, slot):
-            lay = blk["layers"][l]
-            dgamma_direct(blk, ld, P, Hb, Wb, 0, bw.DZ[slot], 48, None, 0, None, 48, Lm.conv1, lay["Cin"], lay["scale1"],
-                          lay["shift1"], bw.cond[bi][l], Lm.norm1)
+        def bn1_direct(*layers):
+            dgamma_direct(blk, ld, P, Hb, Wb, 0, [
+                (bw.DZ[slot], 48, None, 0, None, 48, Lm.conv1, blk["layers"][l]["Cin"], blk["layers"][l]["scale1"],
+                 blk["layers"][l]["shift1"], bw.cond[bi][l], Lm.norm1) for l, Lm, slot in layers])
 
         l = len(blk["layers"]) - 1
         have_top = False
@@ -301,14 +320,13 @@
                 have_top = to_top
                 bn1_finalize(la, Lma, 0, 0, cin_b)
                 bn1_finalize(lb, Lmb, 1, 0, blk["layers"][lb]["Kp"])
-                bn1_direct(la, Lma, 0)
-                bn1_direct(lb, Lmb, 1)
+                bn1_direct((la, Lma, 0), (lb, Lmb, 1))
                 l -= 2
             else:
                 Lm0 = conv2_backward(l, 0)
                 dgrad([l], [0], 0, blk["layers"][l]["Cin"])
                 bn1_finalize(l, Lm0, 0, 0, blk["layers"][l]["Kp"])
-                bn1_direct(l, Lm0, 0)
+                bn1_direct((l, Lm0, 0))
                 l -= 1
         c0b = blk["C0"]
         norm0_fused = bi == 0 and knob_flag("EML_NORM0_FUSED", True) and c0b % 4 == 0 and c0b <= 32
diff --git a/emlight_amd/_lib.py b/emlight_amd/_lib.py
--- a/emlight_amd/_lib.py
+++ b/emlight_amd/_lib.py
@@ -180,6 +180,14 @@
     "eml_dense_conv1x1_bwd_weight_f32": (_int, [_f32p, _int, ctypes.c_long, _int, _int, _int, _int, _int, _f32p,
                                                 _f32p, _f32p, _int, _f32p, _int, _f32p, _f32p, _f32p, _int, _f32p,
                                                 _f32p, _int, _f32p, _f32p, _int, _f32p, _int, _f32p, _f32p, _stream]),
+    "eml_dense_conv1x1_bwd_weight_scratch_floats": (ctypes.c_long, [_int, _int, _int]),
+    "eml_dense_conv1x1_bwd_weight_ex_f32": (_int, [_f32p, _int, ctypes.c_long, _int, _int, _int, _int, _int, _f32p,
+                                                   _f32p, _f32p, _int, _f32p, _int, _f32p, _f32p, _f32p, _int, _f32p,
+                                                   _f32p, _int, _f32p, _f32p, _int, _f32p, _int, _f32p, _f32p,
+                                                   ctypes.c_long, _stream]),
+    "eml_dense_bn_dgamma_direct_multi_f32": (_int, [_int, _f32p, _int, ctypes.c_long, _int, _int, _int] +
+                                                   [ctypes.c_void_p] * 12 + [_f32p, _f32p, ctypes.c_void_p, _f64p,
+                                                    ctypes.c_void_p, _int, _stream]),
     "eml_dense_conv1x1_bwd_narrow_f32": (_int, [_f32p, _f32p, _int, _int, _f32p, _int, _f32p, _f32p, _f32p, _f32p,
                                                 ctypes.c_long, _f32p, _int, _f32p, _f32p, _int, _int, _stream]),
     "eml_dense_permute_w1_bwd_f32": (_int, [_f32p, _int, _int, _int, _int, _f32p, _stream]),
diff --git a/emlight_amd/csrc/dense_bwd.hip b/emlight_amd/csrc/dense_bwd.hip
--- a/emlight_amd/csrc/dense_bwd.hip
+++ b/emlight_amd/csrc/dense_bwd.hip
@@ -1163,6 +1163,27 @@
   if (slice == 0 && valid) out[dst] = (float)((red[0][tid] + red[1][tid]) + (red[2][tid] + red[3][tid]));
 }
 
+__global__ __launch_bounds__(256) void reduce_rows_chunks_kernel(const float* __restrict__ partial, int R, size_t row_stride,
+                                                                 size_t chunk_stride, int dim0, int n_valid, int n0,
+                                                                 float* __restrict__ out) {
+  __shared__ double red[4][64];
+  const int c = blockIdx.y, dim1 = min(48, n_valid - 48 * c);
+  partial += (size_t)c * chunk_stride;
+  n0 += 48 * c;
+  const int tid = threadIdx.x, e = blockIdx.x * 64 + (tid & 63), slice = tid >> 6;
+  const int k = e / 48, o = e - 48 * k;
+  const bool valid = k < dim0 && o < dim1;
+  const size_t src = (size_t)e, dst = (size_t)(n0 + o) * dim0 + k;
+  double s = 0.0;
+  if (valid) {
+#pragma unroll 8
+    for (int r = slice; r < R; r += 4) s += (double)partial[(size_t)r * row_stride + src];
+  }
+  red[slice][tid & 63] = s;
+  __syncthreads();
+  if (slice == 0 && valid) out[dst] = (float)((red[0][tid] + red[1][tid]) + (red[2][tid] + red[3][tid]));
+}
+
 struct NarrowArgs {
   const float* W1;
   const float* G;
@@ -1170,7 +1191,7 @@
   double* partials;
   int Cin, k_lo, ldg;
 };
-template <bool POOL, bool NARROW = false, int VEC = 2>
+template <bool POOL, bool NARROW = false, int VEC = 2, int NT = 3>
 __global__ __launch_bounds__(256, (NARROW || VEC == 4) ? 2 : 1) void conv1x1_bwd_weight_kernel(
     const float* __restrict__ X, int ldx, int P, int Hin, int Win, int Kp, const float* __restrict__ scale1,
     const float* __restrict__ shift1, const float* __restrict__ DY, int ld_dy, const float* __restrict__ Zr,
@@ -1179,7 +1200,9 @@
     float* __restrict__ partial ,
     float* __restrict__ dz_out ,
     NarrowArgs na) {
-  __shared__ __attribute__((aligned(16))) float dz_l[2][64 * 48];
+  constexpr int NCH = (NT + 2) / 3;
+  static_assert(NT >= 3 && NT <= 9 && (NT == 3 || (!POOL && !NARROW && VEC == 2)), "several chunks: the plain variant only");
+  __shared__ __attribute__((aligned(16))) float dz_l[2][NCH * 64 * 48];
   const int tid = threadIdx.x, lane = tid & 63, wave = tid >> 6;
   const int r = lane & 15, kk = lane >> 4;
   static_assert(VEC == 2 || (VEC == 4 && !POOL), "float4 operand: dense layers only");
@@ -1213,16 +1236,17 @@
     }
   }
   const int spix = tid >> 2, sq = tid & 3;
-  __shared__ __attribute__((aligned(16))) float co_l[3 * 48];
+  __shared__ __attribute__((aligned(16))) float co_l[NCH * 3 * 48];
   __shared__ float wn_l[NARROW ? 12 * 64 : 1];
-  constexpr bool CO_LDS = NARROW || VEC == 4;
+  constexpr bool CO_LDS = NARROW || VEC == 4 || NCH > 1;
   float4 sa_r[CO_LDS ? 1 : 3], sb_r[CO_LDS ? 1 : 3], sc_r[CO_LDS ? 1 : 3];
   if constexpr (CO_LDS) {
-    if (tid < 48) {
+    if (tid < 48 * NCH) {
       const bool v = tid < n_valid;
-      co_l[tid] = v ? cA[tid] : 0.f;
-      co_l[48 + tid] = v ? cB[tid] : 0.f;
-      co_l[96 + tid] = v ? cC[tid] : 0.f;
+      const int c = tid / 48, o = tid - 48 * c;
+      co_l[c * 144 + o] = v ? cA[tid] : 0.f;
+      co_l[c * 144 + 48 + o] = v ? cB[tid] : 0.f;
+      co_l[c * 144 + 96 + o] = v ? cC[tid] : 0.f;
     }
   } else {
 #pragma unroll
@@ -1248,19 +1272,19 @@
     }
   }
   __syncthreads();
-  f32x4 acc[MAXG][VEC][3];
+  f32x4 acc[MAXG][VEC][NT];
 #pragma unroll
   for (int i = 0; i < MAXG; ++i)
 #pragma unroll
     for (int t = 0; t < VEC; ++t)
 #pragma unroll
-      for (int n = 0; n < 3; ++n) acc[i][t][n] = f32x4{0.f, 0.f, 0.f, 0.f};
+      for (int n = 0; n < NT; ++n) acc[i][t][n] = f32x4{0.f, 0.f, 0.f, 0.f};
 
   const int Wo = Win >> 1, Ho = Hin >> 1;
   const int nchunks = (P + 63) >> 6;
   const int ngw = (ngroups > wave) ? (ngroups - wave + 3) >> 2 : 0;
 
-  float4 rdy[3], rzr[3];
+  float4 rdy[NT], rzr[NT];
   bool rpv = false;
   int rp = 0;
   auto stage_load = [&](int chunk) {
@@ -1269,7 +1293,7 @@
     const size_t pc = rpv ? p : 0;
     rp = (int)pc;
 #pragma unroll
-    for (int j = 0; j < 3; ++j) {
+    for (int j = 0; j < NT; ++j) {
       const int col = 4 * (sq + 4 * j);
       const bool cv = col < n_load;
       rdy[j] = cv ? *reinterpret_cast<const float4*>(DY + pc * ld_dy + col) : make_float4(0.f, 0.f, 0.f, 0.f);
@@ -1278,13 +1302,13 @@
   };
   auto stage_write = [&](float* dzb) {
 #pragma unroll
-    for (int j = 0; j < 3; ++j) {
-      const int col = 4 * (sq + 4 * j);
+    for (int j = 0; j < NT; ++j) {
+      const int col = 4 * (sq + 4 * (j % 3));
       float4 sa, sb, sc;
       if constexpr (CO_LDS) {
-        sa = *reinterpret_cast<const float4*>(co_l + col);
-        sb = *reinterpret_cast<const float4*>(co_l + 48 + col);
-        sc = *reinterpret_cast<const float4*>(co_l + 96 + col);
+        sa = *reinterpret_cast<const float4*>(co_l + (j / 3) * 144 + col);
+        sb = *reinterpret_cast<const float4*>(co_l + (j / 3) * 144 + 48 + col);
+        sc = *reinterpret_cast<const float4*>(co_l + (j / 3) * 144 + 96 + col);
       } else {
         sa = sa_r[j];
         sb = sb_r[j];
@@ -1295,8 +1319,10 @@
       v.y = rpv ? fmaf(sa.y, rdy[j].y, fmaf(sb.y, rzr[j].y, sc.y)) : 0.f;
       v.z = rpv ? fmaf(sa.z, rdy[j].z, fmaf(sb.z, rzr[j].z, sc.z)) : 0.f;
       v.w = rpv ? fmaf(sa.w, rdy[j].w, fmaf(sb.w, rzr[j].w, sc.w)) : 0.f;
-      *reinterpret_cast<float4*>(dzb + spix * 48 + col) = v;
-      if (dz_out && rpv) *reinterpret_cast<float4*>(dz_out + (size_t)rp * 48 + col) = v;
+      *reinterpret_cast<float4*>(dzb + (j / 3) * (64 * 48) + spix * 48 + col) = v;
+      if constexpr (NCH == 1) {
+        if (dz_out && rpv) *reinterpret_cast<float4*>(dz_out + (size_t)rp * 48 + col) = v;
+      }
     }
   };
   auto chunk_loop = [&](auto ngw_c) {
@@ -1355,9 +1381,9 @@
         ng[1] = *reinterpret_cast<const float2*>(gs + 2);
       }
       if constexpr (NGW > 0) {
-        float bzq[2][3];
-#pragma unroll
-        for (int n = 0; n < 3; ++n) bzq[0][n] = dzb[kk * 48 + 16 * n + r];
+        float bzq[2][NT];
+#pragma unroll
+        for (int n = 0; n < NT; ++n) bzq[0][n] = dzb[(n / 3) * (64 * 48) + kk * 48 + 16 * (n % 3) + r];
 #pragma unroll
         for (int bi = 0; bi < NB; ++bi) {
           const int q0 = bi * UQ;
@@ -1370,12 +1396,13 @@
           for (int u = 0; u < UQ; ++u) {
             const int pl = 4 * (q0 + u) + kk;
             const bool pvu = chunk * 64 + pl < P;
-            float bz[3];
-#pragma unroll
-            for (int n = 0; n < 3; ++n) bz[n] = bzq[(q0 + u) & 1][n];
+            float bz[NT];
+#pragma unroll
+            for (int n = 0; n < NT; ++n) bz[n] = bzq[(q0 + u) & 1][n];
             if (q0 + u + 1 < 16) {
 #pragma unroll
-              for (int n = 0; n < 3; ++n) bzq[(q0 + u + 1) & 1][n] = dzb[(pl + 4) * 48 + 16 * n + r];
+              for (int n = 0; n < NT; ++n)
+                bzq[(q0 + u + 1) & 1][n] = dzb[(n / 3) * (64 * 48) + (pl + 4) * 48 + 16 * (n % 3) + r];
             }
 #pragma unroll
             for (int i = 0; i < NGW; ++i) {
@@ -1398,7 +1425,7 @@
                 if (!pvu) av[t] = 0.f;
               }
 #pragma unroll
-              for (int n = 0; n < 3; ++n)
+              for (int n = 0; n < NT; ++n)
 #pragma unroll
                 for (int t = 0; t < VEC; ++t) acc[i][t][n] = mfma16(av[t], bz[n], acc[i][t][n]);
             }
@@ -1433,6 +1460,7 @@
     default: chunk_loop(std::integral_constant<int, MAXG>{}); break;
   }
   float* out = partial + (size_t)blockIdx.x * Kp * 48;
+  const size_t chunk_stride = (size_t)gridDim.x * Kp * 48;
 #pragma unroll
   for (int i = 0; i < MAXG; ++i) {
     const int cg = wave + 4 * i;
@@ -1443,7 +1471,12 @@
         const int ch = GW * cg + VEC * (4 * kk + g) + t;
         if (cg < ngroups && ch < Kp) {
 #pragma unroll
-          for (int n = 0; n < 3; ++n) out[(size_t)ch * 48 + 16 * n + r] = acc[i][t][n][g];
+          for (int n = 0; n < NT; ++n) {
+            if constexpr (NCH == 1)
+              out[(size_t)ch * 48 + 16 * n + r] = acc[i][t][n][g];
+            else
+              out[(n / 3) * chunk_stride + (size_t)ch * 48 + 16 * (n % 3) + r] = acc[i][t][n][g];
+          }
         }
       }
   }
@@ -2693,6 +2726,105 @@
   dgamma[c] = (float)s;
 }
 
+struct DgammaSet {
+  const float *DY, *Zr, *cA, *cB, *cC, *W, *scale1, *shift1;
+  const int* cond;
+  float* dgamma;
+  int ld_dy, ld_z, Cout, Cin;
+};
+struct DgammaSets {
+  DgammaSet s[2];
+};
+__global__ __launch_bounds__(256) void bn_dgamma_direct_multi_kernel(const float* __restrict__ X, int ldx, long P, int Hin,
+                                                                     int Win, int pool, const float* __restrict__ mean,
+                                                                     const float* __restrict__ istd, int nsets,
+                                                                     DgammaSets sets, double* __restrict__ scratch) {
+  __shared__ int list[2][384];
+  __shared__ int cnt[2];
+  __shared__ int last_l;
+  __shared__ float wcol[192], co[3][192];
+  __shared__ double red[4];
+  const int tid = threadIdx.x;
+  if (tid < 2) cnt[tid] = 0;
+  __syncthreads();
+  for (int s = 0; s < nsets; ++s)
+    for (int c = tid; c < sets.s[s].Cin; c += 256)
+      if (sets.s[s].cond[c]) list[s][atomicAdd(&cnt[s], 1)] = c;
+  __syncthreads();
+  if (cnt[0] + cnt[1] == 0) return;
+  unsigned* counter = reinterpret_cast<unsigned*>(scratch);
+  double* part_s[2] = {scratch + 1, scratch + 1 + (size_t)gridDim.x * sets.s[0].Cin};
+  const long per = (P + gridDim.x - 1) / gridDim.x, p_lo = (long)blockIdx.x * per, p_hi = min(P, p_lo + per);
+  const int Ho = Hin >> 1, Wo = Win >> 1;
+  for (int s = 0; s < nsets; ++s) {
+    const int n = cnt[s];
+    if (n == 0) continue;
+    const DgammaSet& a = sets.s[s];
+    const float* __restrict__ DY = a.DY;
+    const float* __restrict__ Zr = a.Zr;
+    const float* __restrict__ W = a.W;
+    const int Cout = a.Cout, Cin = a.Cin, ld_dy = a.ld_dy, ld_z = a.ld_z;
+    __syncthreads();
+    for (int o = tid; o < Cout; o += 256) {
+      co[0][o] = Zr ? a.cA[o] : 1.f;
+      co[1][o] = Zr ? a.cB[o] : 0.f;
+      co[2][o] = Zr ? a.cC[o] : 0.f;
+    }
+    for (int li = 0; li < n; ++li) {
+      const int c = list[s][li];
+      __syncthreads();
+      for (int o = tid; o < Cout; o += 256) wcol[o] = W[(size_t)o * Cin + c];
+      __syncthreads();
+      const float s1 = a.scale1[c], t1 = a.shift1[c];
+      const double mu = mean[c], is = istd[c];
+      double acc = 0.0;
+      for (long p = p_lo + tid; p < p_hi; p += 256) {
+        const float x = X[(size_t)p * ldx + c];
+        if (fmaf(x, s1, t1) > 0.f) {
+          long pp = p;
+          if (pool) {
+            const long b = p / ((long)Hin * Win), rem = p - b * (long)Hin * Win;
+            const int y = (int)(rem / Win), xx = (int)(rem - (long)y * Win);
+            pp = (b * Ho + (y >> 1)) * Wo + (xx >> 1);
+          }
+          const float* dy = DY + (size_t)pp * ld_dy;
+          const float* zr = Zr ? Zr + (size_t)pp * ld_z : dy;
+          double d = 0.0;
+          for (int o = 0; o < Cout; ++o) d += (double)wcol[o] * (double)fmaf(co[0][o], dy[o], fmaf(co[1][o], zr[o], co[2][o]));
+          if (pool) d *= 0.25;
+          acc += d * (((double)x - mu) * is);
+        }
+      }
+#pragma unroll
+      for (int o = 32; o > 0; o >>= 1) acc += shfl_xor_d(acc, o);
+      if ((tid & 63) == 0) red[tid >> 6] = acc;
+      __syncthreads();
+      if (tid == 0) part_s[s][(size_t)blockIdx.x * Cin + c] = (red[0] + red[1]) + (red[2] + red[3]);
+    }
+  }
+  if (tid == 0) {
+    __threadfence();
+    asm volatile("s_waitcnt vmcnt(0)" ::: "memory");
+    const unsigned t = __hip_atomic_fetch_add(counter, 1u, __ATOMIC_ACQ_REL, __HIP_MEMORY_SCOPE_AGENT);
+    last_l = t == gridDim.x - 1;
+  }
+  __syncthreads();
+  if (!last_l) return;
+  __threadfence();
+  for (int s = 0; s < nsets; ++s) {
+    const int Cin = sets.s[s].Cin;
+    const unsigned long long* rows = reinterpret_cast<const unsigned long long*>(part_s[s]);
+    for (int li = tid; li < cnt[s]; li += 256) {
+      const int c = list[s][li];
+      double sum = 0.0;
+      for (unsigned g = 0; g < gridDim.x; ++g)
+        sum += __longlong_as_double((long long)__hip_atomic_load(rows + (size_t)g * Cin + c, __ATOMIC_RELAXED, __HIP_MEMORY_SCOPE_AGENT));
+      sets.s[s].dgamma[c] = (float)sum;
+    }
+  }
+  if (tid == 0) __hip_atomic_store(counter, 0u, __ATOMIC_RELAXED, __HIP_MEMORY_SCOPE_AGENT);
+}
+
 extern "C" int eml_dense_conv3x3_bwd_data_f32(const float* G, int ldg, int c0, const float* W2, const float* Z,
                                               const float* zmean, const float* zistd, float* DZ, int B, int H, int W,
                                               double* partials, int grid, const float* X, int ldx, int cx,
@@ -2956,12 +3088,59 @@
   return eml::check_launch("eml_dense_bn_dgamma_direct_f32(reduce)");
 }
 
+extern "C" int eml_dense_bn_dgamma_direct_multi_f32(int n, const float* X, int ldx, long P, int Hin, int Win, int pool,
+                                                    const float* const* DY, const int* ld_dy, const float* const* Zr,
+                                                    const int* ld_z, const float* const* cA, const float* const* cB,
+                                                    const float* const* cC, const int* Cout, const float* const* W,
+                                                    const int* Cin, const float* const* scale1,
+                                                    const float* const* shift1, const float* mean, const float* istd,
+                                                    const int* const* cond, double* scratch, float* const* dgamma,
+                                                    int grid, eml_stream_t stream) {
+  if (n < 1 || n > 2) return eml::fail(EML_EINVAL, "eml_dense_bn_dgamma_direct_multi_f32: n must be 1 or 2 (got %d)", n);
+  if (!X || !DY || !ld_dy || !Zr || !ld_z || !cA || !cB || !cC || !Cout || !W || !Cin || !scale1 || !shift1 || !mean ||
+      !istd || !cond || !scratch || !dgamma || P < 1 || grid < 1 || (pool && ((Hin | Win) & 1)))
+    return eml::fail(EML_EINVAL, "eml_dense_bn_dgamma_direct_multi_f32: bad arguments (even maps when pooled)");
+  DgammaSets sets{};
+  for (int j = 0; j < n; ++j) {
+    if (!DY[j] || !W[j] || !scale1[j] || !shift1[j] || !cond[j] || !dgamma[j] || Cin[j] < 1 || Cin[j] > 384 || Cout[j] < 1 ||
+        Cout[j] > 192 || Cin[j] > ldx || Cout[j] > ld_dy[j] || (Zr[j] && (!cA[j] || !cB[j] || !cC[j] || Cout[j] > ld_z[j])))
+      return eml::fail(EML_EINVAL, "eml_dense_bn_dgamma_direct_multi_f32: bad arguments of set %d (Cin <= 384, Cout <= 192)", j);
+    sets.s[j] = DgammaSet{DY[j], Zr[j], cA[j], cB[j], cC[j], W[j], scale1[j], shift1[j], cond[j], dgamma[j],
+                          ld_dy[j], ld_z[j], Cout[j], Cin[j]};
+  }
+  hipLaunchKernelGGL(bn_dgamma_direct_multi_kernel, dim3(grid), dim3(256), 0, (hipStream_t)stream, X, ldx, P, Hin, Win,
+                     pool, mean, istd, n, sets, scratch);
+  return eml::check_launch("eml_dense_bn_dgamma_direct_multi_f32");
+}
+
+static inline bool w1_pair_last_chunks(int Cout) {
+  const int nch = (Cout + 47) / 48;
+  return nch >= 2 && Cout - 48 * (nch - 2) <= 64;
+}
+
+extern "C" long eml_dense_conv1x1_bwd_weight_scratch_floats(int grid, int Kp, int Cout) {
+  if (grid < 1 || Kp < 1 || Cout < 1) return 0;
+  return (long)grid * Kp * 48 * (Cout > 48 ? 2 : 1);
+}
+
 extern "C" int eml_dense_conv1x1_bwd_weight_f32(const float* X, int ldx, long P, int Hin, int Win, int pool, int Kp,
                                                 int Cin, const float* scale1, const float* shift1, const float* DY,
                                                 int ld_dy, const float* Zr, int ld_z, const float* cA, const float* cB,
                                                 const float* cC, int Cout, float* partial, float* dW, int grid,
                                                 float* dz_out, const float* W1, int k_lo, const float* G, int ldg,
                                                 float* N12, double* partials_n, eml_stream_t stream) {
+  return eml_dense_conv1x1_bwd_weight_ex_f32(X, ldx, P, Hin, Win, pool, Kp, Cin, scale1, shift1, DY, ld_dy, Zr, ld_z, cA,
+                                             cB, cC, Cout, partial, dW, grid, dz_out, W1, k_lo, G, ldg, N12, partials_n,
+                                             grid > 0 && Kp > 0 ? (long)grid * Kp * 48 : 0, stream);
+}
+
+extern "C" int eml_dense_conv1x1_bwd_weight_ex_f32(const float* X, int ldx, long P, int Hin, int Win, int pool, int Kp,
+                                                   int Cin, const float* scale1, const float* shift1, const float* DY,
+                                                   int ld_dy, const float* Zr, int ld_z, const float* cA,
+                                                   const float* cB, const float* cC, int Cout, float* partial,
+                                                   float* dW, int grid, float* dz_out, const float* W1, int k_lo,
+                                                   const float* G, int ldg, float* N12, double* partials_n,
+                                                   long partial_floats, eml_stream_t stream) {
   if (dz_out && (Cout != 48 || pool))
     return eml::fail(EML_EINVAL, "eml_dense_conv1x1_bwd_weight_f32: dz_out is for dense layers (Cout == 48, no pool)");
   if (N12 && (Cout != 48 || pool || !W1 || !G || !partials_n || k_lo < 0 || (k_lo & 1) || k_lo + 12 > Cin || (ldg & 1) ||
@@ -2971,13 +3150,31 @@
   if (!X || !scale1 || !shift1 || !DY || !Zr || !cA || !cB || !cC || !partial || !dW || P < 1 || grid < 1 || Kp < 32 ||
       (Kp & 15) || Cin > Kp || Cout < 1)
     return eml::fail(EML_EINVAL, "eml_dense_conv1x1_bwd_weight_f32: bad arguments");
+  if (partial_floats < (long)grid * Kp * 48)
+    return eml::fail(EML_EINVAL, "eml_dense_conv1x1_bwd_weight_ex_f32: partial_floats = %ld, below grid*Kp*48 = %ld",
+                     partial_floats, (long)grid * Kp * 48);
   const int nchunks = (Cout + 47) / 48;
+  const bool pair_last = nchunks > 1 && !pool && w1_pair_last_chunks(Cout) &&
+                         partial_floats >= eml_dense_conv1x1_bwd_weight_scratch_floats(grid, Kp, Cout);
   for (int ch = 0; ch < nchunks; ++ch) {
     const int n0 = ch * 48, nv = (Cout - n0 < 48) ? Cout - n0 : 48;
     int n_load = ((ld_dy < ld_z ? ld_dy : ld_z) - n0) & ~3;
+    const NarrowArgs na{W1, G, N12, partials_n, Cin, k_lo, ldg};
+    if (pair_last && ch == nchunks - 2) {
+      const int nv2 = Cout - n0;
+      if (n_load > 96) n_load = 96;
+      if (n_load < nv2) return eml::fail(EML_EINVAL, "eml_dense_conv1x1_bwd_weight_ex_f32: DY/Zr rows narrower than Cout");
+      hipLaunchKernelGGL((conv1x1_bwd_weight_kernel<false, false, 2, 4>), dim3(grid), dim3(256), 0, (hipStream_t)stream, X,
+                         ldx, (int)P, Hin, Win, Kp, scale1, shift1, DY + n0, ld_dy, Zr + n0, ld_z, cA + n0, cB + n0, cC + n0,
+                         nv2, n_load, partial, nullptr, na);
+      int rc = eml::check_launch("eml_dense_conv1x1_bwd_weight_ex_f32");
+      if (rc) return rc;
+      hipLaunchKernelGGL(reduce_rows_chunks_kernel, dim3((Cin * 48 + 63) / 64, 2), dim3(256), 0, (hipStream_t)stream,
+                         partial, grid, (size_t)Kp * 48, (size_t)grid * Kp * 48, Cin, nv2, n0, dW);
+      return eml::check_launch("eml_dense_conv1x1_bwd_weight_ex_f32(reduce)");
+    }
     if (n_load > 48) n_load = 48;
     if (n_load < nv) return eml::fail(EML_EINVAL, "eml_dense_conv1x1_bwd_weight_f32: DY/Zr rows narrower than Cout");
-    const NarrowArgs na{W1, G, N12, partials_n, Cin, k_lo, ldg};
     static const int vec_env = [] { const char* v = getenv("EML_W1_VEC"); return v ? atoi(v) : 0; }();
     const bool vec4 = !pool && (ldx & 3) == 0 && (reinterpret_cast<uintptr_t>(X) & 15) == 0 &&
                       vec_env == 4;
diff --git a/include/emlight_hip.h b/include/emlight_hip.h
--- a/include/emlight_hip.h
+++ b/include/emlight_hip.h
@@ -188,6 +188,14 @@
                                    const float* istd, const int* cond, double* scratch, float* dgamma,
                                    int grid, eml_stream_t stream);
 
+int eml_dense_bn_dgamma_direct_multi_f32(int n, const float* X, int ldx, long P, int Hin, int Win, int pool,
+                                         const float* const* DY, const int* ld_dy, const float* const* Zr,
+                                         const int* ld_z, const float* const* cA, const float* const* cB,
+                                         const float* const* cC, const int* Cout, const float* const* W,
+                                         const int* Cin, const float* const* scale1, const float* const* shift1,
+                                         const float* mean, const float* istd, const int* const* cond,
+                                         double* scratch, float* const* dgamma, int grid, eml_stream_t stream);
+
 int eml_dense_conv1x1_bwd_weight_f32(const float* X, int ldx, long P, int Hin, int Win, int pool,
                                      int Kp, int Cin, const float* scale1, const float* shift1,
                                      const float* DY, int ld_dy, const float* Zr, int ld_z,
@@ -195,6 +203,16 @@
                                      float* partial, float* dW, int grid, float* dz_out,
                                      const float* W1, int k_lo, const float* G, int ldg, float* N12,
                                      double* partials_n, eml_stream_t stream);
+
+long eml_dense_conv1x1_bwd_weight_scratch_floats(int grid, int Kp, int Cout);
+
+int eml_dense_conv1x1_bwd_weight_ex_f32(const float* X, int ldx, long P, int Hin, int Win, int pool,
+                                        int Kp, int Cin, const float* scale1, const float* shift1,
+                                        const float* DY, int ld_dy, const float* Zr, int ld_z,
+                                        const float* cA, const float* cB, const float* cC, int Cout,
+                                        float* partial, float* dW, int grid, float* dz_out,
+                                        const float* W1, int k_lo, const float* G, int ldg, float* N12,
+                                        double* partials_n, long partial_floats, eml_stream_t stream);
 
 int eml_dense_permute_w1_bwd_f32(const float* W, int Cout, int Cin, int Kp, int Ko, float* Wd,
                                  eml_stream_t stream);
```

Result: no change. 569.2 images/s, median of 6 (+0.4%).
